# JunkyByte/easy_ViTPose

Measured on AMD Instinct MI355X. Metric: persons_per_sec, higher is better.
Workload: dtype fp16; 1 GPU; ViTPose-B coco K=17, batch 256 x 256x192 crops per GPU (f32 input resident in HBM) -> (y,x,conf) keypoints in HBM; global_batch=256, weights=seeded random init (no checkpoint offline)

## Files before the change

### easy_vitpose_amd/_capi.py

```python
from __future__ import annotations

import ctypes as C
import os

LIB_PATH = os.path.join(os.path.dirname(os.path.abspath(__file__)), '_lib', 'libvitpose_hip.so')

VP_OK, VP_ERR_INVALID, VP_ERR_HIP, VP_ERR_STATE, VP_ERR_MISSING_TENSOR, VP_ERR_SHAPE = range(6)
VP_DTYPE_F16, VP_DTYPE_BF16, VP_DTYPE_FP8 = 0, 1, 2
VP_INPUT_F32_NCHW, VP_INPUT_U8_NHWC = 0, 1
VP_PIX_RGB24, VP_PIX_BGR24, VP_PIX_NV12 = 0, 1, 2
VP_YUV_BT601, VP_YUV_BT709, VP_YUV_BT601_FULL = 0, 1, 2
VP_PROF_NAMES = ['gemm_proj', 'gemm_fc1', 'gemm_qkv', 'gemm_patch', 'gemm_deconv', 'gemm_final',
                 'attention', 'layernorm', 'im2col', 'decode', 'gemm_fc2']
VP_PROF_COUNT = len(VP_PROF_NAMES)
DTYPES = {'fp16': VP_DTYPE_F16, 'f16': VP_DTYPE_F16, 'bf16': VP_DTYPE_BF16, 'fp8': VP_DTYPE_FP8}

SYMBOLS = ['vp_abi_version', 'vp_create', 'vp_load_weights', 'vp_infer', 'vp_infer_device', 'vp_infer_device_stream', 'vp_host_alloc', 'vp_host_free',
           'vp_infer_submit', 'vp_infer_wait', 'vp_group_create', 'vp_group_size', 'vp_group_member', 'vp_group_load_weights', 'vp_group_infer',
           'vp_group_infer_allgather', 'vp_group_destroy', 'vp_group_last_error', 'vp_infer_frame', 'vp_infer_flip', 'vp_infer_heatmaps',
           'vp_infer_tokens', 'vp_decode_only', 'vp_stream', 'vp_synchronize', 'vp_set_profiling',
           'vp_reset_profile', 'vp_get_profile', 'vp_profile_kernel', 'vp_group_peer_access_missing', 'vp_destroy', 'vp_last_error',
           'vp_dbg_gemm', 'vp_dbg_attention', 'vp_dbg_layernorm', 'vp_dbg_deconv', 'vp_dbg_gemm_case', 'vp_dbg_crop_prep',
           'vp_dbg_group_plan', 'vp_dbg_group_trace', 'vp_dbg_gemm8_pick', 'vp_dbg_gemm2_pick', 'vp_dbg_splitk_pick', 'vp_dbg_run_batch', 'vp_dbg_fp8_gemm', 'vp_dbg_mx_gemm', 'vp_dbg_host_e4m3', 'vp_dbg_gemm_fp8_case', 'vp_dbg_qkvattn',
           'vp_expert_info', 'vp_set_expert', 'vp_infer_experts', 'vp_dbg_expert_tile', 'vp_infer_frames', 'vp_dbg_frame_plan',
           'vp_dbg_chunk_plan', 'vp_infer_boxes_stream', 'vp_dbg_box_geometry',
           'vp_set_flip_test', 'vp_clear_flip_test', 'vp_flip_test_enabled', 'vp_group_set_flip_test', 'vp_group_clear_flip_test',
           'vp_dbg_flip_partner', 'vp_dbg_flip_layout', 'vp_dbg_decode_flip',
           'vp_infer_experts_device_stream', 'vp_infer_frames_experts', 'vp_infer_boxes_experts_stream', 'vp_dbg_mix_plan', 'vp_dbg_decode_mix',
           'vp_set_flip_test_experts', 'vp_dbg_mix_plan_flip', 'vp_dbg_decode_flip_mix',
           'vp_infer_images', 'vp_infer_boxes_images_stream', 'vp_dbg_image_plan', 'vp_dbg_crop_prep_image',
           'vp_dbg_gemm_case_planes', 'vp_dbg_gemm_fp8_case_planes', 'vp_dbg_attention_case',
           'vp_pose_nms_stream', 'vp_pose_nms', 'vp_dbg_pose_nms_host', 'vp_dbg_pose_oks',
           'vp_dbg_ln_finalize', 'vp_dbg_gemm_case_lnpart', 'vp_dbg_qkvattn_ln', 'vp_dbg_ln_quant',
           'vp_infer_images_affine', 'vp_infer_boxes_affine_stream', 'vp_dbg_box_cs', 'vp_dbg_affine_plan', 'vp_dbg_crop_affine', 'vp_dbg_decode_affine',
           'vp_dbg_decode_affine_flip',
           'vp_draw_poses_stream', 'vp_draw_poses', 'vp_dbg_draw_host',
           'vp_tracker_create', 'vp_tracker_destroy', 'vp_tracker_reset_stream', 'vp_tracker_update_stream', 'vp_tracker_update', 'vp_tracker_state_bytes',
           'vp_tracker_download_state', 'vp_dbg_track_host', 'vp_dbg_lsap']


class HipExtensionMissing(RuntimeError):
    pass


class VpError(RuntimeError):
    def __init__(self, code: int, msg: str):
        super().__init__(f'[vitpose_hip status {code}] {msg}')
        self.code = code
        self.msg = msg


class vp_config(C.Structure):
    _fields_ = [('embed_dim', C.c_int32), ('depth', C.c_int32), ('num_heads', C.c_int32),
                ('num_keypoints', C.c_int32), ('dtype', C.c_int32), ('device_id', C.c_int32),
                ('max_batch', C.c_int32)]


class vp_tensor_desc(C.Structure):
    _fields_ = [('name', C.c_char_p), ('data', C.POINTER(C.c_float)), ('numel', C.c_int64)]


class vp_frame(C.Structure):
    _fields_ = [('data', C.c_void_p), ('h', C.c_int32), ('w', C.c_int32)]


class vp_image(C.Structure):
    _fields_ = [('plane', C.c_void_p * 2), ('pitch', C.c_int64 * 2), ('h', C.c_int32), ('w', C.c_int32), ('format', C.c_int32), ('matrix', C.c_int32)]


class vp_pose_nms_cfg(C.Structure):
    _fields_ = [('oks_thr', C.c_float), ('vis_thr', C.c_float), ('use_vis_thr', C.c_int32), ('soft', C.c_int32), ('max_dets', C.c_int32),
                ('n_sigmas', C.c_int32), ('sigmas', C.c_void_p)]


class vp_draw_cfg(C.Structure):
    _fields_ = [('conf_thr', C.c_float), ('radius', C.c_int32), ('thickness', C.c_int32), ('n_limbs', C.c_int32), ('limbs', C.c_void_p),
                ('n_point_colors', C.c_int32), ('point_colors', C.c_void_p), ('n_limb_colors', C.c_int32), ('limb_colors', C.c_void_p)]


class vp_track_cfg(C.Structure):
    _fields_ = [('max_age', C.c_int32), ('min_hits', C.c_int32), ('iou_threshold', C.c_float), ('n_streams', C.c_int32)]


class vp_profile(C.Structure):
    _fields_ = [('ms', C.c_double * VP_PROF_COUNT), ('flops', C.c_double * VP_PROF_COUNT),
                ('bytes', C.c_double * VP_PROF_COUNT), ('launches', C.c_int64 * VP_PROF_COUNT)]


_lib = None


def load_library():
    global _lib
    if _lib is not None:
        return _lib
    lib_path = os.environ.get('VP_HIP_LIB', LIB_PATH)
    if not os.path.exists(lib_path):
        raise HipExtensionMissing(
            f'{lib_path} not found. Build it with `python -m easy_vitpose_amd.build` '
            '(needs hipcc). There is no CPU fallback for the ViTPose path.')
    try:
        lib = C.CDLL(lib_path)
    except OSError as e:
        raise HipExtensionMissing(f'cannot load {lib_path}: {e}') from e
    H = C.c_void_p
    lib.vp_abi_version.restype = C.c_int
    lib.vp_create.argtypes = [C.POINTER(H), C.POINTER(vp_config)]
    lib.vp_load_weights.argtypes = [H, C.POINTER(vp_tensor_desc), C.c_int32]
    lib.vp_infer.argtypes = [H, C.c_void_p, C.c_int32, C.c_int32, C.c_void_p, C.c_void_p]
    lib.vp_infer_device.argtypes = [H, C.c_void_p, C.c_int32, C.c_int32, C.c_void_p, C.c_void_p, C.c_int32]
    lib.vp_infer_device_stream.argtypes = [H, C.c_void_p, C.c_int32, C.c_int32, C.c_void_p, C.c_void_p, C.c_void_p]
    lib.vp_host_alloc.argtypes = [C.c_size_t]
    lib.vp_host_alloc.restype = C.c_void_p
    lib.vp_host_free.argtypes = [C.c_void_p]
    lib.vp_host_free.restype = None
    lib.vp_infer_submit.argtypes = [H, C.c_void_p, C.c_int32, C.c_int32, C.c_void_p, C.c_void_p, C.POINTER(C.c_int32)]
    lib.vp_infer_wait.argtypes = [H, C.c_int32]
    lib.vp_group_create.argtypes = [C.POINTER(H), C.POINTER(vp_config), C.POINTER(C.c_int32), C.c_int32]
    lib.vp_group_size.argtypes = [H]
    lib.vp_group_member.argtypes = [H, C.c_int32]
    lib.vp_group_member.restype = C.c_void_p
    lib.vp_group_load_weights.argtypes = [H, C.POINTER(vp_tensor_desc), C.c_int32]
    lib.vp_group_infer.argtypes = [H, C.c_void_p, C.c_int32, C.c_int32, C.c_void_p, C.c_void_p]
    lib.vp_group_infer_allgather.argtypes = [H, C.c_void_p, C.c_int32, C.c_int32, C.c_void_p, C.POINTER(C.c_void_p), C.c_void_p]
    lib.vp_group_destroy.argtypes = [H]
    lib.vp_group_last_error.argtypes = [H]
    lib.vp_group_last_error.restype = C.c_char_p
    lib.vp_infer_frame.argtypes = [H, C.c_void_p, C.c_int32, C.c_int32, C.c_void_p, C.c_int32, C.c_void_p]
    lib.vp_infer_frames.argtypes = [H, C.POINTER(vp_frame), C.c_int32, C.c_int32, C.c_void_p, C.c_int32, C.c_void_p]
    lib.vp_dbg_frame_plan.argtypes = [C.POINTER(vp_frame), C.c_int32, C.c_void_p, C.c_int32, C.c_void_p]
    lib.vp_infer_boxes_stream.argtypes = [H, C.POINTER(vp_frame), C.c_int32, C.c_void_p, C.c_int32, C.c_void_p, C.c_int32, C.c_int32,
                                          C.c_void_p, C.c_void_p, C.c_void_p, C.c_void_p]
    lib.vp_dbg_box_geometry.argtypes = [C.c_void_p, C.c_int32, C.c_void_p, C.c_void_p, C.c_int32, C.c_int32, C.c_int32, C.c_void_p, C.c_void_p]
    lib.vp_dbg_crop_prep.argtypes = [C.c_int32, C.c_void_p, C.c_int32, C.c_int32, C.c_void_p, C.c_int32, C.c_void_p]
    lib.vp_infer_heatmaps.argtypes = [H, C.c_void_p, C.c_int32, C.c_int32, C.c_void_p]
    lib.vp_infer_tokens.argtypes = [H, C.c_void_p, C.c_int32, C.c_int32, C.c_void_p]
    lib.vp_decode_only.argtypes = [C.c_int32, C.c_void_p, C.c_int32, C.c_int32, C.c_void_p, C.c_void_p]
    lib.vp_stream.argtypes = [H]
    lib.vp_stream.restype = C.c_void_p
    lib.vp_synchronize.argtypes = [H]
    lib.vp_set_profiling.argtypes = [H, C.c_int32]
    lib.vp_reset_profile.argtypes = [H]
    lib.vp_get_profile.argtypes = [H, C.POINTER(vp_profile)]
    lib.vp_destroy.argtypes = [H]
    lib.vp_last_error.argtypes = [H]
    lib.vp_last_error.restype = C.c_char_p
    lib.vp_dbg_gemm.argtypes = [C.c_int32] * 6 + [C.c_void_p] * 5
    lib.vp_dbg_attention.argtypes = [C.c_int32] * 5 + [C.c_void_p] * 2
    lib.vp_dbg_attention_case.argtypes = [C.c_int32] * 6 + [C.c_void_p] * 3
    lib.vp_dbg_layernorm.argtypes = [C.c_int32] * 4 + [C.c_void_p] * 5
    lib.vp_dbg_deconv.argtypes = [C.c_int32] * 6 + [C.c_void_p, C.POINTER(vp_tensor_desc), C.c_int32, C.c_void_p]
    lib.vp_infer_flip.argtypes = [C.c_void_p, C.c_void_p, C.c_int32, C.c_int32, C.c_void_p, C.c_void_p, C.c_int32, C.c_int32,
                                  C.c_void_p, C.c_void_p]
    lib.vp_dbg_gemm_case.argtypes = [C.c_int32] * 9 + [C.c_void_p] * 8
    if hasattr(lib, 'vp_dbg_gemm8_timeline'):
        lib.vp_dbg_gemm8_timeline.argtypes = [C.c_int32] * 9 + [C.POINTER(C.c_uint64), C.c_int32]
        lib.vp_dbg_gemm_timeline.argtypes = [C.c_int32] * 6 + [C.POINTER(C.c_uint64), C.c_int32]
        lib.vp_dbg_gemm8_timeline.restype = lib.vp_dbg_gemm_timeline.restype = C.c_int
        lib.vp_dbg_gemm_bench.argtypes = [C.c_int32] * 9 + [C.POINTER(C.c_float)]
        lib.vp_dbg_gemm_bench2.argtypes = [C.c_int32] * 10 + [C.POINTER(C.c_float)]
        lib.vp_dbg_gemm_compare.argtypes = [C.c_int32] * 13 + [C.POINTER(C.c_uint64), C.POINTER(C.c_double)]
        lib.vp_dbg_peak.argtypes = [C.c_int32, C.c_int32, C.POINTER(C.c_double)]
        for n_ in ('vp_dbg_gemm_bench', 'vp_dbg_gemm_bench2', 'vp_dbg_gemm_compare', 'vp_dbg_peak'):
            getattr(lib, n_).restype = C.c_int
    lib.vp_profile_kernel.argtypes = [H, C.c_int32, C.c_char_p, C.c_int32]
    lib.vp_group_peer_access_missing.argtypes = [H]
    lib.vp_dbg_group_plan.argtypes = [C.c_int32] * 3 + [C.c_void_p, C.c_void_p, C.c_int32]
    lib.vp_dbg_gemm8_pick.argtypes = [C.c_int32] * 4 + [C.c_void_p]
    lib.vp_dbg_gemm2_pick.argtypes = [C.c_int32] * 4 + [C.c_void_p]
    lib.vp_dbg_splitk_pick.argtypes = [C.c_int32] * 3 + [C.c_void_p]
    lib.vp_dbg_run_batch.argtypes = [C.c_int32] * 3
    lib.vp_dbg_group_trace.argtypes = [C.c_int32] * 3 + [C.c_void_p, C.c_int32]
    lib.vp_dbg_fp8_gemm.argtypes = [C.c_int32] * 4 + [C.c_void_p] * 7
    lib.vp_dbg_mx_gemm.argtypes = [C.c_int32] * 4 + [C.c_void_p] * 7
    lib.vp_dbg_host_e4m3.argtypes = [C.c_void_p, C.c_void_p, C.c_int64]
    lib.vp_dbg_gemm_fp8_case.argtypes = [C.c_int32] * 5 + [C.c_void_p] * 8
    lib.vp_dbg_gemm_case_planes.argtypes = [C.c_int32] * 9 + [C.c_void_p] * 6 + [C.c_int32] + [C.c_void_p] * 3
    lib.vp_dbg_gemm_fp8_case_planes.argtypes = [C.c_int32] * 4 + [C.c_void_p] * 5 + [C.c_int32] + [C.c_void_p] * 5
    lib.vp_expert_info.argtypes = [H, C.c_void_p, C.c_void_p, C.c_void_p]
    lib.vp_set_expert.argtypes = [H, C.c_int32]
    lib.vp_infer_experts.argtypes = [H, C.c_void_p, C.c_int32, C.c_int32, C.c_void_p, C.c_void_p, C.c_void_p]
    lib.vp_dbg_expert_tile.argtypes = [C.c_int32] * 4 + [C.c_void_p, C.c_int32]
    lib.vp_infer_experts_device_stream.argtypes = [H, C.c_void_p, C.c_int32, C.c_int32, C.c_void_p, C.c_void_p, C.c_void_p, C.c_void_p]
    lib.vp_infer_frames_experts.argtypes = [H, C.POINTER(vp_frame), C.c_int32, C.c_int32, C.c_void_p, C.c_int32, C.c_void_p, C.c_void_p]
    lib.vp_infer_boxes_experts_stream.argtypes = [H, C.POINTER(vp_frame), C.c_int32, C.c_void_p, C.c_int32, C.c_void_p, C.c_int32, C.c_int32,
                                                  C.c_void_p, C.c_void_p, C.c_void_p, C.c_void_p, C.c_void_p]
    lib.vp_dbg_mix_plan.argtypes = [C.c_void_p, C.c_int32, C.c_int32, C.c_int32] + [C.c_void_p] * 6
    lib.vp_dbg_decode_mix.argtypes = [C.c_int32, C.c_void_p, C.c_int32, C.c_int32, C.c_int32, C.c_void_p, C.c_void_p, C.c_void_p]
    lib.vp_dbg_chunk_plan.argtypes = [C.POINTER(vp_config), C.c_int32, C.c_void_p, C.c_int32]
    lib.vp_dbg_qkvattn.argtypes = [C.c_int32] * 5 + [C.c_void_p] * 4
    lib.vp_dbg_qkvattn_ln.argtypes = [C.c_int32] * 5 + [C.c_void_p] * 6
    lib.vp_dbg_ln_finalize.argtypes = [C.c_int32] * 4 + [C.c_void_p] * 2
    lib.vp_dbg_gemm_case_lnpart.argtypes = [C.c_int32] * 9 + [C.c_void_p] * 4 + [C.c_int32] + [C.c_void_p] * 2
    lib.vp_dbg_ln_quant.argtypes = [C.c_int32] * 5 + [C.c_void_p] * 4
    lib.vp_set_flip_test.argtypes = [H, C.c_void_p, C.c_int32, C.c_int32]
    lib.vp_clear_flip_test.argtypes = [H]
    lib.vp_flip_test_enabled.argtypes = [H]
    lib.vp_group_set_flip_test.argtypes = [H, C.c_void_p, C.c_int32, C.c_int32]
    lib.vp_group_clear_flip_test.argtypes = [H]
    lib.vp_set_flip_test_experts.argtypes = [H, C.c_void_p, C.c_void_p, C.c_int32]
    lib.vp_dbg_mix_plan_flip.argtypes = [C.c_void_p, C.c_int32, C.c_int32, C.c_int32] + [C.c_void_p] * 6
    lib.vp_dbg_decode_flip_mix.argtypes = [C.c_int32, C.c_void_p, C.c_int32, C.c_int32, C.c_int32, C.c_void_p, C.c_void_p, C.c_int32, C.c_int32, C.c_void_p, C.c_void_p]
    lib.vp_infer_images.argtypes = [H, C.POINTER(vp_image), C.c_int32, C.c_int32, C.c_void_p, C.c_int32, C.c_void_p, C.c_void_p]
    lib.vp_infer_boxes_images_stream.argtypes = [H, C.POINTER(vp_image), C.c_int32, C.c_void_p, C.c_int32, C.c_void_p, C.c_int32, C.c_int32,
                                                 C.c_void_p, C.c_void_p, C.c_void_p, C.c_void_p, C.c_void_p]
    lib.vp_dbg_image_plan.argtypes = [C.POINTER(vp_image), C.c_int32, C.c_void_p, C.c_int32, C.c_void_p]
    lib.vp_dbg_crop_prep_image.argtypes = [C.c_int32, C.POINTER(vp_image), C.c_void_p, C.c_int32, C.c_void_p]
    lib.vp_dbg_flip_partner.argtypes = [C.c_int32, C.c_void_p, C.c_int32, C.c_void_p]
    lib.vp_dbg_flip_layout.argtypes = [C.c_int32, C.c_int32, C.c_void_p, C.c_void_p]
    lib.vp_dbg_decode_flip.argtypes = [C.c_int32, C.c_void_p, C.c_int32, C.c_int32, C.c_void_p, C.c_int32, C.c_int32, C.c_void_p, C.c_void_p]
    nms_host = [C.c_void_p, C.c_int32, C.c_int32, C.c_void_p, C.c_int32, C.c_void_p, C.c_void_p, C.c_int32, C.POINTER(vp_pose_nms_cfg), C.c_void_p, C.c_void_p, C.c_void_p]
    lib.vp_pose_nms_stream.argtypes = [H] + nms_host + [C.c_void_p]
    lib.vp_pose_nms.argtypes = [H] + nms_host
    lib.vp_dbg_pose_nms_host.argtypes = nms_host
    lib.vp_dbg_pose_oks.argtypes = [C.c_int32, C.c_void_p, C.c_int32, C.c_int32, C.c_void_p, C.POINTER(vp_pose_nms_cfg), C.c_void_p]
    lib.vp_infer_images_affine.argtypes = [H, C.POINTER(vp_image), C.c_int32, C.c_int32, C.c_void_p, C.c_void_p, C.c_int32, C.c_void_p]
    lib.vp_infer_boxes_affine_stream.argtypes = [H, C.POINTER(vp_image), C.c_int32, C.c_void_p, C.c_int32, C.c_void_p, C.c_int32, C.c_float,
                                                 C.c_void_p, C.c_void_p, C.c_void_p, C.c_void_p]
    lib.vp_dbg_box_cs.argtypes = [C.c_void_p, C.c_int32, C.c_void_p, C.c_int32, C.c_int32, C.c_float, C.c_void_p, C.c_void_p]
    lib.vp_dbg_affine_plan.argtypes = [C.POINTER(vp_image), C.c_int32, C.c_void_p, C.c_void_p, C.c_int32, C.c_void_p]
    lib.vp_dbg_crop_affine.argtypes = [C.c_int32, C.POINTER(vp_image), C.c_void_p, C.c_int32, C.c_void_p]
    lib.vp_dbg_decode_affine.argtypes = [C.c_int32, C.c_void_p, C.c_int32, C.c_int32, C.c_void_p, C.c_void_p]
    lib.vp_dbg_decode_affine_flip.argtypes = [C.c_int32, C.c_void_p, C.c_int32, C.c_int32, C.c_void_p, C.c_int32, C.c_int32, C.c_void_p, C.c_void_p]
    draw_host = [C.POINTER(vp_image), C.c_int32, C.c_void_p, C.c_int32, C.c_int32, C.c_void_p, C.c_int32, C.c_void_p, C.c_void_p, C.c_void_p, C.c_int32,
                 C.POINTER(vp_draw_cfg)]
    lib.vp_draw_poses_stream.argtypes = [H] + draw_host + [C.c_void_p]
    lib.vp_draw_poses.argtypes = [H] + draw_host
    lib.vp_dbg_draw_host.argtypes = draw_host
    trk_io = [C.c_void_p, C.c_int32, C.c_void_p, C.c_int32, C.c_uint64, C.c_void_p, C.c_void_p, C.c_void_p, C.c_int32, C.c_void_p, C.c_void_p]
    lib.vp_tracker_create.argtypes = [H, C.POINTER(vp_track_cfg), C.POINTER(C.c_void_p)]
    lib.vp_tracker_destroy.argtypes = [C.c_void_p]
    lib.vp_tracker_reset_stream.argtypes = [C.c_void_p, C.c_uint64, C.c_void_p]
    lib.vp_tracker_update_stream.argtypes = [C.c_void_p] + trk_io + [C.c_void_p]
    lib.vp_tracker_update.argtypes = [C.c_void_p] + trk_io
    lib.vp_tracker_state_bytes.argtypes = [C.c_int32, C.POINTER(C.c_int64)]
    lib.vp_tracker_download_state.argtypes = [C.c_void_p, C.c_void_p]
    lib.vp_dbg_track_host.argtypes = [C.c_void_p, C.POINTER(vp_track_cfg)] + trk_io
    lib.vp_dbg_lsap.argtypes = [C.c_int32, C.c_void_p, C.c_int32, C.c_int32, C.c_float, C.c_void_p]
    for name in SYMBOLS:
        if name not in ('vp_stream', 'vp_last_error', 'vp_host_alloc', 'vp_host_free', 'vp_group_member', 'vp_group_last_error'):
            getattr(lib, name).restype = C.c_int
    _lib = lib
    return lib


def last_error(handle=None) -> str:
    lib = load_library()
    s = lib.vp_last_error(handle)
    return s.decode('utf-8', 'replace') if s else ''


def check(code: int, handle=None):
    if code != VP_OK:
        raise VpError(code, last_error(handle))
```

### easy_vitpose_amd/csrc/api_internal.h

```cpp
#pragma once
#include <hip/hip_runtime.h>

#include <algorithm>
#include <cmath>
#include <cstdio>
#include <cstdlib>
#include <cstring>
#include <string>
#include <unordered_map>
#include <vector>

#include "../../include/vitpose_hip.h"
#ifdef VP_TOOLS
#include "../../include/vitpose_hip_tools.h"
#endif
#include "kernels.h"
#include "mx8.h"

namespace vpi {

struct Block {
    float *ln1_g, *ln1_b, *ln2_g, *ln2_b;
    uint16_t *w_qkv, *w_proj, *w_fc1, *w_fc2;
    float *b_qkv, *b_proj, *b_fc1, *b_fc2;
    float *s_qkv, *s_fc1;
    uint16_t* w_qkvh = nullptr;
    float *b_qkvh = nullptr, *s_qkvh = nullptr;
    uint8_t *w_qkv8 = nullptr, *w_fc18 = nullptr, *w_fc28 = nullptr, *w_proj8 = nullptr;
    float *ws_qkv = nullptr, *ws_fc1 = nullptr, *ws_fc2 = nullptr, *ws_proj = nullptr;
};

struct Switches {
    int g8_stagger = 0;
    int gemm8_mask = 0x7;
    long g8_min_tiles = 448;
    bool persist_gemm = true;
    int order_mask = 8;
    bool blocked_hid = true;
    bool blocked_qkv = true;
    bool fuse_ln = true;
    bool fuse_qkv_attn = true;
    bool qa_min_set = false;
    long qa_min_tiles = 108;
    long qa80_min_tiles = 192;
    int qa80_group = 8;
    int attn_qsplit = 128;
    int g8_bm192 = 3;
    bool pad_batch = true;
    bool g8_cost_model = true;
    bool deconv_parity_fast = true;
    bool fuse_head = true;
    bool fp8_proj16 = false;
    int graph_max_n = 16;
    bool graph_null = true;
    int caller_stream_max_n = 16;
    bool fold_rule = true;
    int graph_max_n_stats = 8;
    bool splitk_on = true;
    int splitk_force[2][2] = {{0, 0}, {0, 0}};
    int gemm_variant[VP_PROF_COUNT] = {-1, -1, -1, -1, -1, -1, -1, -1, -1, -1, -1};
    int gemm_group_m[VP_PROF_COUNT] = {0};
    int fam_ablate[VP_PROF_COUNT] = {0};
};

}

namespace vpi {
struct MixPlan {
    int nb = 0;
    std::vector<int32_t> order, ids;
    std::vector<int> seg_e, seg_s;
    uint64_t pattern = 0;
};
}

struct vp_ctx {
    vp_config cfg;
    vpi::Switches sw;
    int D, L, heads, Kp, dtype, maxb;
    hipStream_t stream = nullptr;
    std::string err;
    bool loaded = false;
    std::vector<void*> allocs;
    uint16_t* w_patch = nullptr;
    float* pos = nullptr;
    std::vector<vpi::Block> blocks;
    float *lnf_g = nullptr, *lnf_b = nullptr;
    uint16_t *w_d1 = nullptr, *w_d2 = nullptr, *w_fin = nullptr;
    size_t fin_rows = 0;
    float *b_d1 = nullptr, *b_d2 = nullptr, *b_fin = nullptr, *b_zero = nullptr;
    uint16_t* zero = nullptr;
    void* in_stage = nullptr;
    int32_t* wh_stage = nullptr;
    float* x = nullptr;
    uint16_t *y = nullptr, *qkv = nullptr, *hid = nullptr, *d1 = nullptr, *d2 = nullptr;
    float *hm = nullptr, *kp = nullptr, *tok = nullptr;
    float* hm_keep = nullptr;
    int32_t* partner = nullptr;
    bool flip_on = false;
    int flip_shift = 0;
    uint32_t flip_gen = 0, flip_counter = 0;
    int32_t* flip_table = nullptr;
    std::vector<int32_t> flip_pairs;
    bool flip_ex = false;
    int32_t* flip_tables = nullptr;
    float *ln_part = nullptr, *rowstat = nullptr;
    bool fp8 = false;
    size_t Mp = 0;
    uint8_t *x8 = nullptr, *xs8 = nullptr, *hs8 = nullptr;
    uint8_t *y8 = nullptr, *ys8 = nullptr;
    struct Slot {
        void* in = nullptr; int32_t* wh = nullptr; float* kp = nullptr; hipEvent_t h2d = nullptr, done = nullptr, out = nullptr; bool busy = false;
        float* host_kp = nullptr; float* user_out = nullptr; size_t out_bytes = 0;
        char* host_in = nullptr; size_t host_in_cap = 0;
    };
    Slot slots[2];
    hipStream_t copy_stream = nullptr;
    hipStream_t d2h_stream = nullptr;
    int next_slot = 0;
    struct GraphKey {
        int n = 0, fmt = -1;
        const void* src = nullptr; const int32_t* wh = nullptr; float* out = nullptr;
        int expert = 0;
        const int32_t* post = nullptr;
        uint32_t flip = 0;
        const float* cs = nullptr;
        uint64_t mix = 0;
        bool wide = false;
        bool operator==(const GraphKey& o) const {
            return n == o.n && fmt == o.fmt && src == o.src && wh == o.wh && out == o.out && expert == o.expert && post == o.post && flip == o.flip &&
                   cs == o.cs && mix == o.mix && wide == o.wide;
        }
    };
    struct GraphEntry { GraphKey key; hipGraphExec_t exec = nullptr; bool no_graph = false; };
    GraphEntry graphs[4];
    int graph_victim = 0;
    float* splitk_ws = nullptr;
    size_t splitk_rows = 0;
    hipEvent_t ev_in = nullptr, ev_out = nullptr;
    hipStream_t own_stream = nullptr;
    const void* last_stream_id = nullptr;
    bool foreign_pending = false;
    hipEvent_t ev_sw = nullptr;
    uint8_t* frame_stage = nullptr;
    size_t frame_cap = 0;
    vp::CropRec* crecs = nullptr;
    vp::AffRec* arecs = nullptr;
    float* cs_stage = nullptr;
    void* draw_ws = nullptr;
    int32_t* box_aux = nullptr;
    struct Head { uint16_t *w_d1 = nullptr, *w_d2 = nullptr, *w_fin = nullptr; float *b_d1 = nullptr, *b_d2 = nullptr, *b_fin = nullptr; size_t fin_rows = 0; int K = 0; };
    int Kmax = 0;
    int n_experts = 0, part_features = 0, expert = 0;
    size_t fc2_w_stride = 0, fc2_b_stride = 0;
    std::vector<Head> ex_heads;
    int32_t* expert_ids = nullptr;
    void* mix_stage = nullptr;
    size_t mix_stage_cap = 0;
    const int32_t* mix_expert = nullptr;
    std::vector<int> mix_bounds;
    int32_t* mix_slot = nullptr;
    vp::MixRec* mix_recs = nullptr;
    vp::MixRecFlip* mix_recs_flip = nullptr;
    const vpi::MixPlan* mix = nullptr;
    vpi::MixPlan mix_host;
    std::vector<int32_t> mix_ks, mix_first, mix_k;
    uint32_t prof = 0;
    int gemm_ablate = 0;
    struct Ev { hipEvent_t a, b; int fam; double flops, bytes; };
    std::vector<Ev> evs;
    std::vector<std::pair<hipEvent_t, hipEvent_t>> ev_pool;
    vp_profile acc{};
    std::string kernel_desc[VP_PROF_COUNT];
};

namespace vpi {

extern thread_local std::string g_create_error;

int fail(vp_ctx* c, int code, const std::string& msg);
int need_weights(vp_ctx* c);
bool slots_busy(const vp_ctx* c);
int slots_idle(vp_ctx* c, const char* who);
int quiesce(vp_ctx* c);
inline size_t crop_bytes(int fmt) { return (size_t)3 * 256 * 192 * (fmt == VP_INPUT_F32_NCHW ? 4 : 1); }

#define HIPCHK(c, expr)                                                                         \
    do {                                                                                        \
        hipError_t e__ = (expr);                                                                \
        if (e__ != hipSuccess)                                                                  \
            return fail((c), VP_ERR_HIP, std::string(#expr) + ": " + hipGetErrorString(e__));   \
    } while (0)

template <class T> int dalloc(vp_ctx* c, T** p, size_t count) {
    void* q = nullptr;
    HIPCHK(c, hipMalloc(&q, count * sizeof(T) + 256));
    c->allocs.push_back(q);
    *p = (T*)q;
    return VP_OK;
}

uint16_t host_to_bits(float v, int dtype);
float host_from_bits(uint16_t h, int dtype);
size_t pad128(size_t n);
// ... 115 lines not shown
```

### easy_vitpose_amd/csrc/debug_taps.hip

```cpp
#include "dbg_util.h"

using namespace vpi;


static int upload_planes(vp_ctx* c, uint16_t** dst, const float* aux, const uint16_t* r_hi, const uint16_t* r_lo, size_t MN) {
    if (!(r_hi && r_lo) && !aux) return fail(c, VP_ERR_INVALID, "aux required");
    std::vector<uint16_t> hp(2 * MN);
    if (r_hi && r_lo) {
        std::memcpy(hp.data(), r_hi, MN * 2);
        std::memcpy(hp.data() + MN, r_lo, MN * 2);
    } else
        for (size_t i = 0; i < MN; ++i) {
            const uint16_t hi = host_to_bits(aux[i], c->dtype);
            hp[i] = hi;
            hp[MN + i] = host_to_bits(aux[i] - host_from_bits(hi, c->dtype), c->dtype);
        }
    int r;
    if ((r = dalloc(c, dst, 2 * MN))) return r;
    if (hipMemcpy(*dst, hp.data(), hp.size() * 2, hipMemcpyHostToDevice) != hipSuccess) return fail(c, VP_ERR_HIP, "H2D");
    return VP_OK;
}
static int download_planes(vp_ctx* c, const uint16_t* planes, float* out, uint16_t* o_hi, uint16_t* o_lo, size_t MN) {
    if (o_hi && o_lo) {
        if (hipMemcpy(o_hi, planes, MN * 2, hipMemcpyDeviceToHost) != hipSuccess || hipMemcpy(o_lo, planes + MN, MN * 2, hipMemcpyDeviceToHost) != hipSuccess)
// ... 80 lines not shown
    const size_t out_bytes = mx ? MD : MD * 2;
    if ((rc = dalloc(c, &dq, M * N3)) || (rc = dalloc(c, &dout, out_bytes)) || (mx && (rc = dalloc(c, &dsc, MD / 32)))) return dbg_finish(c, rc);
    hipError_t e = hipMemcpy(dq, hq.data(), hq.size() * 2, hipMemcpyHostToDevice);
    if (e == hipSuccess) e = hipMemset(dout, 0xff, out_bytes);
    if (e == hipSuccess && mx) e = hipMemset(dsc, 0xff, MD / 32);
    if (e == hipSuccess) e = vp::attention_launch(c->dtype, dq, (uint16_t*)dout, B, D, heads, nullptr, qsplit, blocked, dsc);
    if (e == hipSuccess) e = hipDeviceSynchronize();
    if (e != hipSuccess) return dbg_finish(c, fail(c, VP_ERR_HIP, std::string("attention case: ") + hipGetErrorString(e)));
    if (!mx) return dbg_finish(c, download16(c, (const uint16_t*)dout, out, MD));
    std::vector<uint8_t> co(MD), so(MD / 32);
    if (hipMemcpy(co.data(), dout, MD, hipMemcpyDeviceToHost) != hipSuccess || hipMemcpy(so.data(), dsc, MD / 32, hipMemcpyDeviceToHost) != hipSuccess)
        return dbg_finish(c, fail(c, VP_ERR_HIP, "D2H"));
    for (size_t m = 0; m < M; ++m)
        for (size_t n = 0; n < (size_t)D; ++n) {
            const uint8_t sb = so[vp::mx_scale_off(m, n >> 5, D)];
            out[m * D + n] = vp_host_e4m3_to_float(co[vp::mx_code_off(m, n, D)]) * std::ldexp(1.0f, (int)sb - 127);
            if (!(n & 31)) out_scales[m * (D / 32) + (n >> 5)] = sb;
        }
    return dbg_finish(c, VP_OK);
}

}

static int qkvattn_case(int32_t device, int32_t dtype, int32_t npairs, int32_t D, int32_t heads, const float* x, const float* W, const float* bias, const float* rowstat,
                        const float* ln_s, float* out) {
    if (npairs <= 0 || D <= 0 || heads <= 0 || !x || !W || !bias || !out || !rowstat != !ln_s) return fail(nullptr, VP_ERR_INVALID, "bad qkvattn test shape");
    vp_ctx* c = dbg_ctx(device, dtype);
    if (!c) return VP_ERR_HIP;
    const size_t M = (size_t)npairs * 384;
    uint16_t *dx, *dw, *dwh, *dy;
    float *db, *dbh, *ds, *dsh, *drow;
    int rc;
    std::vector<float> zeros(3 * (size_t)D, 0.f), row(2 * M);
    for (size_t m = 0; m < M; ++m) { row[2 * m] = 0.f; row[2 * m + 1] = 1.f; }
    if ((rc = upload_mat(c, &dx, x, M, D, M)) || (rc = upload_mat(c, &dw, W, 3 * (size_t)D, D, pad128(3 * (size_t)D))) || (rc = upload_f32(c, &db, bias, 3 * (size_t)D)) ||
        (rc = upload_f32(c, &ds, ln_s ? ln_s : zeros.data(), 3 * (size_t)D)) || (rc = upload_f32(c, &drow, rowstat ? rowstat : row.data(), 2 * M)) || (rc = dalloc(c, &dwh, 3 * (size_t)D * D)) ||
        (rc = dalloc(c, &dbh, 3 * (size_t)D)) || (rc = dalloc(c, &dsh, 3 * (size_t)D)) || (rc = dalloc(c, &dy, M * D)))
        return dbg_finish(c, rc);
    if (heads * 80 == D) {
        uint16_t* dwh80; float *dbh80, *dsh80;
        const size_t rows = (size_t)heads * 256;
        if ((rc = dalloc(c, &dwh80, rows * D)) || (rc = dalloc(c, &dbh80, rows)) || (rc = dalloc(c, &dsh80, rows))) return dbg_finish(c, rc);
        hipError_t e8 = vp::qkv_head_major80_launch(dw, db, ds, dwh80, dbh80, dsh80, D, D, heads, nullptr);
        vp::GemmArgs g80{};
        g80.A = dx; g80.W = dwh80; g80.bias = dbh80; g80.ln_s = dsh80; g80.rowstat = drow; g80.out = dy;
        g80.M = (int)M; g80.N = heads * 256; g80.K = D; g80.ldo = D; g80.w_rows = heads * 256; g80.variant = 18;
        g80.attn_scale_log2e = vp::softmax_scale_log2e(80);
        if (e8 == hipSuccess && !vp::gemm8_supported(vp::EPI_QKV_ATTN, g80, 256, 192)) return dbg_finish(c, fail(c, VP_ERR_INVALID, "shape not supported by the fused qkv + attention tile (head dim 80)"));
        if (e8 == hipSuccess) e8 = vp::gemm_launch(c->dtype, vp::EPI_QKV_ATTN, g80, nullptr);
        if (e8 == hipSuccess) e8 = hipDeviceSynchronize();
        if (e8 != hipSuccess) return dbg_finish(c, fail(c, VP_ERR_HIP, std::string("qkvattn (head dim 80): ") + hipGetErrorString(e8)));
        return dbg_finish(c, download16(c, dy, out, M * D));
    }
    hipError_t e = vp::qkv_head_major_launch(dw, db, ds, dwh, dbh, dsh, D, D, nullptr);
    vp::QkvAttnArgs qa{};
    qa.x_hi = dx; qa.wh = dwh; qa.bh = dbh; qa.sh = dsh; qa.rowstat = drow; qa.y = dy; qa.npairs = npairs; qa.ncrops = 2 * npairs; qa.heads = heads; qa.D = D;
    qa.scale_log2e = vp::softmax_scale_log2e(64);
    if (e == hipSuccess && !vp::qkvattn_supported(qa)) return dbg_finish(c, fail(c, VP_ERR_INVALID, "shape not supported by the fused qkv + attention kernel"));
    if (e == hipSuccess) e = vp::qkvattn_launch(c->dtype, qa, nullptr, nullptr, 0);
    if (e == hipSuccess) e = hipDeviceSynchronize();
    if (e != hipSuccess) return dbg_finish(c, fail(c, VP_ERR_HIP, std::string("qkvattn: ") + hipGetErrorString(e)));
    return dbg_finish(c, download16(c, dy, out, M * D));
}

extern "C" {

VP_API int vp_dbg_qkvattn(int32_t device, int32_t dtype, int32_t npairs, int32_t D, int32_t heads, const float* x, const float* W, const float* bias, float* out) {
    return qkvattn_case(device, dtype, npairs, D, heads, x, W, bias, nullptr, nullptr, out);
}

VP_API int vp_dbg_qkvattn_ln(int32_t device, int32_t dtype, int32_t npairs, int32_t D, int32_t heads, const float* x, const float* W, const float* bias,
                             const float* rowstat, const float* ln_s, float* out) {
    if (!rowstat || !ln_s) return fail(nullptr, VP_ERR_INVALID, "bad qkvattn test shape");
    return qkvattn_case(device, dtype, npairs, D, heads, x, W, bias, rowstat, ln_s, out);
}

VP_API int vp_dbg_ln_finalize(int32_t device, int32_t M, int32_t tiles, int32_t D, const float* partials, float* rowstat) {
    if (M <= 0 || tiles <= 0 || D <= 0 || !partials || !rowstat) return fail(nullptr, VP_ERR_INVALID, "bad ln_finalize case");
    vp_ctx* c = dbg_ctx(device, VP_DTYPE_F16);
    if (!c) return VP_ERR_HIP;
    float *dP, *dR;
    int rc;
    if ((rc = upload_f32(c, &dP, partials, (size_t)M * tiles * 2)) || (rc = dalloc(c, &dR, (size_t)M * 2))) return dbg_finish(c, rc);
    hipError_t e = hipMemset(dR, 0xff, (size_t)M * 8);
    if (e == hipSuccess) e = vp::ln_finalize_launch(dP, dR, M, tiles, D, nullptr);
    if (e == hipSuccess) e = hipDeviceSynchronize();
    if (e == hipSuccess) e = hipMemcpy(rowstat, dR, (size_t)M * 8, hipMemcpyDeviceToHost);
    if (e != hipSuccess) rc = fail(c, VP_ERR_HIP, std::string("ln_finalize: ") + hipGetErrorString(e));
    return dbg_finish(c, rc);
}

VP_API int vp_dbg_ln_quant(int32_t device, int32_t dtype, int32_t M, int32_t Mp, int32_t D, const uint16_t* x_hi, const float* partials, uint8_t* codes, uint8_t* scales) {
    if (M <= 0 || Mp < M || Mp % 64 || D <= 0 || D % 128 || !x_hi || !partials || !codes || !scales || (dtype != VP_DTYPE_F16 && dtype != VP_DTYPE_BF16))
        return fail(nullptr, VP_ERR_INVALID, "bad ln_quant case");
    vp_ctx* c = dbg_ctx(device, dtype);
    if (!c) return VP_ERR_HIP;
    const size_t MD = (size_t)M * D, PD = (size_t)Mp * D;
    uint16_t* dX;
    float* dP;
    uint8_t *dC, *dS;
    int rc;
    if ((rc = dalloc(c, &dX, MD)) || (rc = upload_f32(c, &dP, partials, (size_t)M * (D / 64) * 2)) || (rc = dalloc(c, &dC, PD)) || (rc = dalloc(c, &dS, PD / 32)))
        return dbg_finish(c, rc);
    hipError_t e = hipMemcpy(dX, x_hi, MD * 2, hipMemcpyHostToDevice);
    if (e == hipSuccess) e = hipMemset(dC, 0xff, PD);
    if (e == hipSuccess) e = hipMemset(dS, 0xff, PD / 32);
    if (e == hipSuccess) e = vp::ln_quant_launch(c->dtype, dX, dP, D / 64, dC, dS, M, Mp, D, nullptr);
    if (e == hipSuccess) e = hipDeviceSynchronize();
    if (e == hipSuccess) e = hipMemcpy(codes, dC, PD, hipMemcpyDeviceToHost);
    if (e == hipSuccess) e = hipMemcpy(scales, dS, PD / 32, hipMemcpyDeviceToHost);
    if (e != hipSuccess) rc = fail(c, VP_ERR_HIP, std::string("ln_quant: ") + hipGetErrorString(e));
    return dbg_finish(c, rc);
}

VP_API int vp_dbg_layernorm(int32_t device, int32_t dtype, int32_t M, int32_t D, const float* x, const float* gamma,
                            const float* beta, float* out16, float* out32) {
    vp_ctx* c = dbg_ctx(device, dtype);
    if (!c) return VP_ERR_HIP;
    float *dx, *dg, *db, *d32;
    uint16_t* d16;
    int rc;
    const size_t MD = (size_t)M * D;
    if ((rc = upload_f32(c, &dx, x, MD)) || (rc = upload_f32(c, &dg, gamma, D)) || (rc = upload_f32(c, &db, beta, D)) ||
        (rc = dalloc(c, &d32, MD)) || (rc = dalloc(c, &d16, MD))) return dbg_finish(c, rc);
    hipError_t e = vp::layernorm_launch(c->dtype, dx, dg, db, d16, d32, M, D, nullptr);
    if (e == hipSuccess) e = hipDeviceSynchronize();
    if (e == hipSuccess) e = hipMemcpy(out32, d32, MD * 4, hipMemcpyDeviceToHost);
    if (e != hipSuccess) return dbg_finish(c, fail(c, VP_ERR_HIP, std::string("layernorm: ") + hipGetErrorString(e)));
    return dbg_finish(c, download16(c, d16, out16, MD));
}

VP_API int vp_dbg_deconv(int32_t device, int32_t dtype, int32_t B, int32_t Hin, int32_t Win, int32_t Cin, const float* x,
                         const vp_tensor_desc* tensors, int32_t n_tensors, float* out) {
    vp_ctx* c = dbg_ctx(device, dtype);
    if (!c) return VP_ERR_HIP;
    Lookup lk;
    lk.c = c;
    for (int i = 0; i < n_tensors; ++i) lk.map[tensors[i].name] = &tensors[i];
    uint16_t *dx, *dw, *dout;
    float* db;
    int rc;
    const size_t Min = (size_t)B * Hin * Win;
    if ((rc = pack_deconv(c, lk, 0, Cin, &dw, &db))) return dbg_finish(c, rc);
    if ((rc = upload_mat(c, &dx, x, Min, Cin, Min))) return dbg_finish(c, rc);
    if ((rc = dalloc(c, &dout, Min * 4 * 256))) return dbg_finish(c, rc);
    if ((rc = dalloc(c, &c->zero, (size_t)256))) return dbg_finish(c, rc);
    if (hipMemset(c->zero, 0, 512) != hipSuccess) return dbg_finish(c, fail(c, VP_ERR_HIP, "memset"));
    rc = gemm(c, 0, vp::EPI_DECONV, resolve_gemm(c->sw, 0, vp::EPI_DECONV, (int)Min, 256, 4 * Cin), dx, dw, db, dout, nullptr, (int)Min, 256, 4 * Cin, 256, Hin, Win, Cin);
    if (!rc && hipDeviceSynchronize() != hipSuccess) rc = fail(c, VP_ERR_HIP, "deconv kernel failed");
    if (!rc) rc = download16(c, dout, out, Min * 4 * 256);
    return dbg_finish(c, rc);
}


static int gemm_case(int32_t device, int32_t dtype, int32_t epi, int32_t variant, int32_t group_m, int32_t flags, int32_t M, int32_t N, int32_t K, const float* A,
                     const float* W, const float* bias, const float* aux, const float* rowstat, const float* ln_s, float* out, float* stats, const PlaneIO* io,
                     const float* ln_part = nullptr, int ln_tiles = 0) {
    if (M <= 0 || N <= 0 || K <= 0 || K % 64 || !A || !W || !bias) return fail(nullptr, VP_ERR_INVALID, "bad gemm case");
    vp_ctx* c = dbg_ctx(device, dtype);
    if (!c) return VP_ERR_HIP;
    c->Kp = N;
    int r;
    const size_t MN = (size_t)M * N, wrows = pad128(N);
    const bool ablk = (flags & 4) != 0, oblk = (flags & 2) != 0;
    uint16_t *dA, *dW;
    float *dB, *dAux32 = nullptr, *dRow = nullptr, *dS = nullptr, *dStats = nullptr;
    uint16_t* dAux16 = nullptr;
    void* dOut = nullptr;
    {
        std::vector<uint16_t> ha((size_t)M * K);
        for (size_t m = 0; m < (size_t)M; ++m)
            for (size_t k = 0; k < (size_t)K; ++k) {
                const size_t dst = ablk ? ((((m >> 6) * (K >> 6) + (k >> 6)) << 12) + ((m & 63) << 6) + (k & 63)) : m * K + k;
                ha[dst] = host_to_bits(A[m * K + k], c->dtype);
            }
        if ((r = dalloc(c, &dA, (size_t)M * K))) return dbg_finish(c, r);
        if (hipMemcpy(dA, ha.data(), ha.size() * 2, hipMemcpyHostToDevice) != hipSuccess) return dbg_finish(c, fail(c, VP_ERR_HIP, "H2D"));
    }
    size_t fin_rows = 0;
    if (epi == vp::EPI_HEATMAP) { if ((r = upload_final(c, &dW, W, N, K, &fin_rows))) return dbg_finish(c, r); }
    else if ((r = upload_mat(c, &dW, W, N, K, wrows))) return dbg_finish(c, r);
    if ((r = upload_f32(c, &dB, bias, N, wrows)) || (r = dalloc(c, &c->zero, (size_t)256))) return dbg_finish(c, r);
    vp::GemmArgs g{};
    g.A = dA; g.W = dW; g.bias = dB; g.M = M; g.N = N; g.K = K; g.ldo = N; g.zero = c->zero; g.Kp = N;
    g.w_rows = (int)wrows; g.variant = variant; g.group_m = group_m;
    g.persist = (flags & 1) != 0; g.out_blocked = oblk; g.a_blocked = ablk; g.reverse = (flags & 8) != 0;
    if (rowstat && ln_s) {
        if ((r = upload_f32(c, &dRow, rowstat, (size_t)M * 2)) || (r = upload_f32(c, &dS, ln_s, N, wrows))) return dbg_finish(c, r);
        g.rowstat = dRow; g.ln_s = dS;
    }
    if (ln_part) {
        float* dPart;
        if ((r = upload_f32(c, &dPart, ln_part, (size_t)M * ln_tiles * 2)) || (r = upload_f32(c, &dS, ln_s, N, wrows))) return dbg_finish(c, r);
        g.ln_part = dPart; g.ln_tiles = ln_tiles; g.ln_inv_d = 1.0f / (float)K; g.ln_s = dS;
    }
    size_t out_bytes = 0;
    const bool prod = epi == vp::EPI_BIAS_RESID_LN || epi == vp::EPI_POS_LN;
    if (epi == vp::EPI_BIAS || epi == vp::EPI_BIAS_GELU) out_bytes = MN * 2;
    else if (epi == vp::EPI_BIAS_RESID || epi == vp::EPI_POS || prod) out_bytes = MN * 4;
    else if (epi == vp::EPI_HEATMAP) { out_bytes = MN * 4; g.N = (int)fin_rows; g.ldo = 0; g.w_rows = (int)pad128(fin_rows); }
    else return dbg_finish(c, fail(c, VP_ERR_INVALID, "unsupported epilogue"));
    if (epi == vp::EPI_BIAS_RESID || epi == vp::EPI_POS || epi == vp::EPI_POS_LN) {
        if (!aux) return dbg_finish(c, fail(c, VP_ERR_INVALID, "aux required"));
        if ((r = upload_f32(c, &dAux32, aux, epi == vp::EPI_BIAS_RESID ? MN : (size_t)192 * N))) return dbg_finish(c, r);
        g.aux = dAux32;
    }
    if (epi == vp::EPI_BIAS_RESID_LN) {
        if ((r = upload_planes(c, &dAux16, aux, io ? io->r_hi : nullptr, io ? io->r_lo : nullptr, MN))) return dbg_finish(c, r);
        g.aux = (const float*)dAux16;
    }
    if (prod) {
        g.plane = MN;
        if ((r = dalloc(c, &dStats, (size_t)M * (N / 64) * 2))) return dbg_finish(c, r);
        g.stats_out = dStats;
    }
    if (io && io->in_place) dOut = dAux16;
    else {
        char* o;
        if ((r = dalloc(c, &o, out_bytes))) return dbg_finish(c, r);
        dOut = o;
        hipMemset(dOut, 0xff, out_bytes);
    }
    g.out = dOut;
    const int splitk = (flags >> 8) & 15;
    hipError_t e;
    if (splitk > 1) {
        if (epi != vp::EPI_BIAS_RESID_LN) return dbg_finish(c, fail(c, VP_ERR_INVALID, "split-K is a residual-GEMM path (epi 6)"));
        float* ws = nullptr;
        if ((r = dalloc(c, &ws, (size_t)splitk * MN))) return dbg_finish(c, r);
        hipMemset(ws, 0xff, (size_t)splitk * MN * 4);
        vp::GemmArgs p = g;
        p.out = ws; p.aux = nullptr; p.bias = nullptr; p.stats_out = nullptr; p.plane = 0; p.splitk = splitk; p.persist = 0;
        e = vp::gemm_launch(c->dtype, vp::EPI_PARTIAL, p, nullptr);
        if (e == hipSuccess) e = vp::splitk_reduce_launch(c->dtype, ws, splitk, dB, dAux16, MN, dStats, M, N, nullptr);
        dOut = dAux16;
    } else {
        e = vp::gemm_launch(c->dtype, epi, g, nullptr);
    }
    if (e == hipSuccess) e = hipDeviceSynchronize();
    if (e != hipSuccess) return dbg_finish(c, fail(c, VP_ERR_HIP, std::string("gemm case: ") + hipGetErrorString(e)));
    if (epi == vp::EPI_BIAS || epi == vp::EPI_BIAS_GELU) {
        std::vector<float> t(MN);
        if ((r = download16(c, (const uint16_t*)dOut, t.data(), MN))) return dbg_finish(c, r);
        for (size_t m = 0; m < (size_t)M; ++m)
            for (size_t n = 0; n < (size_t)N; ++n) {
                const size_t src = oblk ? ((((m >> 6) * ((size_t)N >> 6) + (n >> 6)) << 12) + ((m & 63) << 6) + (n & 63)) : m * N + n;
                out[m * N + n] = t[src];
            }
    } else if (prod) {
        if ((r = download_planes(c, (const uint16_t*)dOut, out, io ? io->o_hi : nullptr, io ? io->o_lo : nullptr, MN))) return dbg_finish(c, r);
        if (stats && hipMemcpy(stats, dStats, (size_t)M * (N / 64) * 8, hipMemcpyDeviceToHost) != hipSuccess) return dbg_finish(c, fail(c, VP_ERR_HIP, "D2H"));
    } else {
        if (hipMemcpy(out, dOut, out_bytes, hipMemcpyDeviceToHost) != hipSuccess) return dbg_finish(c, fail(c, VP_ERR_HIP, "D2H"));
    }
    return dbg_finish(c, VP_OK);
}

VP_API int vp_dbg_gemm_case(int32_t device, int32_t dtype, int32_t epi, int32_t variant, int32_t group_m, int32_t flags, int32_t M,
                            int32_t N, int32_t K, const float* A, const float* W, const float* bias, const float* aux, const float* rowstat,
                            const float* ln_s, float* out, float* stats) {
    if (!out) return fail(nullptr, VP_ERR_INVALID, "bad gemm case");
    return gemm_case(device, dtype, epi, variant, group_m, flags, M, N, K, A, W, bias, aux, rowstat, ln_s, out, stats, nullptr);
}

VP_API int vp_dbg_gemm_case_lnpart(int32_t device, int32_t dtype, int32_t epi, int32_t variant, int32_t group_m, int32_t flags, int32_t M, int32_t N, int32_t K,
                                   const float* A, const float* W, const float* bias, const float* partials, int32_t ln_tiles, const float* ln_s, float* out) {
    if ((epi != vp::EPI_BIAS && epi != vp::EPI_BIAS_GELU) || !partials || ln_tiles <= 0 || !ln_s || !out) return fail(nullptr, VP_ERR_INVALID, "bad gemm ln_part case");
    return gemm_case(device, dtype, epi, variant, group_m, flags, M, N, K, A, W, bias, nullptr, nullptr, ln_s, out, nullptr, nullptr, partials, ln_tiles);
}

VP_API int vp_dbg_gemm_case_planes(int32_t device, int32_t dtype, int32_t epi, int32_t variant, int32_t group_m, int32_t flags, int32_t M, int32_t N, int32_t K,
                                   const float* A, const float* W, const float* bias, const uint16_t* r_hi, const uint16_t* r_lo, const float* pos,
                                   int32_t in_place, uint16_t* o_hi, uint16_t* o_lo, float* stats) {
    if ((epi != vp::EPI_BIAS_RESID_LN && epi != vp::EPI_POS_LN) || !o_hi || !o_lo || !stats || (epi == vp::EPI_BIAS_RESID_LN ? !r_hi || !r_lo : !pos || in_place))
        return fail(nullptr, VP_ERR_INVALID, "bad gemm planes case");
    const PlaneIO io{r_hi, r_lo, o_hi, o_lo, in_place != 0};
    return gemm_case(device, dtype, epi, variant, group_m, flags, M, N, K, A, W, bias, pos, nullptr, nullptr, nullptr, stats, &io);
}

VP_API int vp_dbg_crop_prep_image(int32_t device, const vp_image* image, const int32_t* crop_params, int32_t n, uint8_t* out) {
    if (!image || !crop_params || !out || n <= 0) return fail(nullptr, VP_ERR_INVALID, "bad argument");
    std::vector<int32_t> p9((size_t)n * 9, 0);
    for (int i = 0; i < n; ++i) std::memcpy(&p9[9 * (size_t)i + 1], crop_params + 8 * (size_t)i, 32);
    int32_t band[2];
    std::string why;
    if (image_plan(image, 1, p9.data(), n, band, &why)) return fail(nullptr, VP_ERR_INVALID, why);
    vp_ctx* c = dbg_ctx(device, VP_DTYPE_F16);
    if (!c) return VP_ERR_HIP;
    std::vector<vp::CropRec> recs;
    uint8_t* dout;
    vp::CropRec* drec;
    int rc;
    const size_t ob = (size_t)n * 256 * 192 * 3;
    if ((rc = stage_frames(c, image, 1, false, p9.data(), n, band, recs)) || (rc = dalloc(c, &dout, ob)) || (rc = dalloc(c, &drec, (size_t)n)))
        return dbg_finish(c, rc);
    hipError_t e = hipMemcpy(drec, recs.data(), (size_t)n * sizeof(vp::CropRec), hipMemcpyHostToDevice);
    if (e == hipSuccess) e = vp::crop_resize_launch(drec, dout, n, nullptr);
    if (e == hipSuccess) e = hipDeviceSynchronize();
    if (e == hipSuccess) e = hipMemcpy(out, dout, ob, hipMemcpyDeviceToHost);
    if (e != hipSuccess) rc = fail(c, VP_ERR_HIP, std::string("crop_prep: ") + hipGetErrorString(e));
    return dbg_finish(c, rc);
}

VP_API int vp_dbg_crop_affine(int32_t device, const vp_image* image, const float* cs, int32_t n, uint8_t* out) {
    if (!image || !cs || !out || n <= 0) return fail(nullptr, VP_ERR_INVALID, "bad argument");
    int32_t band[2];
// ... 158 lines not shown
```

### easy_vitpose_amd/csrc/forward.hip

```cpp
#include "api_internal.h"
#include "tiles.h"

using namespace vpi;

namespace vpi {

static void note_kernel(vp_ctx* c, int fam, const char* desc) {
    if (desc[0] && c->kernel_desc[fam] != desc) c->kernel_desc[fam] = desc;
}

int gemm(vp_ctx* c, int fam, int epi, const GemmPick& pk, const uint16_t* A, const uint16_t* W, const float* bias, void* out,
         const float* aux, int M, int N, int K, int ldo, int Hin, int Win, int Cin, const LnFuse* ln) {
    vp::GemmArgs g{};
    g.A = A; g.W = W; g.bias = bias; g.out = out; g.aux = aux;
    g.M = M; g.N = N; g.K = K; g.ldo = ldo;
    g.Hin = Hin; g.Win = Win; g.Cin = Cin; g.zero = c->zero; g.Kp = c->Kp;
    g.w_rows = (int)pad128((size_t)N);
    g.variant = pk.variant; g.group_m = pk.group_m; g.persist = pk.persist; g.stagger = pk.stagger;
    g.ablate = c->gemm_ablate | c->sw.fam_ablate[fam];
    g.parity_fast = c->sw.deconv_parity_fast;
    if (c->mix_expert && fam == VP_PROF_GEMM_FC2) g.expert = c->mix_expert;
    if (ln) {
        g.a_blocked = ln->a_blocked; g.out_blocked = ln->out_blocked; g.reverse = ln->reverse;
        g.plane = ln->plane; g.stats_out = ln->stats_out; g.rowstat = ln->rowstat; g.ln_s = ln->ln_s;
        g.ln_part = ln->ln_part; g.ln_tiles = ln->ln_tiles; g.ln_inv_d = 1.0f / (float)K;
        if (ln->tiles_out) *ln->tiles_out = N / 64;
    }
    if (epi == vp::EPI_DECONV_FINAL) { g.W2 = c->w_fin; g.bias2 = c->b_fin; g.out2 = (float*)out; g.out = nullptr; }
    const bool deconv = epi == vp::EPI_DECONV || epi == vp::EPI_DECONV_FINAL;
    const double par = deconv ? 4.0 : 1.0;
    const double Nalg = (epi == vp::EPI_HEATMAP) ? (double)c->Kp : (double)N;
    double flops = 2.0 * M * Nalg * K * par;
    const bool resid = epi == vp::EPI_BIAS_RESID || epi == vp::EPI_BIAS_RESID_LN;
    const bool f32out = resid || epi == vp::EPI_POS || epi == vp::EPI_POS_LN || epi == vp::EPI_HEATMAP;
    const double out_b = f32out ? 4.0 : 2.0;
    double bytes = 2.0 * M * (double)(deconv ? Cin : K) + 2.0 * N * (double)K * par + out_b * M * Nalg * par;
    if (epi == vp::EPI_DECONV_FINAL) {
        flops += 2.0 * M * par * (double)c->Kp * N;
        bytes += (4.0 * c->Kp - out_b * N) * M * par + 2.0 * c->fin_rows * N;
    }
    if (resid) bytes += 4.0 * M * (double)N;
    if (epi == vp::EPI_BIAS_RESID_LN || epi == vp::EPI_POS_LN) bytes += 8.0 * M * (double)(N / 64);
    char desc[192];
    desc[0] = 0;
    g.desc = desc; g.desc_cap = (int)sizeof(desc);
    if (pk.splitk > 1) {
        if (out != (void*)aux || (size_t)M > c->splitk_rows || !c->splitk_ws) return fail(c, VP_ERR_INVALID, "split-K: a residual GEMM in place within the workspace only");
        vp::GemmArgs p = g;
        p.out = c->splitk_ws; p.aux = nullptr; p.bias = nullptr; p.stats_out = nullptr; p.plane = 0;
        p.variant = pk.splitk_variant; p.group_m = 0; p.splitk = pk.splitk; p.ldo = N; p.persist = 0;
        LAUNCH(c, fam, flops, bytes, vp::gemm_launch(c->dtype, vp::EPI_PARTIAL, p, c->stream));
        if (desc[0]) {
            char d2[224];
            snprintf(d2, sizeof(d2), "%s x split-K %d + splitk_reduce_kernel", desc, pk.splitk);
            note_kernel(c, fam, d2);
        }
        LAUNCH(c, fam, 0.0, 0.0, vp::splitk_reduce_launch(c->dtype, c->splitk_ws, pk.splitk, bias, (uint16_t*)out, g.plane, g.stats_out, M, N, c->stream));
        return VP_OK;
    }
    LAUNCH(c, fam, flops, bytes, vp::gemm_launch(c->dtype, epi, g, c->stream));
    note_kernel(c, fam, desc);
    return VP_OK;
}

int gemm_fp8(vp_ctx* c, int fam, int epi, const GemmPick& pk, const uint8_t* A8, const uint8_t* a_scales, const uint8_t* W8, const float* w_scale, const float* bias,
             void* out, uint8_t* out_scales, const float* aux, int M, int N, int K, const LnFuse* ln) {
    vp::GemmArgs g{};
    g.A = (const uint16_t*)A8; g.W = (const uint16_t*)W8; g.bias = bias; g.out = out; g.aux = aux;
    g.M = M; g.N = N; g.K = K; g.ldo = N;
    g.a_scales = a_scales; g.w_scale = w_scale; g.out_scales = out_scales;
    g.w_rows = (int)pad128((size_t)N);
    if (ln) {
        g.out_blocked = ln->out_blocked; g.reverse = ln->reverse;
        g.plane = ln->plane; g.stats_out = ln->stats_out;
        if (ln->tiles_out) *ln->tiles_out = N / 64;
    }
    const int bn = vp::tile8_bn(pk.variant);
    g.group_m = pk.group_m;
    if (!vp::gemm8f_supported(epi, g, bn))
        return fail(c, VP_ERR_SHAPE, "fp8 mode: GEMM shape " + std::to_string(M) + " x " + std::to_string(N) + " x " + std::to_string(K) + " not supported by the MXFP8 kernel");
    const double flops = 2.0 * M * (double)N * K;
    double bytes = 1.0 * M * (double)K + M * (double)(K / 32) + 1.0 * N * (double)K;
    bytes += epi == vp::EPI_BIAS ? 2.0 * M * (double)N : epi == vp::EPI_BIAS_GELU ? (1.0 + 1.0 / 32) * M * (double)N : 8.0 * M * (double)N + 8.0 * M * (double)(N / 64);
    char desc[192];
    desc[0] = 0;
    g.desc = desc; g.desc_cap = (int)sizeof(desc);
    LAUNCH(c, fam, flops, bytes, vp::gemm8f_launch(epi, g, bn, c->stream));
    note_kernel(c, fam, desc);
    return VP_OK;
}

static const uint16_t* fc2_w(const vp_ctx* c, const vpi::Block& b) { return c->mix_expert ? b.w_fc2 : b.w_fc2 + (size_t)c->expert * c->fc2_w_stride; }
static const float* fc2_b(const vp_ctx* c, const vpi::Block& b) { return c->mix_expert ? b.b_fc2 : b.b_fc2 + (size_t)c->expert * c->fc2_b_stride; }

int forward_chunk(vp_ctx* c, const void* d_crops, int fmt, int n_in, const FwdOpts& o) {
    const int D = c->D;
    const ChunkPlan pl = plan_chunk(c->sw, D, c->heads, c->maxb, c->fp8, n_in, c->fin_rows, c->mix_expert ? &c->mix_bounds : nullptr);
    const GemmPick* pk = pl.gemm;
    const int n = pl.n;
    const int M = n * 192;
    const double in_b = (fmt == VP_INPUT_F32_NCHW ? 4.0 : 1.0) * n_in * 3.0 * 256 * 192;
    if (o.twin_src) LAUNCH(c, VP_PROF_IM2COL, 0.0, 0.5 * in_b + 2.0 * M * 768, vp::im2col_twin_launch(c->dtype, d_crops, fmt, c->hid, n, o.twin_src, c->stream));
    else LAUNCH(c, VP_PROF_IM2COL, 0.0, in_b + 2.0 * M * 768, vp::im2col_launch(c->dtype, d_crops, fmt, c->hid, n, c->stream, o.mirror, n_in));
    int rc;
    size_t plane = 0;
    const bool qkv_blocked = c->sw.blocked_qkv && D / c->heads == 64;
    auto attention = [&](uint16_t* out, double bytes, uint8_t* mx_scales) -> int {
        LAUNCH(c, VP_PROF_ATTN, 4.0 * 192 * 192 * (double)D * n, bytes,
               vp::attention_launch(c->dtype, c->qkv, out, n, D, c->heads, c->stream, pl.attn_qsplit, qkv_blocked ? 1 : 0, mx_scales));
        return VP_OK;
    };
    if (c->fp8) {
        const int Mp = (int)std::max<size_t>((size_t)(M + 255) / 256 * 256, 512);
        plane = c->Mp * (size_t)D;
        uint16_t* xh = (uint16_t*)c->x;
        int tiles = 0;
        LnFuse prod; prod.plane = plane; prod.stats_out = c->ln_part; prod.tiles_out = &tiles;
        auto quant = [&]() -> int {
            LAUNCH(c, VP_PROF_LAYERNORM, 0.0, 8.0 * M * tiles + 2.0 * M * D + (1.0 + 1.0 / 32) * Mp * (double)D,
                   vp::ln_quant_launch(c->dtype, xh, c->ln_part, tiles, c->x8, c->xs8, M, Mp, D, c->stream));
            return VP_OK;
        };
        if ((rc = gemm(c, VP_PROF_GEMM_PATCH, vp::EPI_POS_LN, pk[VP_PROF_GEMM_PATCH], c->hid, c->w_patch, c->b_zero, c->x, c->pos, M, D, 768, D, 0, 0, 0, &prod))) return rc;
        for (int l = 0; l < c->L; ++l) {
            const Block& b = c->blocks[l];
            if ((rc = quant())) return rc;
            LnFuse cq; cq.out_blocked = qkv_blocked;
            if ((rc = gemm_fp8(c, VP_PROF_GEMM_QKV, vp::EPI_BIAS, pk[VP_PROF_GEMM_QKV], c->x8, c->xs8, b.w_qkv8, b.ws_qkv, b.b_qkv, c->qkv, nullptr, nullptr, Mp, 3 * D, D, &cq))) return rc;
            LnFuse pp = prod;
            if (pl.proj_fp8) {
                if ((rc = attention((uint16_t*)c->y8, 7.0 * M * D, c->ys8))) return rc;
                if ((rc = gemm_fp8(c, VP_PROF_GEMM_PROJ, vp::EPI_BIAS_RESID_LN, pk[VP_PROF_GEMM_PROJ], c->y8, c->ys8, b.w_proj8, b.ws_proj, b.b_proj, c->x, nullptr, c->x, Mp, D, D, &pp))) return rc;
            } else {
                if ((rc = attention(c->y, 8.0 * M * D, nullptr))) return rc;
                if ((rc = gemm(c, VP_PROF_GEMM_PROJ, vp::EPI_BIAS_RESID_LN, pk[VP_PROF_GEMM_PROJ], c->y, b.w_proj, b.b_proj, c->x, c->x, M, D, D, D, 0, 0, 0, &pp))) return rc;
            }
            if ((rc = quant())) return rc;
            if ((rc = gemm_fp8(c, VP_PROF_GEMM_FC1, vp::EPI_BIAS_GELU, pk[VP_PROF_GEMM_FC1], c->x8, c->xs8, b.w_fc18, b.ws_fc1, b.b_fc1, c->hid, c->hs8, nullptr, Mp, 4 * D, D, nullptr))) return rc;
            LnFuse p2 = prod;
            if ((rc = gemm_fp8(c, VP_PROF_GEMM_FC2, vp::EPI_BIAS_RESID_LN, pk[VP_PROF_GEMM_FC2], (const uint8_t*)c->hid, c->hs8, b.w_fc28, b.ws_fc2, b.b_fc2, c->x, nullptr, c->x, Mp, D, 4 * D, &p2))) return rc;
        }
    } else if (c->sw.fuse_ln) {
        plane = (size_t)M * D;
        uint16_t* xh = (uint16_t*)c->x;
        int tiles = 0;
        LnFuse prod; prod.plane = plane; prod.stats_out = c->ln_part; prod.tiles_out = &tiles;
        auto finalize = [&](bool folded) -> int {
            if (folded) return VP_OK;
            LAUNCH(c, VP_PROF_LAYERNORM, 0.0, 8.0 * M * tiles + 8.0 * M, vp::ln_finalize_launch(c->ln_part, c->rowstat, M, tiles, D, c->stream));
            return VP_OK;
        };
        const double qkv_attn_flops = 2.0 * M * 3.0 * D * D + 4.0 * 192 * 192 * (double)D * n, qkv_attn_bytes = 2.0 * M * D + 2.0 * 3 * D * (double)D + 2.0 * M * D;
        if ((rc = gemm(c, VP_PROF_GEMM_PATCH, vp::EPI_POS_LN, pk[VP_PROF_GEMM_PATCH], c->hid, c->w_patch, c->b_zero, c->x, c->pos, M, D, 768, D, 0, 0, 0, &prod))) return rc;
        if ((rc = finalize(pl.fold1))) return rc;
        for (int l = 0; l < c->L; ++l) {
            const Block& b = c->blocks[l];
            if (pl.qkv_path == QKV_ATTN80) {
                vp::GemmArgs g80{};
                g80.A = xh; g80.W = b.w_qkvh; g80.bias = b.b_qkvh; g80.ln_s = b.s_qkvh; g80.rowstat = c->rowstat; g80.out = c->y;
                g80.M = M; g80.N = c->heads * 256; g80.K = D; g80.ldo = D; g80.w_rows = c->heads * 256; g80.variant = 18;
                g80.group_m = c->sw.qa80_group;
                g80.attn_scale_log2e = vp::softmax_scale_log2e(80);
                g80.ablate = c->gemm_ablate | c->sw.fam_ablate[VP_PROF_GEMM_QKV];
                char desc[192];
                desc[0] = 0;
                g80.desc = desc; g80.desc_cap = (int)sizeof(desc);
                LAUNCH(c, VP_PROF_GEMM_QKV, qkv_attn_flops, qkv_attn_bytes, vp::gemm_launch(c->dtype, vp::EPI_QKV_ATTN, g80, c->stream));
                note_kernel(c, VP_PROF_GEMM_QKV, desc);
            } else if (pl.qkv_path == QKV_ATTN64) {
                vp::QkvAttnArgs qa{};
                qa.x_hi = xh; qa.wh = b.w_qkvh; qa.bh = b.b_qkvh; qa.sh = b.s_qkvh; qa.rowstat = c->rowstat; qa.y = c->y;
                qa.npairs = (n + 1) / 2; qa.ncrops = n; qa.heads = c->heads; qa.D = D;
                qa.scale_log2e = vp::softmax_scale_log2e(64);
                char desc[96];
                desc[0] = 0;
                LAUNCH(c, VP_PROF_GEMM_QKV, qkv_attn_flops, qkv_attn_bytes, vp::qkvattn_launch(c->dtype, qa, c->stream, desc, (int)sizeof(desc)));
                note_kernel(c, VP_PROF_GEMM_QKV, desc);
            } else {
                LnFuse cq; cq.rowstat = c->rowstat; cq.ln_s = b.s_qkv; cq.reverse = (c->sw.order_mask & 1) != 0; cq.out_blocked = qkv_blocked;
                if (pl.fold1) { cq.rowstat = nullptr; cq.ln_part = c->ln_part; cq.ln_tiles = D / 64; }
                if ((rc = gemm(c, VP_PROF_GEMM_QKV, vp::EPI_BIAS, pk[VP_PROF_GEMM_QKV], xh, b.w_qkv, b.b_qkv, c->qkv, nullptr, M, 3 * D, D, 3 * D, 0, 0, 0, &cq))) return rc;
// ... 199 lines not shown
```

### easy_vitpose_amd/csrc/gemm.hip

```cpp
#include <cstdio>
#include <cstdlib>
#include <type_traits>
#include <utility>

#include "common.h"
#include "kernels.h"
#include "tiles.h"

namespace vp {

template <int BM_, int BN_, int BK_, int WM_, int WN_, int STAGES_, int PIPE_ = 0>
struct TileCfg {
    static constexpr int BM = BM_, BN = BN_, BK = BK_, WM = WM_, WN = WN_, STAGES = STAGES_;
    static constexpr int PIPE = PIPE_;
    static_assert(PIPE == 0 || PIPE == 1 || PIPE == 6, "PIPE");
    static constexpr int NWM = BM / WM, NWN = BN / WN, NWAVES = NWM * NWN, NT = NWAVES * 64;
    static constexpr int ROWB = BK * 2;
    static constexpr int SLOTS = ROWB / 16;
    static constexpr int RPG = 1024 / ROWB;
    static constexpr int W_BYTES = BN * ROWB, A_BYTES = BM * ROWB, STAGE_BYTES = W_BYTES + A_BYTES;
    static constexpr int LDS = STAGES * STAGE_BYTES;
    static constexpr int WP = BN / RPG / NWAVES, AP = BM / RPG / NWAVES;
    static constexpr int G = WP + AP;
    static constexpr int KK = BK / 32, TI = WN / 16, TJ = WM / 16;
    static_assert(BK == 64 || BK == 32, "BK");
    static_assert(WP * RPG * NWAVES == BN && AP * RPG * NWAVES == BM, "tile rows must split evenly over waves");
    static_assert(LDS <= 160 * 1024, "LDS");
};

template <int BK> __device__ __forceinline__ int swz(int row, int slot) {
    return BK == 64 ? (slot ^ ((row >> 1) & 7)) : (slot ^ (((row >> 3) & 1) * 3));
}


template <class C, int ES> constexpr int epi_rows_per_pass() {
    int jp = C::TJ;
    while (jp > 1 && C::NWM * jp * 16 * (C::BN * ES + 16) > C::LDS) jp /= 2;
    return jp;
}

template <class C> constexpr int epi_rows_per_pass_ln() {
    int jp = C::TJ;
    while (jp > 1 && C::NWM * jp * 16 * (C::BN * 4 + 16) + C::BM * (C::BN / 64) * 8 > C::LDS) jp /= 2;
    return jp;
}

template <class T, int EPI_, int AMODE, class C, bool EXPERT = false>
__global__ __launch_bounds__(C::NT, 2) void gemm_kernel(GemmArgs g) {
    constexpr bool LN_PROD = (EPI_ == EPI_BIAS_RESID_LN || EPI_ == EPI_POS_LN);
    constexpr int EPI = LN_PROD ? EPI_ - 4 : EPI_;
    extern __shared__ __attribute__((aligned(16))) char smem[];
    const int tid = threadIdx.x, lane = tid & 63, wave = tid >> 6;
    const int tiles_n = (g.N + C::BN - 1) / C::BN;
    const int tiles_m = (g.M + C::BM - 1) / C::BM;
    int bid, parity = 0, split = 0;
    if (AMODE == A_DECONV && g.parity_fast) {
        const int lb = xcd_remap(blockIdx.x, tiles_m * tiles_n * 4);
        parity = lb & 3;
        bid = lb >> 2;
    } else if (EPI_ == EPI_PARTIAL) {
        const int lb = xcd_remap(blockIdx.x, tiles_m * tiles_n * g.splitk);
        split = lb / (tiles_m * tiles_n);
        bid = lb - split * (tiles_m * tiles_n);
    } else {
        bid = xcd_remap(blockIdx.x, tiles_m * tiles_n);
        if (AMODE == A_DECONV) parity = blockIdx.y;
    }
    if (g.reverse) bid = tiles_m * tiles_n - 1 - bid;
    int tm, tn;
    if (g.group_m > 1) {
        const int per_group = g.group_m * tiles_n;
        const int grp = bid / per_group, first_m = grp * g.group_m;
        const int gsz = min(tiles_m - first_m, g.group_m);
        const int r = bid - grp * per_group;
        tm = first_m + r % gsz;
        tn = r / gsz;
    } else {
        tm = bid / tiles_n;
        tn = bid - tm * tiles_n;
    }
    const int n0 = tn * C::BN, m0 = tm * C::BM;
    if constexpr (EXPERT) {
        const int e = g.expert[m0 / 192];
        g.W += (size_t)e * g.w_rows * g.K;
        g.bias += (size_t)e * g.w_rows;
    }
    const int K = g.K;
    const int klen = (EPI_ == EPI_PARTIAL) ? K / g.splitk : K;
    const int kbase = (EPI_ == EPI_PARTIAL) ? split * klen : 0;

    const int rip = lane / C::SLOTS, pslot = lane % C::SLOTS;
    const uint16_t* wsrc[C::WP];
    const uint16_t* asrc[C::AP];
    int ai[C::AP], aj[C::AP];
    const uint16_t* W = g.W + (AMODE == A_DECONV ? (size_t)parity * g.w_parity_stride : 0);
#pragma unroll
    for (int p = 0; p < C::WP; ++p) {
        const int r = (p * C::NWAVES + wave) * C::RPG + rip;
        wsrc[p] = W + (size_t)(n0 + r) * K + swz<C::BK>(r, pslot) * 8;
    }
#pragma unroll
    for (int p = 0; p < C::AP; ++p) {
        const int r = (p * C::NWAVES + wave) * C::RPG + rip;
        int m = ((VP_ABLATE(g) & 2) ? 0 : m0) + r;
        if (m > g.M - 1) m = g.M - 1;
        const int sl = swz<C::BK>(r, pslot) * 8;
        if (AMODE == A_DENSE) {
            asrc[p] = g.a_blocked ? g.A + ((size_t)(m >> 6) * (K >> 6) << 12) + ((m & 63) << 6) + sl : g.A + (size_t)m * K + sl;
        } else {
            const int t = m / g.Win;
            ai[p] = t % g.Hin;
            aj[p] = m - t * g.Win;
            asrc[p] = g.A + (size_t)m * g.Cin + sl;
        }
    }
    auto stage = [&](int kt, int buf) {
        char* base = smem + buf * C::STAGE_BYTES + wave * 1024;
        const int k0 = kbase + kt * C::BK;
#pragma unroll
        for (int p = 0; p < C::WP; ++p) glds16(wsrc[p] + k0, base + p * (C::NWAVES * 1024));
        if (AMODE == A_DENSE) {
            const int ka = g.a_blocked ? ((k0 >> 6) << 12) + (k0 & 63) : k0;
#pragma unroll
            for (int p = 0; p < C::AP; ++p) glds16(asrc[p] + ka, base + C::W_BYTES + p * (C::NWAVES * 1024));
        } else {
            const int tap = k0 / g.Cin, c0 = k0 - tap * g.Cin;
            const int ti = tap >> 1, tj = tap & 1;
            const int pa = parity >> 1, pb = parity & 1;
            const int di = pa ? (ti ? 0 : 1) : (ti ? -1 : 0);
            const int dj = pb ? (tj ? 0 : 1) : (tj ? -1 : 0);
#pragma unroll
            for (int p = 0; p < C::AP; ++p) {
                const bool ok = (unsigned)(ai[p] + di) < (unsigned)g.Hin && (unsigned)(aj[p] + dj) < (unsigned)g.Win;
                const uint16_t* src = ok ? asrc[p] + (ptrdiff_t)(di * g.Win + dj) * g.Cin + c0 : g.zero + pslot * 8;
                glds16(src, base + C::W_BYTES + p * (C::NWAVES * 1024));
            }
        }
    };

    const int wn = wave / C::NWM, wm = wave % C::NWM;
    const int frow = lane & 15, fg = lane >> 4;
    const int foff = frow * C::ROWB + (swz<C::BK>(frow, fg) << 4);
    const int woff = wn * C::WN * C::ROWB + foff;
    const int aoff = C::W_BYTES + wm * C::WM * C::ROWB + foff;

    f32x4 acc[C::TI][C::TJ];
#pragma unroll
    for (int i = 0; i < C::TI; ++i)
#pragma unroll
        for (int j = 0; j < C::TJ; ++j) acc[i][j] = f32x4{0.f, 0.f, 0.f, 0.f};

    const int nk = klen / C::BK;
    constexpr int KS = (C::PIPE == 6) ? 2 : 1;
    static_assert(C::PIPE != 6 || (C::STAGES >= 4 && C::KK == 2), "PIPE 6: >= 4 stages, BK = 64");
#pragma unroll
    for (int s = 0; s < C::STAGES - KS; ++s)
        if (s < nk) stage(s, s);
    if constexpr (EPI == EPI_BIAS || EPI == EPI_BIAS_GELU) {
        if (g.ln_part) {
            float2* st = (float2*)(smem + C::LDS);
            for (int r = tid; r < C::BM; r += C::NT) {
                int m = m0 + r;
                if (m > g.M - 1) m = g.M - 1;
                const float* src = g.ln_part + (size_t)m * g.ln_tiles * 2;
                float mean = 0.f, rstd = 1.f;
                switch (g.ln_tiles) {
                    case 6: ln_merge_row<6>(src, g.ln_inv_d, mean, rstd); break;
                    case 12: ln_merge_row<12>(src, g.ln_inv_d, mean, rstd); break;
                    case 16: ln_merge_row<16>(src, g.ln_inv_d, mean, rstd); break;
                    case 20: ln_merge_row<20>(src, g.ln_inv_d, mean, rstd); break;
                    default: ln_merge(src, g.ln_tiles, g.ln_inv_d, mean, rstd);
                }
                st[r] = float2{mean, rstd};
            }
        }
    }
    int buf = 0, pbuf = C::STAGES - KS;
    for (int kt = 0; kt < nk; kt += KS) {
        if (C::STAGES > 2 * KS && kt + C::STAGES - KS <= nk) wait_vmcnt<C::G * (C::STAGES - 2 * KS)>();
        else wait_vmcnt<0>();
        __builtin_amdgcn_s_barrier();
        asm volatile("" ::: "memory");
#pragma unroll
        for (int ks = 0; ks < KS; ++ks) {
            const int pb = pbuf + ks >= C::STAGES ? pbuf + ks - C::STAGES : pbuf + ks;
            if (kt + C::STAGES - KS + ks < nk && !(VP_ABLATE(g) & 1)) stage(kt + C::STAGES - KS + ks, pb);
        }
#pragma unroll
        for (int ks = 0; ks < KS; ++ks) {
            const int cbuf = buf + ks >= C::STAGES ? buf + ks - C::STAGES : buf + ks;
            const char* sb = smem + cbuf * C::STAGE_BYTES;
            if (C::PIPE == 1 && C::KK == 2) {
                u32x4 wf0[C::TI], af0[C::TJ], wf1[C::TI], af1[C::TJ];
#pragma unroll
                for (int i = 0; i < C::TI; ++i) wf0[i] = *(const u32x4*)(sb + (woff + i * 16 * C::ROWB));
#pragma unroll
                for (int j = 0; j < C::TJ; ++j) af0[j] = *(const u32x4*)(sb + (aoff + j * 16 * C::ROWB));
                __builtin_amdgcn_sched_barrier(0);
                __builtin_amdgcn_s_setprio(1);
#pragma unroll
                for (int i = 0; i < C::TI / 2; ++i)
#pragma unroll
                    for (int j = 0; j < C::TJ; ++j) acc[i][j] = mfma16<T>(wf0[i], af0[j], acc[i][j]);
                __builtin_amdgcn_sched_barrier(0);
#pragma unroll
                for (int i = 0; i < C::TI; ++i) wf1[i] = *(const u32x4*)(sb + ((woff + i * 16 * C::ROWB) ^ 64));
#pragma unroll
                for (int j = 0; j < C::TJ; ++j) af1[j] = *(const u32x4*)(sb + ((aoff + j * 16 * C::ROWB) ^ 64));
                __builtin_amdgcn_sched_barrier(0);
#pragma unroll
                for (int i = C::TI / 2; i < C::TI; ++i)
#pragma unroll
                    for (int j = 0; j < C::TJ; ++j) acc[i][j] = mfma16<T>(wf0[i], af0[j], acc[i][j]);
                __builtin_amdgcn_sched_barrier(0);
#pragma unroll
                for (int i = 0; i < C::TI; ++i)
#pragma unroll
                    for (int j = 0; j < C::TJ; ++j) acc[i][j] = mfma16<T>(wf1[i], af1[j], acc[i][j]);
                __builtin_amdgcn_s_setprio(0);
            } else {
#pragma unroll
                for (int kk = 0; kk < C::KK; ++kk) {
                    u32x4 wf[C::TI], af[C::TJ];
#pragma unroll
                    for (int i = 0; i < C::TI; ++i) wf[i] = *(const u32x4*)(sb + ((woff + i * 16 * C::ROWB) ^ (kk << 6)));
#pragma unroll
                    for (int j = 0; j < C::TJ; ++j) af[j] = *(const u32x4*)(sb + ((aoff + j * 16 * C::ROWB) ^ (kk << 6)));
#pragma unroll
                    for (int i = 0; i < C::TI; ++i)
#pragma unroll
                        for (int j = 0; j < C::TJ; ++j) acc[i][j] = mfma16<T>(wf[i], af[j], acc[i][j]);
                }
            }
        }
        buf = (buf + KS >= C::STAGES) ? buf + KS - C::STAGES : buf + KS;
        pbuf = (pbuf + KS >= C::STAGES) ? pbuf + KS - C::STAGES : pbuf + KS;
    }

    if constexpr (EPI == EPI_DECONV_FINAL) {
        static_assert(C::BN == 256 && C::BM % (C::NWAVES * 16) == 0, "the fused head needs all 256 channels in one tile");
        constexpr int RB = C::BN * 2 + 16;
        constexpr int RPW = C::BM / C::NWAVES, JW = RPW / 16;
        f32x4 bias4[C::TI];
#pragma unroll
        for (int i = 0; i < C::TI; ++i) bias4[i] = *(const f32x4*)(g.bias + wn * C::WN + i * 16 + fg * 4);
        asm volatile("s_waitcnt vmcnt(0)" ::: "memory");
        __syncthreads();
#pragma unroll
        for (int j = 0; j < C::TJ; ++j) {
            char* lrow = smem + (wm * C::WM + j * 16 + frow) * RB + (wn * C::WN + fg * 4) * 2;
#pragma unroll
            for (int i = 0; i < C::TI; ++i) {
                f32x4 v = acc[i][j] + bias4[i];
#pragma unroll
                for (int r = 0; r < 4; ++r) v[r] = fmaxf(v[r], 0.f);
                u32x2 o;
                o[0] = pack2<T>(v[0], v[1]);
                o[1] = pack2<T>(v[2], v[3]);
                *(u32x2*)(lrow + i * 32) = o;
            }
        }
        const int groups = (g.Kp + 15) >> 4;
        auto ldw = [&](u32x4(&w)[16], int u) {
            int frow_w = frow, fg_w = fg;
            asm volatile("" : "+v"(frow_w), "+v"(fg_w));
            const uint16_t* wrow = g.W2 + (size_t)(u * 32 + frow_w) * C::BN + fg_w * 8;
#pragma unroll
            for (int ks = 0; ks < 8; ++ks) {
                w[2 * ks] = *(const u32x4*)(wrow + ks * 32);
                w[2 * ks + 1] = *(const u32x4*)(wrow + 16 * C::BN + ks * 32);
            }
        };
        u32x4 wA[16], wB[16];
        ldw(wA, 0);
        __syncthreads();
        u32x4 bf[JW][8];
#pragma unroll
        for (int jj = 0; jj < JW; ++jj)
#pragma unroll
            for (int ks = 0; ks < 8; ++ks) bf[jj][ks] = *(const u32x4*)(smem + (wave * RPW + jj * 16 + frow) * RB + (ks * 32 + fg * 8) * 2);
        int oimg[JW], opx[JW];
        const int opix = 4 * g.Hin * g.Win;
#pragma unroll
        for (int jj = 0; jj < JW; ++jj) {
            const int m = m0 + wave * RPW + jj * 16 + frow;
            const int t = m / g.Win, jx = m - t * g.Win, ii = t % g.Hin, img = t / g.Hin;
            oimg[jj] = (m < g.M && !(VP_ABLATE(g) & 8)) ? img : -1;
            opx[jj] = (2 * ii + (parity >> 1)) * (2 * g.Win) + 2 * jx + (parity & 1);
        }
        auto group = [&](const u32x4(&w)[16], int u) {
            f32x4 ah[JW], al[JW];
            int fg_g = fg;
            asm volatile("" : "+v"(fg_g));
            const int nb = u * 16 + fg_g * 4;
            const f32x4 b2 = *(const f32x4*)(g.bias2 + nb);
#pragma unroll
            for (int jj = 0; jj < JW; ++jj) { ah[jj] = f32x4{0.f, 0.f, 0.f, 0.f}; al[jj] = f32x4{0.f, 0.f, 0.f, 0.f}; }
#pragma unroll
            for (int ks = 0; ks < 8; ++ks)
#pragma unroll
                for (int jj = 0; jj < JW; ++jj) {
                    ah[jj] = mfma16<T>(w[2 * ks], bf[jj][ks], ah[jj]);
                    al[jj] = mfma16<T>(w[2 * ks + 1], bf[jj][ks], al[jj]);
                }
#pragma unroll
            for (int jj = 0; jj < JW; ++jj) {
                const f32x4 v = ah[jj] + al[jj];
                int im = oimg[jj], px = opx[jj];
                asm volatile("" : "+v"(im), "+v"(px));
                float* orow = g.out2 + ((size_t)im * g.Kp + nb) * opix + px;
#pragma unroll
                for (int r = 0; r < 4; ++r)
                    if (im >= 0 && nb + r < g.Kp) orow[(size_t)r * opix] = v[r] + b2[r];
            }
        };
        for (int u = 0; u < groups; u += 2) {
            if (u + 1 < groups) ldw(wB, u + 1);
            group(wA, u);
            if (u + 1 < groups) {
                if (u + 2 < groups) ldw(wA, u + 2);
                group(wB, u + 1);
            }
        }
    } else if constexpr (LN_PROD) {
        constexpr int ROWBYTES = C::BN * 4 + 16;
        constexpr int JP = epi_rows_per_pass_ln<C>();
        constexpr int CR = C::NWM * JP * 16;
        constexpr int CPR = C::BN / 8;
        constexpr int NCH = CR * CPR / C::NT;
        constexpr int GR = C::BN / 64;
        static_assert(NCH * C::NT == CR * CPR && CPR % 8 == 0 && C::NT % 8 == 0, "chunks must split evenly over threads");
        static_assert(CR * ROWBYTES + C::BM * GR * 8 <= C::LDS, "row statistics must fit behind the staged rows");
        float* statbuf = (float*)(smem + CR * ROWBYTES);
        uint16_t* out_hi = (uint16_t*)g.out;
        uint16_t* out_lo = out_hi + g.plane;
        const uint16_t* aux_hi = (const uint16_t*)g.aux;
        const uint16_t* aux_lo = aux_hi + g.plane;
        f32x4 bias4[C::TI];
#pragma unroll
        for (int i = 0; i < C::TI; ++i)
            bias4[i] = (EPI == EPI_POS) ? f32x4{0.f, 0.f, 0.f, 0.f} : *(const f32x4*)(g.bias + n0 + wn * C::WN + i * 16 + fg * 4);
        asm volatile("s_waitcnt vmcnt(0)" ::: "memory");
        __syncthreads();
#pragma unroll
        for (int p = 0; p < C::TJ / JP; ++p) {
            size_t orow_q[NCH];
            u32x4 ra[NCH], rb[NCH];
#pragma unroll
            for (int q = 0; q < NCH; ++q) {
                const int c = tid + q * C::NT;
                const int lr = c / CPR, ch = c - lr * CPR;
                const int wmr = lr / (JP * 16), rr = lr - wmr * (JP * 16);
                const int m = m0 + wmr * C::WM + p * JP * 16 + rr;
                const int n = n0 + ch * 8;
                orow_q[q] = (size_t)-1;
                if (m >= g.M || n >= g.N) continue;
                orow_q[q] = (size_t)m * g.ldo;
                if (EPI == EPI_POS) {
                    const float* pr = g.aux + (size_t)(m % 192) * g.ldo + n;
                    ra[q] = *(const u32x4*)pr;
                    rb[q] = *(const u32x4*)(pr + 4);
                } else {
                    ra[q] = *(const u32x4*)(aux_hi + orow_q[q] + n);
                    rb[q] = *(const u32x4*)(aux_lo + orow_q[q] + n);
                }
            }
#pragma unroll
            for (int jj = 0; jj < JP; ++jj) {
                char* lrow = smem + ((wm * JP + jj) * 16 + frow) * ROWBYTES + (wn * C::WN + fg * 4) * 4;
#pragma unroll
                for (int i = 0; i < C::TI; ++i) *(f32x4*)(lrow + i * 64) = acc[i][p * JP + jj] + bias4[i];
            }
            __syncthreads();
#pragma unroll
            for (int q = 0; q < NCH; ++q) {
                const int c = tid + q * C::NT;
                const int lr = c / CPR, ch = c - lr * CPR;
                const bool ok = orow_q[q] != (size_t)-1;
                float v[8];
#pragma unroll
                for (int e = 0; e < 8; ++e) v[e] = 0.f;
                if (ok) {
                    const f32x4 s0 = *(const f32x4*)(smem + lr * ROWBYTES + ch * 32);
                    const f32x4 s1 = *(const f32x4*)(smem + lr * ROWBYTES + ch * 32 + 16);
#pragma unroll
                    for (int e = 0; e < 8; ++e) {
                        const float r = EPI == EPI_POS ? __builtin_bit_cast(float, e < 4 ? ra[q][e] : rb[q][e - 4]) : planes_decode8<T>(ra[q], rb[q], e);
                        v[e] = (e < 4 ? s0[e] : s1[e - 4]) + r;
                    }
                    u32x4 oh, ol;
                    planes_split8<T>(v, oh, ol);
                    if (!(VP_ABLATE(g) & 8)) {
                        *(u32x4*)(out_hi + orow_q[q] + n0 + ch * 8) = oh;
                        *(u32x4*)(out_lo + orow_q[q] + n0 + ch * 8) = ol;
                    }
                }
                const float2 gs = granule_stats8(v);
                if ((ch & 7) == 0) {
                    const int wmr = lr / (JP * 16), rr = lr - wmr * (JP * 16);
                    const int trow = wmr * C::WM + p * JP * 16 + rr;
                    *(float2*)(statbuf + (trow * GR + (ch >> 3)) * 2) = gs;
                }
            }
            if (p + 1 < C::TJ / JP) __syncthreads();
        }
        __syncthreads();
        for (int t = tid; t < C::BM * GR; t += C::NT) {
            const int trow = t / GR, gi = t - trow * GR;
            const int m = m0 + trow, n = n0 + gi * 64;
            if (m < g.M && n < g.N && !(VP_ABLATE(g) & 8))
                *(float2*)(g.stats_out + ((size_t)m * (g.N / 64) + (n >> 6)) * 2) = *(const float2*)(statbuf + t * 2);
        }
    } else if constexpr (EPI != EPI_HEATMAP) {
        constexpr int ES = (EPI == EPI_BIAS_RESID || EPI == EPI_POS || EPI == EPI_PARTIAL) ? 4 : 2;
        constexpr int ROWBYTES = C::BN * ES + 16;
        constexpr int JP = epi_rows_per_pass<C, ES>();
        constexpr int CR = C::NWM * JP * 16;
        constexpr int CPR = C::BN * ES / 16;
        constexpr int EPC = 16 / ES;
        constexpr int NCH = CR * CPR / C::NT;
        static_assert(NCH * C::NT == CR * CPR, "chunks must split evenly over threads");
        f32x4 bias4[C::TI];
#pragma unroll
        for (int i = 0; i < C::TI; ++i)
            bias4[i] = (EPI == EPI_POS || EPI == EPI_PARTIAL) ? f32x4{0.f, 0.f, 0.f, 0.f} : *(const f32x4*)(g.bias + n0 + wn * C::WN + i * 16 + fg * 4);
        constexpr bool LN_CONSUMER = (EPI == EPI_BIAS || EPI == EPI_BIAS_GELU);
        const bool ln_in = LN_CONSUMER && (g.rowstat != nullptr || g.ln_part != nullptr);
        float ln_mean[LN_CONSUMER ? C::TJ : 1], ln_rstd[LN_CONSUMER ? C::TJ : 1];
        f32x4 ln_s4[LN_CONSUMER ? C::TI : 1];
        if (LN_CONSUMER) {
#pragma unroll
            for (int i = 0; i < C::TI; ++i) ln_s4[i] = f32x4{0.f, 0.f, 0.f, 0.f};
#pragma unroll
            for (int j = 0; j < C::TJ; ++j) { ln_mean[j] = 0.f; ln_rstd[j] = 1.f; }
        }
        if (LN_CONSUMER && ln_in) {
#pragma unroll
            for (int i = 0; i < C::TI; ++i) ln_s4[i] = *(const f32x4*)(g.ln_s + n0 + wn * C::WN + i * 16 + fg * 4);
#pragma unroll
            for (int j = 0; j < C::TJ; ++j) {
                int m = m0 + wm * C::WM + j * 16 + frow;
                if (m > g.M - 1) m = g.M - 1;
                if (g.ln_part) {
                    const float2 s2 = ((const float2*)(smem + C::LDS))[wm * C::WM + j * 16 + frow];
                    ln_mean[j] = s2.x;
                    ln_rstd[j] = s2.y;
                } else {
                    ln_mean[j] = g.rowstat[2 * (size_t)m];
                    ln_rstd[j] = g.rowstat[2 * (size_t)m + 1];
                }
            }
        }
        asm volatile("s_waitcnt vmcnt(0)" ::: "memory");
        __syncthreads();
#pragma unroll
        for (int p = 0; p < C::TJ / JP; ++p) {
            size_t orow_q[NCH];
            f32x4 res[(ES == 4 && EPI != EPI_PARTIAL) ? NCH : 1];
#pragma unroll
            for (int q = 0; q < NCH; ++q) {
                const int c = tid + q * C::NT;
                const int lr = c / CPR, ch = c - lr * CPR;
                const int wmr = lr / (JP * 16), rr = lr - wmr * (JP * 16);
                const int m = m0 + wmr * C::WM + p * JP * 16 + rr;
                const int n = n0 + ch * EPC;
                orow_q[q] = (size_t)-1;
                if (m >= g.M || n >= g.N) continue;
                if (EPI == EPI_DECONV) {
                    const int t = m / g.Win, jx = m - t * g.Win, ii = t % g.Hin, img = t / g.Hin;
                    orow_q[q] = ((size_t)(img * 2 * g.Hin + 2 * ii + (parity >> 1)) * (2 * g.Win) + 2 * jx + (parity & 1)) * (size_t)g.ldo;
                } else {
                    orow_q[q] = (size_t)m * g.ldo;
                }
                if (EPI == EPI_PARTIAL) orow_q[q] += (size_t)split * g.M * g.ldo;
                if (ES == 4 && EPI != EPI_PARTIAL) {
                    const size_t arow = (EPI == EPI_POS) ? (size_t)(m % 192) * g.ldo : orow_q[q];
                    res[q] = *(const f32x4*)(g.aux + arow + n);
                }
            }
#pragma unroll
            for (int jj = 0; jj < JP; ++jj) {
                char* lrow = smem + ((wm * JP + jj) * 16 + frow) * ROWBYTES + (wn * C::WN + fg * 4) * ES;
#pragma unroll
                for (int i = 0; i < C::TI; ++i) {
                    f32x4 v = acc[i][p * JP + jj];
                    if (LN_CONSUMER) {
                        const float mu = ln_mean[p * JP + jj], rs = ln_rstd[p * JP + jj];
#pragma unroll
                        for (int r = 0; r < 4; ++r) v[r] = ln_fold(v[r], mu, ln_s4[i][r], rs, bias4[i][r]);
                    } else {
                        v += bias4[i];
                    }
                    if (EPI == EPI_BIAS_GELU) {
#pragma unroll
                        for (int r = 0; r < 4; ++r) v[r] = gelu_sat<T>(v[r]);
                    }
                    if (EPI == EPI_DECONV) {
#pragma unroll
                        for (int r = 0; r < 4; ++r) v[r] = fmaxf(v[r], 0.f);
                    }
                    if (ES == 2) {
                        u32x2 o;
                        if (EPI == EPI_BIAS_GELU) {
                            o[0] = pack2_nosat<T>(v[0], v[1]);
                            o[1] = pack2_nosat<T>(v[2], v[3]);
                        } else {
                            o[0] = pack2<T>(v[0], v[1]);
                            o[1] = pack2<T>(v[2], v[3]);
                        }
                        *(u32x2*)(lrow + i * 16 * ES) = o;
                    } else {
                        *(f32x4*)(lrow + i * 16 * ES) = v;
                    }
                }
            }
            __syncthreads();
            if (!(VP_ABLATE(g) & 8)) {
#pragma unroll
                for (int q = 0; q < NCH; ++q) {
                    const int c = tid + q * C::NT;
                    const int lr = c / CPR, ch = c - lr * CPR;
                    const int n = n0 + ch * EPC;
                    const char* src = smem + lr * ROWBYTES + ch * 16;
                    if (orow_q[q] == (size_t)-1) continue;
                    if (ES == 2) {
                        const u32x4 v = *(const u32x4*)src;
                        uint16_t* dst = (uint16_t*)g.out + orow_q[q] + n;
                        if (EPI != EPI_DECONV && g.out_blocked) {
                            const int wmr = lr / (JP * 16), rr = lr - wmr * (JP * 16);
                            const int m = m0 + wmr * C::WM + p * JP * 16 + rr;
                            dst = (uint16_t*)g.out + (((size_t)(m >> 6) * (g.ldo >> 6) + (n >> 6)) << 12) + ((m & 63) << 6) + (n & 63);
                        }
                        if (n + 8 <= g.N) *(u32x4*)dst = v;
                        else *(u32x2*)dst = u32x2{v[0], v[1]};
                    } else if (EPI == EPI_PARTIAL) {
                        *(f32x4*)((float*)g.out + orow_q[q] + n) = *(const f32x4*)src;
                    } else {
                        *(f32x4*)((float*)g.out + orow_q[q] + n) = *(const f32x4*)src + res[q];
                    }
                }
            }
            if (p + 1 < C::TJ / JP) __syncthreads();
        }
    } else {
#pragma unroll
        for (int j = 0; j < C::TJ; ++j) {
            const int m = m0 + wm * C::WM + j * 16 + frow;
            if (m >= g.M || (VP_ABLATE(g) & 8)) continue;
            const int img = m / 3072, pix = m - img * 3072;
            const size_t orow = (size_t)img * g.Kp * 3072 + pix;
#pragma unroll
            for (int u = 0; u < C::TI / 2; ++u) {
                const int nb = (n0 + wn * C::WN) / 2 + u * 16 + fg * 4;
                if (nb >= g.Kp) continue;
                const f32x4 v = acc[2 * u][j] + acc[2 * u + 1][j];
#pragma unroll
                for (int r = 0; r < 4; ++r)
                    if (nb + r < g.Kp) ((float*)g.out)[orow + (size_t)(nb + r) * 3072] = v[r] + g.bias[nb + r];
            }
        }
    }
}

template <class T, int EPI, class C>
__global__ __launch_bounds__(C::NT, 2) void gemm_persist_kernel(GemmArgs g) {
    static_assert(C::BK == 64 && C::STAGES == 2 && C::PIPE == 1 && (EPI == EPI_BIAS || EPI == EPI_BIAS_GELU), "persistent variant");
    extern __shared__ __attribute__((aligned(16))) char smem[];
    const int tid = threadIdx.x, lane = tid & 63, wave = __builtin_amdgcn_readfirstlane(tid >> 6);
    const int tiles_n = (g.N + C::BN - 1) / C::BN;
    const int tiles_m = (g.M + C::BM - 1) / C::BM;
    const int ntiles = tiles_m * tiles_n;
    const int K = g.K, nk = K / C::BK;
    const int xcd = blockIdx.x & 7, j0 = blockIdx.x >> 3, nloc = gridDim.x >> 3;
    const int q = ntiles >> 3, r8 = ntiles & 7;
    const int base = (xcd < r8) ? xcd * (q + 1) : r8 * (q + 1) + (xcd - r8) * q;
    const int cnt = q + (xcd < r8 ? 1 : 0);
    if (j0 >= cnt) return;
    auto tile_origin = [&](int t, int& m0, int& n0) {
        const int bid = base + t;
        int tm, tn;
        if (g.group_m > 1) {
            const int per_group = g.group_m * tiles_n;
            const int grp = bid / per_group, first_m = grp * g.group_m;
            const int gsz = min(tiles_m - first_m, g.group_m);
            const int r = bid - grp * per_group;
            tm = first_m + r % gsz;
            tn = r / gsz;
        } else {
            tm = bid / tiles_n;
            tn = bid - tm * tiles_n;
        }
        m0 = tm * C::BM;
        n0 = tn * C::BN;
    };
    static_assert(C::RPG == 8 && C::NWAVES % 2 == 0, "address split assumes 8 rows per piece and an even wave count");
    const int rip = lane >> 3, pslot = lane & 7;
    const int sw = pslot ^ (((wave & 1) << 2) | (rip >> 1));
    const uint32_t voff_w = (uint32_t)(rip * K + sw * 8) * 2u;
    const uint32_t voff_a = g.a_blocked ? (uint32_t)(rip * 64 + sw * 8) * 2u : voff_w;
    const char* wbase = nullptr;
    const char* abase = nullptr;
    auto set_addr = [&](int m0, int n0) {
        wbase = (const char*)(g.W + (size_t)(n0 + wave * 8) * K);
        abase = g.a_blocked ? (const char*)(g.A + ((size_t)(m0 >> 6) * (K >> 6) << 12))
                            : (const char*)(g.A + (size_t)(m0 + wave * 8) * K);
    };
    auto stage = [&](int kt, int buf) {
        char* sbase = smem + buf * C::STAGE_BYTES + wave * 1024;
        const int k0 = kt * C::BK;
#pragma unroll
        for (int p = 0; p < C::WP; ++p)
            glds16(wbase + ((size_t)(p * C::NWAVES * 8) * K + k0) * 2 + voff_w, sbase + p * (C::NWAVES * 1024));
#pragma unroll
        for (int p = 0; p < C::AP; ++p) {
            const char* pa;
            if (g.a_blocked) {
                const int pr = p * C::NWAVES + wave;
                pa = abase + ((((size_t)(pr >> 3) * (K >> 6) + (k0 >> 6)) << 12) + ((pr & 7) << 9)) * 2;
            } else {
                pa = abase + ((size_t)(p * C::NWAVES * 8) * K + k0) * 2;
            }
            glds16(pa + voff_a, sbase + C::W_BYTES + p * (C::NWAVES * 1024));
        }
    };
    const int wn = wave / C::NWM, wm = wave % C::NWM;
    const int frow = lane & 15, fg = lane >> 4;
    const int foff = frow * C::ROWB + (swz<C::BK>(frow, fg) << 4);
    const int woff = wn * C::WN * C::ROWB + foff;
    const int aoff = C::W_BYTES + wm * C::WM * C::ROWB + foff;

    constexpr int ROWBYTES = C::BN * 2 + 16;
    constexpr int JP = [] { int jp = C::TJ; while (jp > 1 && (C::TJ % jp || C::NWM * jp * 16 * ROWBYTES > C::STAGE_BYTES)) --jp; return jp; }();
    constexpr int CR = C::NWM * JP * 16, CPR = C::BN / 8, NCH = CR * CPR / C::NT;
    static_assert(C::TJ % JP == 0 && NCH * C::NT == CR * CPR && CR * ROWBYTES <= C::STAGE_BYTES, "epilogue staging must fit one ring buffer");
    char* cst = smem + C::STAGE_BYTES;
    const bool ln_in = g.rowstat != nullptr;

    int t = j0, m0, n0;
    tile_origin(t, m0, n0);
    set_addr(m0, n0);
    stage(0, 0);
    bool landed = false;
    for (;;) {
        f32x4 acc[C::TI][C::TJ];
#pragma unroll
        for (int i = 0; i < C::TI; ++i)
#pragma unroll
            for (int j = 0; j < C::TJ; ++j) acc[i][j] = f32x4{0.f, 0.f, 0.f, 0.f};
        int nm0 = 0, nn0 = 0;
        bool has_next = false;
        unsigned long long ts0 = 0, ts1 = 0, ks[5] = {0, 0, 0, 0, 0};
        if (VP_ABLATE(g) & 32) ts0 = __builtin_readcyclecounter();
        for (int kt = 0; kt < nk; ++kt) {
            const bool stamp = (VP_ABLATE(g) & 32) && kt == 5;
            if (stamp) ks[0] = __builtin_readcyclecounter();
            if (kt > 0 || !landed) wait_vmcnt<0>();
            __builtin_amdgcn_s_barrier();
            asm volatile("" ::: "memory");
            if (stamp) ks[1] = __builtin_readcyclecounter();
            if (kt + 1 < nk) {
                stage(kt + 1, (kt + 1) & 1);
            } else {
                has_next = t + nloc < cnt;
                if (has_next) {
                    tile_origin(t + nloc, nm0, nn0);
                    set_addr(nm0, nn0);
                    stage(0, 0);
                }
            }
            if (stamp) ks[2] = __builtin_readcyclecounter();
            const char* sb = smem + (kt & 1) * C::STAGE_BYTES;
            u32x4 wf0[C::TI], af0[C::TJ], wf1[C::TI], af1[C::TJ];
#pragma unroll
            for (int i = 0; i < C::TI; ++i) wf0[i] = *(const u32x4*)(sb + (woff + i * 16 * C::ROWB));
#pragma unroll
            for (int j = 0; j < C::TJ; ++j) af0[j] = *(const u32x4*)(sb + (aoff + j * 16 * C::ROWB));
            __builtin_amdgcn_sched_barrier(0);
            __builtin_amdgcn_s_setprio(1);
#pragma unroll
            for (int i = 0; i < C::TI / 2; ++i)
#pragma unroll
                for (int j = 0; j < C::TJ; ++j) acc[i][j] = mfma16<T>(wf0[i], af0[j], acc[i][j]);
            __builtin_amdgcn_sched_barrier(0);
            if (stamp) ks[3] = __builtin_readcyclecounter();
#pragma unroll
            for (int i = 0; i < C::TI; ++i) wf1[i] = *(const u32x4*)(sb + ((woff + i * 16 * C::ROWB) ^ 64));
#pragma unroll
            for (int j = 0; j < C::TJ; ++j) af1[j] = *(const u32x4*)(sb + ((aoff + j * 16 * C::ROWB) ^ 64));
            __builtin_amdgcn_sched_barrier(0);
#pragma unroll
            for (int i = C::TI / 2; i < C::TI; ++i)
#pragma unroll
                for (int j = 0; j < C::TJ; ++j) acc[i][j] = mfma16<T>(wf0[i], af0[j], acc[i][j]);
            __builtin_amdgcn_sched_barrier(0);
#pragma unroll
            for (int i = 0; i < C::TI; ++i)
#pragma unroll
                for (int j = 0; j < C::TJ; ++j) acc[i][j] = mfma16<T>(wf1[i], af1[j], acc[i][j]);
            __builtin_amdgcn_s_setprio(0);
            if (stamp) ks[4] = __builtin_readcyclecounter();
        }

        if (VP_ABLATE(g) & 32) ts1 = __builtin_readcyclecounter();
        f32x4 bias4[C::TI], ln_s4[C::TI];
        float ln_mean[C::TJ], ln_rstd[C::TJ];
#pragma unroll
        for (int i = 0; i < C::TI; ++i) bias4[i] = (VP_ABLATE(g) & 64) ? f32x4{0.f, 0.f, 0.f, 0.f} : *(const f32x4*)(g.bias + n0 + wn * C::WN + i * 16 + fg * 4);
#pragma unroll
        for (int i = 0; i < C::TI; ++i) ln_s4[i] = f32x4{0.f, 0.f, 0.f, 0.f};
#pragma unroll
        for (int j = 0; j < C::TJ; ++j) { ln_mean[j] = 0.f; ln_rstd[j] = 1.f; }
        if (ln_in) {
#pragma unroll
            for (int i = 0; i < C::TI; ++i) ln_s4[i] = *(const f32x4*)(g.ln_s + n0 + wn * C::WN + i * 16 + fg * 4);
#pragma unroll
            for (int j = 0; j < C::TJ; ++j) {
                int m = m0 + wm * C::WM + j * 16 + frow;
                if (m > g.M - 1) m = g.M - 1;
                ln_mean[j] = g.rowstat[2 * (size_t)m];
                ln_rstd[j] = g.rowstat[2 * (size_t)m + 1];
            }
        }
        __syncthreads();
#pragma unroll
        for (int p = 0; p < C::TJ / JP; ++p) {
#pragma unroll
            for (int jj = 0; jj < JP; ++jj) {
                char* lrow = cst + ((wm * JP + jj) * 16 + frow) * ROWBYTES + (wn * C::WN + fg * 4) * 2;
#pragma unroll
                for (int i = 0; i < C::TI; ++i) {
                    f32x4 v = acc[i][p * JP + jj];
                    {
                        const float mu = ln_mean[p * JP + jj], rs = ln_rstd[p * JP + jj];
#pragma unroll
                        for (int r = 0; r < 4; ++r) v[r] = ln_fold(v[r], mu, ln_s4[i][r], rs, bias4[i][r]);
                    }
                    u32x2 o;
                    if (EPI == EPI_BIAS_GELU) {
#pragma unroll
                        for (int r = 0; r < 4; ++r) v[r] = gelu_sat<T>(v[r]);
                        o[0] = pack2_nosat<T>(v[0], v[1]);
                        o[1] = pack2_nosat<T>(v[2], v[3]);
                    } else {
                        o[0] = pack2<T>(v[0], v[1]);
                        o[1] = pack2<T>(v[2], v[3]);
                    }
                    *(u32x2*)(lrow + i * 32) = o;
                }
            }
            if (p == 0) wait_vmcnt<0>();
            __syncthreads();
#pragma unroll
            for (int qq = 0; qq < NCH; ++qq) {
                const int c = tid + qq * C::NT;
                const int lr = c / CPR, ch = c - lr * CPR;
                const int wmr = lr / (JP * 16), rr = lr - wmr * (JP * 16);
                const int m = m0 + wmr * C::WM + p * JP * 16 + rr;
                const int n = n0 + ch * 8;
                if (m >= g.M || n >= g.N) continue;
                const u32x4 v = *(const u32x4*)(cst + lr * ROWBYTES + ch * 16);
                uint16_t* dst = g.out_blocked
                    ? (uint16_t*)g.out + (((size_t)(m >> 6) * (g.ldo >> 6) + (n >> 6)) << 12) + ((m & 63) << 6) + (n & 63)
                    : (uint16_t*)g.out + (size_t)m * g.ldo + n;
                *(u32x4*)dst = v;
            }
            if (p + 1 < C::TJ / JP) __syncthreads();
        }
        if ((VP_ABLATE(g) & 32) && tid == 0) {
            unsigned long long* st = (unsigned long long*)g.stats_out + ((size_t)blockIdx.x * 32 + (t - j0) / nloc) * 8;
            st[0] = ts0; st[1] = ts1; st[2] = __builtin_readcyclecounter();
#pragma unroll
            for (int e = 0; e < 5; ++e) st[3 + e] = ks[e];
        }
        if (!has_next) break;
        t += nloc;
        m0 = nm0;
        n0 = nn0;
        landed = true;
    }
}

template <class T, int EPI, class C>
static hipError_t launch_persist(const GemmArgs& a, hipStream_t s) {
    auto kern = gemm_persist_kernel<T, EPI, C>;
    static bool attr_done[64] = {};
    if (hipError_t e = lds_opt_in((const void*)kern, C::LDS, attr_done); e != hipSuccess) return e;
    const int tiles = ((a.M + C::BM - 1) / C::BM) * ((a.N + C::BN - 1) / C::BN);
    const int resident = 256 * (160 * 1024 / C::LDS);
    int grid = tiles < resident ? tiles : resident;
    grid &= ~7;
    if (grid < 8) return hipErrorInvalidValue;
    if (a.desc)
        snprintf(a.desc, a.desc_cap, "gemm_persist_kernel<%s, %d, TileCfg<%d, %d, %d, %d, %d, %d, %d>>", std::is_same<T, F16>::value ? "F16" : "BF16", EPI,
                 C::BM, C::BN, C::BK, C::WM, C::WN, C::STAGES, C::PIPE);
    hipLaunchKernelGGL(kern, dim3(grid), dim3(C::NT), C::LDS, s, a);
    return hipGetLastError();
}

template <int I>
using CfgAt = TileCfg<TILES[I].BM, TILES[I].BN, TILES[I].BK, TILES[I].WM, TILES[I].WN, TILES[I].STAGES, TILES[I].PIPE>;
constexpr int tile_index(int id) { return (int)(find_tile(id) - TILES); }
using Cfg3 = CfgAt<tile_index(3)>;
using Cfg8 = CfgAt<tile_index(8)>;
template <int... I>
constexpr bool table_matches_kernels(std::integer_sequence<int, I...>) {
    return ((tile_ring_bytes(TILES[I]) == CfgAt<I>::LDS && tile_threads(TILES[I]) == CfgAt<I>::NT) && ...);
}
static_assert(table_matches_kernels(std::make_integer_sequence<int, NUM_TILES>{}), "tiles.h: ring bytes / thread count differ from TileCfg");

template <class T, int EPI, int AMODE, class C>
static hipError_t launch(const GemmArgs& a, hipStream_t s) {
    auto kern = gemm_kernel<T, EPI, AMODE, C>;
    int ex = 0;
    if constexpr (EPI == EPI_BIAS_RESID || EPI == EPI_BIAS_RESID_LN)
        if (a.expert) { kern = gemm_kernel<T, EPI, AMODE, C, true>; ex = 1; }
    constexpr int LDS_BYTES = (EPI == EPI_DECONV_FINAL && C::BM * (C::BN * 2 + 16) > C::LDS) ? C::BM * (C::BN * 2 + 16) : C::LDS;
    constexpr int LN_STAT_BYTES = C::BM * 8;
    static_assert(LDS_BYTES + LN_STAT_BYTES <= 160 * 1024, "LDS");
    if (C::PIPE == 6 && a.K % 128 != 0) return hipErrorInvalidValue;
    if (a.ln_part && (a.ln_tiles & 1)) return hipErrorInvalidValue;
    static bool attr_done[2][64] = {};
    if (hipError_t e = lds_opt_in((const void*)kern, LDS_BYTES + LN_STAT_BYTES, attr_done[ex]); e != hipSuccess) return e;
    GemmArgs g = a;
    const int tiles_n = (a.N + C::BN - 1) / C::BN;
    g.w_parity_stride = (size_t)a.w_rows * a.K;
    if ((size_t)tiles_n * C::BN > (size_t)a.w_rows) return hipErrorInvalidValue;
    const int tiles = ((a.M + C::BM - 1) / C::BM) * tiles_n;
    if constexpr (EPI == EPI_PARTIAL) {
        if (a.splitk < 1 || a.K % (a.splitk * C::BK * (C::PIPE == 6 ? 2 : 1)) != 0 || a.ldo != a.N || a.N % 4 != 0) return hipErrorInvalidValue;
    }
    dim3 grid(AMODE == A_DECONV && a.parity_fast ? tiles * 4 : (EPI == EPI_PARTIAL ? tiles * a.splitk : tiles), AMODE == A_DECONV && !a.parity_fast ? 4 : 1);
    if (a.desc)
        snprintf(a.desc, a.desc_cap, "gemm_kernel<%s, %d, %d, TileCfg<%d, %d, %d, %d, %d, %d, %d>%s>", std::is_same<T, F16>::value ? "F16" : "BF16", EPI,
                 AMODE, C::BM, C::BN, C::BK, C::WM, C::WN, C::STAGES, C::PIPE, ex ? ", true" : "");
    hipLaunchKernelGGL(kern, grid, dim3(C::NT), LDS_BYTES + (a.ln_part ? LN_STAT_BYTES : 0), s, g);
    return hipGetLastError();
}

#ifdef VP_TOOLS
constexpr bool ALL_TILES = true;
#else
constexpr bool ALL_TILES = false;
#endif
template <class T, int EPI, int AMODE, int I>
static bool launch_row(const GemmArgs& a, hipStream_t s, hipError_t& e) {
    constexpr bool instantiated = EPI == EPI_PARTIAL ? TILES[I].partial : (TILES[I].product || ALL_TILES);
    if constexpr (instantiated)
        if (a.variant == TILES[I].id) { e = launch<T, EPI, AMODE, CfgAt<I>>(a, s); return true; }
    return false;
}
template <class T, int EPI, int AMODE, int... I>
static hipError_t by_variant(const GemmArgs& a, hipStream_t s, std::integer_sequence<int, I...>) {
    hipError_t e = hipErrorInvalidValue;
    (void)(... || launch_row<T, EPI, AMODE, I>(a, s, e));
    return e;
}
template <class T, int EPI, int AMODE>
static hipError_t by_variant(const GemmArgs& a, hipStream_t s) {
    return by_variant<T, EPI, AMODE>(a, s, std::make_integer_sequence<int, NUM_TILES>{});
}

template <class T>
static hipError_t dispatch(int epi, const GemmArgs& a, hipStream_t s) {
    switch (epi) {
        case EPI_BIAS: return by_variant<T, EPI_BIAS, A_DENSE>(a, s);
        case EPI_BIAS_GELU: return by_variant<T, EPI_BIAS_GELU, A_DENSE>(a, s);
        case EPI_BIAS_RESID: return by_variant<T, EPI_BIAS_RESID, A_DENSE>(a, s);
        case EPI_POS: return by_variant<T, EPI_POS, A_DENSE>(a, s);
        case EPI_DECONV: return by_variant<T, EPI_DECONV, A_DECONV>(a, s);
        case EPI_HEATMAP: return by_variant<T, EPI_HEATMAP, A_DENSE>(a, s);
        case EPI_BIAS_RESID_LN: return by_variant<T, EPI_BIAS_RESID_LN, A_DENSE>(a, s);
        case EPI_POS_LN: return by_variant<T, EPI_POS_LN, A_DENSE>(a, s);
        case EPI_PARTIAL: return by_variant<T, EPI_PARTIAL, A_DENSE>(a, s);
        case EPI_DECONV_FINAL:
            if (a.variant != 3 || a.N != Cfg3::BN || !a.W2 || !a.bias2 || !a.out2 || a.Kp <= 0) return hipErrorInvalidValue;
            return launch<T, EPI_DECONV_FINAL, A_DECONV, Cfg3>(a, s);
    }
    return hipErrorInvalidValue;
}

hipError_t gemm_launch(int dtype, int epi, const GemmArgs& a, hipStream_t s) {
    if (a.K % 64 != 0 || a.M <= 0 || a.N <= 0) return hipErrorInvalidValue;
    if (a.expert && ((epi != EPI_BIAS_RESID && epi != EPI_BIAS_RESID_LN) || a.persist || a.M % 192)) return hipErrorInvalidValue;
    if (const Tile8Row* t8 = find_tile8(a.variant)) {
        if (a.ln_part && (epi == EPI_BIAS || epi == EPI_BIAS_GELU)) return hipErrorInvalidValue;
#ifdef VP_TOOLS
        static const int stagger_env = [] { const char* e = getenv("VP_G8_STAGGER"); return e ? atoi(e) : -1; }();
        if (stagger_env >= 0) {
            GemmArgs b = a;
            b.stagger = stagger_env;
            return gemm8_launch(dtype, epi, b, t8->BN, s, t8->BM);
        }
#endif
        return gemm8_launch(dtype, epi, a, t8->BN, s, t8->BM);
    }
    if (a.persist) {
        if ((epi != EPI_BIAS && epi != EPI_BIAS_GELU) || a.variant != 8 || a.ln_part || a.K % 128 || a.N % 8 || a.ldo != a.N || a.reverse ||
            a.M % Cfg8::BM || (size_t)a.M * a.K * 2 >= (1ull << 32) ||
            (size_t)((a.N + Cfg8::BN - 1) / Cfg8::BN) * Cfg8::BN > (size_t)a.w_rows)
            return hipErrorInvalidValue;
        if (dtype == DT_F16)
            return epi == EPI_BIAS ? launch_persist<F16, EPI_BIAS, Cfg8>(a, s) : launch_persist<F16, EPI_BIAS_GELU, Cfg8>(a, s);
        return epi == EPI_BIAS ? launch_persist<BF16, EPI_BIAS, Cfg8>(a, s) : launch_persist<BF16, EPI_BIAS_GELU, Cfg8>(a, s);
    }
    if (a.a_blocked && (epi == EPI_DECONV || epi == EPI_DECONV_FINAL || (a.M & 63))) return hipErrorInvalidValue;
    if (a.out_blocked && ((epi != EPI_BIAS && epi != EPI_BIAS_GELU) || (a.M & 63) || (a.N & 63) || a.ldo != a.N)) return hipErrorInvalidValue;
    if ((epi == EPI_BIAS_RESID_LN || epi == EPI_POS_LN) && (a.N % 64 != 0 || !a.plane || !a.stats_out)) return hipErrorInvalidValue;
    return dtype == DT_F16 ? dispatch<F16>(epi, a, s) : dispatch<BF16>(epi, a, s);
}

}
```

### easy_vitpose_amd/csrc/handle.hip

```cpp
#include "api_internal.h"

using namespace vpi;

namespace vpi {

thread_local std::string g_create_error;

int fail(vp_ctx* c, int code, const std::string& msg) {
    if (c) c->err = msg; else g_create_error = msg;
    return code;
}

int need_weights(vp_ctx* c) {
    if (!c) return VP_ERR_INVALID;
    return c->loaded ? (int)VP_OK : fail(c, VP_ERR_STATE, "weights not loaded: call vp_load_weights first");
}

bool slots_busy(const vp_ctx* c) { return c->slots[0].busy || c->slots[1].busy; }

int slots_idle(vp_ctx* c, const char* who) {
    return slots_busy(c) ? fail(c, VP_ERR_STATE, std::string(who) + " with a vp_infer_submit in flight: call vp_infer_wait first") : (int)VP_OK;
}

int quiesce(vp_ctx* c) {
    if (c->foreign_pending && c->ev_sw) HIPCHK(c, hipEventSynchronize(c->ev_sw));
    if (c->stream) HIPCHK(c, hipStreamSynchronize(c->stream));
    return VP_OK;
}

bool prof_begin(vp_ctx* c, int fam, double flops, double bytes) {
    if (!((c->prof >> fam) & 1u)) return false;
    std::pair<hipEvent_t, hipEvent_t> p;
    if (!c->ev_pool.empty()) {
        p = c->ev_pool.back();
        c->ev_pool.pop_back();
    } else {
        hipEventCreate(&p.first);
        hipEventCreate(&p.second);
    }
    hipEventRecord(p.first, c->stream);
    c->evs.push_back({p.first, p.second, fam, flops, bytes});
    return true;
}
void prof_end(vp_ctx* c, bool on) {
    if (on) hipEventRecord(c->evs.back().b, c->stream);
}
void prof_collect(vp_ctx* c) {
    for (auto& e : c->evs) {
        float ms = 0.f;
        if (hipEventElapsedTime(&ms, e.a, e.b) == hipSuccess) {
            c->acc.ms[e.fam] += ms;
            c->acc.flops[e.fam] += e.flops;
            c->acc.bytes[e.fam] += e.bytes;
            c->acc.launches[e.fam] += 1;
        }
        c->ev_pool.push_back({e.a, e.b});
    }
    c->evs.clear();
}

void apply_gemm_tuning(Switches& s) {
#ifndef VP_TOOLS
    (void)s;
#else
    if (const char* t = getenv("VP_GEMM_TUNE")) {
        int f, v, gm, used = 0;
        while (sscanf(t, "%d:%d:%d%n", &f, &v, &gm, &used) == 3) {
            if (f >= 0 && f < VP_PROF_COUNT) { s.gemm_variant[f] = v; s.gemm_group_m[f] = gm; }
            t += used;
            if (*t == ',') ++t; else break;
        }
    }
#endif
}

void read_switches(Switches& s) {
    auto on = [](const char* name, bool& dst) { if (const char* f = getenv(name)) dst = atoi(f) != 0; };
    auto num = [](const char* name, auto& dst) { if (const char* f = getenv(name)) dst = atol(f); };
    on("VP_FUSE_LN", s.fuse_ln);
    on("VP_PERSIST", s.persist_gemm);
    if (const char* f = getenv("VP_GRAPH")) s.graph_max_n = atoi(f) == 1 ? 16 : atoi(f);
    on("VP_GRAPH_NULL", s.graph_null);
    if (const char* f = getenv("VP_CALLER_STREAM")) s.caller_stream_max_n = atoi(f) == 1 ? 16 : atoi(f);
    on("VP_FUSE_HEAD", s.fuse_head);
    if (const char* f = getenv("VP_FOLD_STATS")) { s.graph_max_n_stats = atoi(f); s.fold_rule = false; }
    on("VP_BLOCKED_QKV", s.blocked_qkv);
    on("VP_FUSE_QKV_ATTN", s.fuse_qkv_attn);
    s.qa_min_set = getenv("VP_QA_MIN_TILES") != nullptr;
    num("VP_QA_MIN_TILES", s.qa_min_tiles);
    num("VP_QA80_MIN_TILES", s.qa80_min_tiles);
    num("VP_QA80_GROUP", s.qa80_group);
    num("VP_ATTN_QSPLIT", s.attn_qsplit);
    on("VP_DECONV_PARITY_FAST", s.deconv_parity_fast);
    on("VP_G8_COST", s.g8_cost_model);
    on("VP_PAD_BATCH", s.pad_batch);
    num("VP_G8_BM192", s.g8_bm192);
    if (const char* f = getenv("VP_SPLITK")) {
        if (!strchr(f, ':')) s.splitk_on = atoi(f) != 0;
        else {
            const char* t = f;
            while (*t) {
                const int which = !strncmp(t, "fc2:", 4) ? 1 : !strncmp(t, "proj:", 5) ? 0 : -1;
                if (which < 0) break;
                t = strchr(t, ':') + 1;
                int S = 0, v = 0, used = 0;
                if (sscanf(t, "%d:%d%n", &S, &v, &used) != 2) break;
                s.splitk_force[which][0] = S; s.splitk_force[which][1] = v;
                t += used;
                if (*t == ',') ++t;
            }
        }
    }
    num("VP_GEMM8", s.gemm8_mask);
    s.fp8_proj16 = getenv("VP_FP8_PROJ16") != nullptr;
#ifdef VP_TOOLS
    num("VP_G8_MIN_TILES", s.g8_min_tiles);
    on("VP_BLOCKED_HID", s.blocked_hid);
    num("VP_ORDER", s.order_mask);
    num("VP_G8_STAGGER", s.g8_stagger);
    if (const char* t = getenv("VP_ABLATE_FAM")) {
        int f, b, used = 0;
        while (sscanf(t, "%d:%d%n", &f, &b, &used) == 2) {
            if (f >= 0 && f < VP_PROF_COUNT) s.fam_ablate[f] = b;
            t += used;
            if (*t == ',') ++t; else break;
        }
    }
#endif
    apply_gemm_tuning(s);
}

int flip_partner_table(int K, const int32_t* pairs, int n_pairs, int32_t* partner, std::string* why) {
    auto bad = [&](const std::string& m) { if (why) *why = m; return VP_ERR_INVALID; };
    if (K <= 0 || !partner) return bad("no joints");
    if (n_pairs < 0) return bad("negative n_pairs");
    if (n_pairs > 0 && !pairs) return bad("null flip_pairs with n_pairs > 0");
    for (int k = 0; k < K; ++k) partner[k] = k;
    for (int i = 0; i < n_pairs; ++i) {
        const int a = pairs[2 * i], b = pairs[2 * i + 1];
        if (a < 0 || b < 0 || a >= K || b >= K)
            return bad("flip pair " + std::to_string(i) + " = (" + std::to_string(a) + ", " + std::to_string(b) + ") outside the head's " + std::to_string(K) + " joints");
        partner[a] = b;
        partner[b] = a;
    }
    return VP_OK;
}

}

extern "C" {

int vp_abi_version(void) { return VP_ABI_VERSION; }

int vp_create(vp_handle* out, const vp_config* cfg) {
    if (!out || !cfg) return fail(nullptr, VP_ERR_INVALID, "null argument");
    *out = nullptr;
    const int D = cfg->embed_dim, h = cfg->num_heads;
    if (D <= 0 || h <= 0 || D % h != 0 || D % 128 != 0 || D > 1280)
        return fail(nullptr, VP_ERR_INVALID, "embed_dim must be a multiple of 128 (<= 1280) and divisible by num_heads");
    const int hd = D / h;
    if (hd != 32 && hd != 64 && hd != 80) return fail(nullptr, VP_ERR_INVALID, "head_dim must be 32, 64 or 80");
    if (cfg->depth <= 0 || cfg->num_keypoints <= 0 || cfg->num_keypoints > 1024 || cfg->max_batch <= 0)
        return fail(nullptr, VP_ERR_INVALID, "depth, num_keypoints and max_batch must be positive");
    if (cfg->dtype != VP_DTYPE_F16 && cfg->dtype != VP_DTYPE_BF16 && cfg->dtype != VP_DTYPE_FP8) return fail(nullptr, VP_ERR_INVALID, "unknown dtype");
    if (cfg->dtype == VP_DTYPE_FP8 && (D % 256 != 0 || D < 768))
        return fail(nullptr, VP_ERR_INVALID, "the fp8 mode needs embed_dim >= 768 and a multiple of 256 (K-tiles of 128, an even number of them; >= 8 tiles per GEMM at the smallest batch): ViTPose-B / -L / -H");
    int ndev = 0;
    hipError_t e = hipGetDeviceCount(&ndev);
    if (e != hipSuccess || ndev <= 0)
        return fail(nullptr, VP_ERR_HIP, std::string("no HIP device available (this library has no CPU fallback): ") +
                                             (e != hipSuccess ? hipGetErrorString(e) : "device count 0"));
    if (cfg->device_id < 0 || cfg->device_id >= ndev) return fail(nullptr, VP_ERR_INVALID, "device_id out of range");
    vp_ctx* c = new vp_ctx();
    c->cfg = *cfg;
    c->D = D; c->L = cfg->depth; c->heads = h; c->Kp = cfg->num_keypoints; c->Kmax = c->Kp;
    c->dtype = cfg->dtype == VP_DTYPE_BF16 ? vp::DT_BF16 : vp::DT_F16;
    c->fp8 = cfg->dtype == VP_DTYPE_FP8;
    c->maxb = cfg->max_batch;
    read_switches(c->sw);
    auto bail = [&](int rc) { g_create_error = c->err; vp_destroy(c); return rc; };
    if ((e = hipSetDevice(cfg->device_id)) != hipSuccess) { c->err = hipGetErrorString(e); return bail(VP_ERR_HIP); }
    if ((e = hipStreamCreateWithFlags(&c->stream, hipStreamNonBlocking)) != hipSuccess) { c->err = hipGetErrorString(e); return bail(VP_ERR_HIP); }
    c->own_stream = c->stream;
    const size_t B = (size_t)((c->maxb + 3) / 4 * 4);
    c->Mp = std::max<size_t>((B * 192 + 255) / 256 * 256, 512);
    const size_t M = c->fp8 ? c->Mp : B * 192;
    int rc = 0;
    void* stage = nullptr;
    if ((rc = dalloc(c, (char**)&stage, B * crop_bytes(VP_INPUT_F32_NCHW)))) return bail(rc);
    c->in_stage = stage;
    if ((rc = dalloc(c, &c->wh_stage, B * 2))) return bail(rc);
    if ((rc = dalloc(c, &c->x, M * D))) return bail(rc);
    if ((rc = dalloc(c, &c->y, M * D))) return bail(rc);
    if (c->fp8 && !c->sw.fuse_ln) { c->err = "the fp8 mode is built on the fused-LayerNorm path (unset VP_FUSE_LN)"; return bail(VP_ERR_INVALID); }
    if (c->sw.fuse_ln) {
        if ((rc = dalloc(c, &c->ln_part, M * (size_t)(D / 64) * 2))) return bail(rc);
        if ((rc = dalloc(c, &c->rowstat, M * 2))) return bail(rc);
    }
    if (c->fp8) {
        if ((rc = dalloc(c, &c->x8, M * D)) || (rc = dalloc(c, &c->xs8, M * (size_t)(D / 32))) || (rc = dalloc(c, &c->hs8, M * (size_t)(4 * D / 32)))) return bail(rc);
        if (hipMemset(c->x, 0, M * D * 4) != hipSuccess) { c->err = "hipMemset"; return bail(VP_ERR_HIP); }
        if (hd == 64 && !c->sw.fp8_proj16) {
            if ((rc = dalloc(c, &c->y8, M * D)) || (rc = dalloc(c, &c->ys8, M * (size_t)(D / 32)))) return bail(rc);
            if (hipMemset(c->y8, 0, M * D) != hipSuccess || hipMemset(c->ys8, 0, M * (size_t)(D / 32)) != hipSuccess) { c->err = "hipMemset"; return bail(VP_ERR_HIP); }
        }
    }
    if ((rc = dalloc(c, &c->qkv, M * 3 * D))) return bail(rc);
    if ((rc = dalloc(c, &c->hid, M * 4 * D))) return bail(rc);
    if ((rc = dalloc(c, &c->d1, B * 768 * 256))) return bail(rc);
    if ((rc = dalloc(c, &c->d2, B * 3072 * 256))) return bail(rc);
    if ((rc = dalloc(c, &c->hm, B * c->Kp * 3072))) return bail(rc);
    if ((rc = dalloc(c, &c->kp, B * c->Kp * 3))) return bail(rc);
    if (c->sw.fuse_ln && !c->fp8 && c->sw.splitk_on) {
        c->splitk_rows = (size_t)std::min<int>(c->maxb, SPLITK_MAX_CROPS) * 192;
        if ((rc = dalloc(c, &c->splitk_ws, (size_t)SPLITK_MAX_S * c->splitk_rows * D))) return bail(rc);
    }
    if ((rc = dalloc(c, &c->zero, (size_t)256))) return bail(rc);
    if ((rc = dalloc(c, (char**)&c->draw_ws, (size_t)VP_DRAW_MAX_RECORDS * 48))) return bail(rc);
    if (hipMemset(c->zero, 0, 512) != hipSuccess) { c->err = "hipMemset"; return bail(VP_ERR_HIP); }
    *out = c;
    return VP_OK;
}

void* vp_host_alloc(size_t bytes) {
    void* p = nullptr;
    if (hipHostMalloc(&p, bytes ? bytes : 1, hipHostMallocDefault) != hipSuccess) return nullptr;
    return p;
}
void vp_host_free(void* p) { if (p) hipHostFree(p); }

int vp_set_flip_test(vp_handle c, const int32_t* flip_pairs, int32_t n_pairs, int32_t shift_heatmap) {
    int rc = need_weights(c);
    if (rc) return rc;
    std::vector<int32_t> partner((size_t)c->Kmax);
    std::string why;
    if (flip_partner_table(c->Kp, flip_pairs, n_pairs, partner.data(), &why)) return fail(c, VP_ERR_INVALID, "vp_set_flip_test: " + why);
    for (int k = c->Kp; k < c->Kmax; ++k) partner[k] = k;
// ... 165 lines not shown
```

### easy_vitpose_amd/csrc/kernels.h

```cpp
#pragma once
#include <hip/hip_runtime.h>
#include <stdint.h>

#ifdef VP_TOOLS
#define VP_ABLATE(g) ((g).ablate)
#define VP_STAGGER(g) ((g).stagger)
namespace vp {
hipError_t peak_bench(int kind, double* result);
hipError_t hwid_probe_launch(uint32_t* d_out, int blocks, int threads, int lds_bytes, int spin, hipStream_t s);
}
#else
#define VP_ABLATE(g) 0
#define VP_STAGGER(g) 0
#endif

namespace vp {

enum { DT_F16 = 0, DT_BF16 = 1 };

inline hipError_t lds_opt_in(const void* kern, int bytes, bool (&done)[64]) {
    int dev = 0;
    (void)hipGetDevice(&dev);
    const bool known = dev >= 0 && dev < 64;
    if (known && done[dev]) return hipSuccess;
    const hipError_t e = hipFuncSetAttribute(kern, hipFuncAttributeMaxDynamicSharedMemorySize, bytes);
    if (e == hipSuccess && known) done[dev] = true;
    return e;
}

enum GemmEpi {
    EPI_BIAS = 0,
    EPI_BIAS_GELU = 1,
    EPI_BIAS_RESID = 2,
    EPI_POS = 3,
    EPI_DECONV = 4,
    EPI_HEATMAP = 5,
    EPI_BIAS_RESID_LN = 6,
    EPI_POS_LN = 7,
    EPI_DECONV_FINAL = 8,
    EPI_QKV_ATTN = 9,
    EPI_PARTIAL = 10,
};
enum GemmAMode { A_DENSE = 0, A_DECONV = 1 };

struct GemmArgs {
    const uint16_t* A;
    const uint16_t* W;
    const float* bias;
    void* out;
    const float* aux;
    int M, N, K, ldo;
    int Hin, Win, Cin;
    const uint16_t* zero;
    int Kp;
    const uint16_t* W2;
    const float* bias2;
    float* out2;
    int w_rows;
    int variant;
    int group_m;
    size_t w_parity_stride;
    size_t plane;
    float* stats_out;
    const float* rowstat;
    const float* ln_s;
    const float* ln_part;
    int ln_tiles;
    float ln_inv_d;
    int a_blocked, out_blocked;
    int reverse;
    int persist;
    int stagger;
    int ablate;
    char* desc;
    int desc_cap;
    float attn_scale_log2e;
    int splitk;
    int parity_fast;
    union {
        const uint8_t* a_scales;
        const int32_t* expert;
    };
    const float* w_scale;
    uint8_t* out_scales;
};
hipError_t gemm_launch(int dtype, int epi, const GemmArgs& a, hipStream_t s);
bool gemm8_supported(int epi, const GemmArgs& a, int bn, int bm = 256);
bool gemm8_shape_ok(int epi, int M, int N, int K, int ldo, int w_rows, int bn, int bm);
hipError_t gemm8_launch(int dtype, int epi, const GemmArgs& a, int bn, hipStream_t s, int bm = 256);

bool gemm8f_supported(int epi, const GemmArgs& a, int bn);
hipError_t gemm8f_launch(int epi, const GemmArgs& a, int bn, hipStream_t s);
hipError_t ln_quant_launch(int dtype, const uint16_t* x_hi, const float* ln_part, int tiles, uint8_t* codes, uint8_t* scales, int M, int Mp, int D,
                           hipStream_t s);
hipError_t mx_quantize_launch(const float* src, uint8_t* codes, uint8_t* scales, int M, int K, hipStream_t s);

hipError_t fill_random16(int dtype, uint16_t* p, size_t n, uint32_t seed, hipStream_t s);

hipError_t ln_finalize_launch(const float* partials, float* rowstat, int M, int tiles, int D, hipStream_t s);
hipError_t splitk_reduce_launch(int dtype, const float* partials, int S, const float* bias, uint16_t* x_hi, size_t plane, float* stats_out, int M, int N,
                                hipStream_t s);

hipError_t fp8_probe_launch(const float* dA, const float* dW, const float* dAs, const float* dWs, uint8_t* dA8, uint8_t* dW8, float* dOut,
                            int M, int N, int K, hipStream_t s);

hipError_t mx_probe_launch(const float* dA, const float* dW, const float* dWs, uint8_t* dA8, uint8_t* dAs, uint8_t* dW8, float* dOut,
                           int M, int N, int K, hipStream_t s);

hipError_t attention_launch(int dtype, const uint16_t* qkv, uint16_t* out, int B, int D, int heads, hipStream_t s, bool qsplit, int qkv_blocked = 0,
                            uint8_t* mx_scales = nullptr);
inline float softmax_scale_log2e(int head_dim) { return (1.0f / sqrtf((float)head_dim)) * 1.4426950408889634f; }

struct QkvAttnArgs {
    const uint16_t* x_hi;
    const uint16_t* wh;
    const float* bh;
    const float* sh;
    const float* rowstat;
    uint16_t* y;
    int npairs, heads, D;
    int ncrops;
    float scale_log2e;
    int ablate;
};
bool qkvattn_supported(const QkvAttnArgs& a);
hipError_t qkvattn_launch(int dtype, const QkvAttnArgs& a, hipStream_t s, char* desc, int desc_cap);
hipError_t qkv_head_major_launch(const uint16_t* w, const float* b, const float* s, uint16_t* wh, float* bh, float* sh, int D, int K, hipStream_t st);
hipError_t qkv_head_major80_launch(const uint16_t* w, const float* b, const float* s, uint16_t* wh, float* bh, float* sh, int D, int K, int heads, hipStream_t st);

hipError_t layernorm_launch(int dtype, const float* x, const float* gamma, const float* beta,
                            uint16_t* out16, float* out32, int M, int D, hipStream_t s, size_t plane = 0);
hipError_t im2col_launch(int dtype, const void* crops, int input_format, uint16_t* out, int B, hipStream_t s, bool flip = false, int n_src = 0);
hipError_t gather_crops_launch(const void* src, void* dst, const int32_t* idx, int n, size_t crop_bytes, hipStream_t s);
hipError_t flip_merge_launch(float* hm, const float* hm_flipped, const int32_t* partner, int N, int K, int shift, hipStream_t s, int interleaved = 0);
hipError_t im2col_twin_launch(int dtype, const void* crops, int input_format, uint16_t* out, int B, int n_src, hipStream_t s);
void flip_twin_layout(int bo, int n_src, int* src, int* mirror);

struct CropRec {
    const uint8_t* src;
    int64_t pitch;
    int32_t cw, ch, left, top, pw, ph;
    const uint8_t* src1;
    int64_t pitch1;
    int32_t format, matrix, oy, ox;
};
hipError_t crop_resize_launch(const CropRec* recs, uint8_t* out, int n, hipStream_t s);

constexpr int BOX_FRAMES_PER_LAUNCH = 64;
struct BoxFrame {
    const uint8_t* plane[2];
    int64_t pitch[2];
    int32_t h, w, format, matrix;
};
struct BoxFrames {
    BoxFrame fr[BOX_FRAMES_PER_LAUNCH];
    int32_t f0, count, n_frames;
};
hipError_t box_geometry_launch(const BoxFrames& fr, const float* xyxy, int row_stride, const int32_t* frame_idx, int n, int pad, const uint8_t* zero_px,
                               CropRec* recs, int32_t* wh, int32_t* aux, int32_t* p9_out, int32_t* status_out, hipStream_t s, const int32_t* slot = nullptr);

struct AffRec {
    const uint8_t* plane[2];
    int64_t pitch[2];
    double ax, bx, ay, by;
    int32_t w, y0, y1, format, matrix, pad_;
};
hipError_t crop_affine_launch(const AffRec* recs, uint8_t* out, int n, hipStream_t s);
hipError_t box_cs_launch(const BoxFrames& fr, const float* xyxy, int row_stride, const int32_t* frame_idx, int n, float box_scale, AffRec* recs, float* cs,
                         float* cs_out, int32_t* status_out, hipStream_t s);

hipError_t decode_launch(const float* hm, const int32_t* org_wh, float* out, int N, int K, hipStream_t s);
hipError_t decode_flip_launch(const float* hm, const int32_t* partner, int shift, const int32_t* org_wh, float* out, int N, int K, hipStream_t s);

hipError_t decode_affine_launch(const float* hm, const float* cs, float* out, int N, int K, hipStream_t s);
hipError_t decode_affine_flip_launch(const float* hm, const int32_t* partner, int shift, const float* cs, float* out, int N, int K, hipStream_t s);

struct MixRec {
    int32_t first, K, dst;
};
hipError_t decode_mix_launch(const float* hm, const MixRec* recs, const int32_t* org_wh, float* out, int N, int Kmax, hipStream_t s);
struct MixRecFlip {
    int32_t first, K, dst, e;
};
hipError_t decode_flip_mix_launch(const float* hm, const MixRecFlip* recs, const int32_t* partners, int shift, const int32_t* org_wh, float* out, int N, int Kmax,
                                  hipStream_t s);
hipError_t box_offsets_launch(const int32_t* aux, float* out, int n, int K, hipStream_t s, const int32_t* slot = nullptr, const MixRec* recs = nullptr);

constexpr int MIX_CROPS_PER_LAUNCH = 128;
struct MixTable {
    int32_t id[MIX_CROPS_PER_LAUNCH], order[MIX_CROPS_PER_LAUNCH], first[MIX_CROPS_PER_LAUNCH], K[MIX_CROPS_PER_LAUNCH];
    int32_t base, count, pad_to;
};
hipError_t mix_tables_launch(const MixTable& t, int32_t* ids, int32_t* order, int32_t* slot, MixRec* recs, hipStream_t s);
hipError_t mix_tables_flip_launch(const MixTable& t, int32_t* ids, int32_t* order, int32_t* slot, MixRec* recs, MixRecFlip* recs_flip, hipStream_t s);

}
```

### easy_vitpose_amd/csrc/tools_taps.hip

```cpp
#include "dbg_util.h"

using namespace vpi;

namespace {
struct RandCase {
    vp::GemmArgs g{};
    size_t out_bytes = 0, stats_floats = 0;
    void* out[2] = {nullptr, nullptr};
    float* stats[2] = {nullptr, nullptr};
};
int make_rand_case(vp_ctx* c, RandCase& rc, int epi, int flags, int M, int N, int K, int nout) {
    uint16_t *dA, *dW, *dAux16 = nullptr;
    float *dB, *dAux32 = nullptr, *dRow = nullptr, *dS = nullptr;
    int r;
    const size_t MN = (size_t)M * N, wrows = pad128(N);
    if ((r = dalloc(c, &dA, (size_t)M * K)) || (r = dalloc(c, &dW, wrows * K)) || (r = dalloc(c, &c->zero, (size_t)256))) return r;
    vp::fill_random16(c->dtype, dA, (size_t)M * K, 1u, nullptr);
    vp::fill_random16(c->dtype, dW, wrows * K, 2u, nullptr);
    if (flags & 64) { HIPCHK(c, hipMemset(dA, 0, (size_t)M * K * 2)); HIPCHK(c, hipMemset(dW, 0, wrows * K * 2)); }
    if (flags & 128) { HIPCHK(c, hipMemsetD16(dA, 0x3c00, (size_t)M * K)); HIPCHK(c, hipMemsetD16(dW, 0x3c00, wrows * K)); }
    std::vector<float> hb(wrows), hs(wrows), hr((size_t)M * 2);
    uint32_t lcg = 12345u;
    auto rnd = [&]() { lcg = lcg * 1664525u + 1013904223u; return (float)((lcg >> 8) & 0xffff) / 65536.f - 0.5f; };
    for (auto& v : hb) v = rnd();
// ... 59 lines not shown
    vp::fill_random16(c->dtype, dx, M * D, 1u, nullptr);
    vp::fill_random16(c->dtype, dwh, 3 * (size_t)D * D, 2u, nullptr);
    hipMemset(dbh, 0, 3 * (size_t)D * 4); hipMemset(dsh, 0, 3 * (size_t)D * 4); hipMemset(drow, 0, 2 * M * 4);
    vp::QkvAttnArgs qa{};
    qa.x_hi = dx; qa.wh = dwh; qa.bh = dbh; qa.sh = dsh; qa.rowstat = drow; qa.y = dy; qa.npairs = npairs; qa.ncrops = 2 * npairs; qa.heads = heads; qa.D = D; qa.ablate = ablate;
    qa.scale_log2e = vp::softmax_scale_log2e(64);
    vp::GemmArgs g80{};
    const bool h80 = heads * 80 == D;
    g80.A = dx; g80.W = dwh; g80.bias = dbh; g80.ln_s = dsh; g80.rowstat = drow; g80.out = dy;
    g80.M = (int)M; g80.N = heads * 256; g80.K = D; g80.ldo = D; g80.w_rows = heads * 256; g80.variant = 18; g80.ablate = ablate;
    g80.attn_scale_log2e = vp::softmax_scale_log2e(80);
    auto launch = [&]() { return h80 ? vp::gemm_launch(c->dtype, vp::EPI_QKV_ATTN, g80, nullptr) : vp::qkvattn_launch(c->dtype, qa, nullptr, nullptr, 0); };
    hipEvent_t e0, e1;
    hipEventCreate(&e0); hipEventCreate(&e1);
    hipError_t e = hipSuccess;
    for (int i = 0; i < 2 && e == hipSuccess; ++i) e = launch();
    hipDeviceSynchronize();
    hipEventRecord(e0, nullptr);
    for (int i = 0; i < iters && e == hipSuccess; ++i) e = launch();
    hipEventRecord(e1, nullptr);
    if (e == hipSuccess) e = hipDeviceSynchronize();
    float ms = 0.f;
    hipEventElapsedTime(&ms, e0, e1);
    *ms_out = ms / iters;
    hipEventDestroy(e0); hipEventDestroy(e1);
    if (e != hipSuccess) return dbg_finish(c, fail(c, VP_ERR_HIP, std::string("qkvattn bench: ") + hipGetErrorString(e)));
    return dbg_finish(c, VP_OK);
}

VP_API int vp_dbg_gemm_timeline(int32_t device, int32_t dtype, int32_t epi, int32_t M, int32_t N, int32_t K, uint64_t* stamps,
                                int32_t max_wg) {
    if ((epi != 0 && epi != 1) || !stamps) return fail(nullptr, VP_ERR_INVALID, "bad timeline request");
    vp_ctx* c = dbg_ctx(device, dtype);
    if (!c) return VP_ERR_HIP;
    uint16_t *dA, *dW, *dO;
    float* dB;
    unsigned long long* dS;
    int rc;
    const size_t wrows = pad128(N), nst = (size_t)max_wg * 32 * 8;
    if ((rc = dalloc(c, &dA, (size_t)M * K)) || (rc = dalloc(c, &dW, wrows * K)) || (rc = dalloc(c, &dB, wrows)) ||
        (rc = dalloc(c, &dO, (size_t)M * N)) || (rc = dalloc(c, &dS, nst)) || (rc = dalloc(c, &c->zero, (size_t)256)))
        return dbg_finish(c, rc);
    vp::fill_random16(c->dtype, dA, (size_t)M * K, 1u, nullptr);
    vp::fill_random16(c->dtype, dW, wrows * K, 2u, nullptr);
    hipMemset(dB, 0, wrows * 4);
    hipMemset(dS, 0, nst * 8);
    vp::GemmArgs g{};
    g.A = dA; g.W = dW; g.bias = dB; g.out = dO; g.M = M; g.N = N; g.K = K; g.ldo = N; g.zero = c->zero;
    g.w_rows = (int)wrows; g.variant = 8; g.group_m = 8; g.persist = 1;
    hipError_t e = vp::gemm_launch(c->dtype, epi, g, nullptr);
    g.ablate = 32 | (getenv("VP_TL_ABL") ? atoi(getenv("VP_TL_ABL")) : 0); g.stats_out = (float*)dS;
    if (e == hipSuccess) e = vp::gemm_launch(c->dtype, epi, g, nullptr);
    if (e == hipSuccess) e = hipDeviceSynchronize();
    if (e == hipSuccess) e = hipMemcpy(stamps, dS, nst * 8, hipMemcpyDeviceToHost);
    if (e != hipSuccess) return dbg_finish(c, fail(c, VP_ERR_HIP, std::string("timeline: ") + hipGetErrorString(e)));
    return dbg_finish(c, VP_OK);
}

VP_API int vp_dbg_gemm_bench(int32_t device, int32_t dtype, int32_t epi, int32_t variant, int32_t group_m, int32_t M,
                             int32_t N, int32_t K, int32_t iters, float* ms_out) {
    if (epi < 0 || epi > 3 || M <= 0 || N <= 0 || K <= 0 || K % 64 || iters <= 0 || !ms_out)
        return fail(nullptr, VP_ERR_INVALID, "bad gemm bench shape");
    vp_ctx* c = dbg_ctx(device, dtype);
    if (!c) return VP_ERR_HIP;
    uint16_t *dA, *dW, *dO16 = nullptr;
    float *dB, *dAux = nullptr, *dO32 = nullptr;
    int rc;
    const size_t MN = (size_t)M * N, wrows = pad128(N);
    if ((rc = dalloc(c, &dA, (size_t)M * K)) || (rc = dalloc(c, &dW, wrows * K)) || (rc = dalloc(c, &dB, wrows)) ||
        (rc = dalloc(c, &c->zero, (size_t)256)))
        return dbg_finish(c, rc);
    if (epi >= 2) { if ((rc = dalloc(c, &dO32, MN)) || (rc = dalloc(c, &dAux, (size_t)192 * N))) return dbg_finish(c, rc); }
    else if ((rc = dalloc(c, &dO16, MN))) return dbg_finish(c, rc);
    vp::fill_random16(c->dtype, dA, (size_t)M * K, 1u, nullptr);
    vp::fill_random16(c->dtype, dW, wrows * K, 2u, nullptr);
    hipMemset(dB, 0, wrows * 4);
    if (dO32) hipMemset(dO32, 0, MN * 4);
    if (dAux) hipMemset(dAux, 0, (size_t)192 * N * 4);
    c->sw.gemm_variant[0] = variant & 0xff;
    c->sw.gemm_group_m[0] = group_m;
    c->gemm_ablate = variant >> 8;
    hipEvent_t e0, e1;
    hipEventCreate(&e0); hipEventCreate(&e1);
    void* outp = epi >= 2 ? (void*)dO32 : (void*)dO16;
    const float* aux = epi == 2 ? dO32 : dAux;
    const GemmPick pk = resolve_gemm(c->sw, 0, epi, M, N, K);
    for (int i = 0; i < 2 && !rc; ++i) rc = gemm(c, 0, epi, pk, dA, dW, dB, outp, aux, M, N, K, N);
    hipDeviceSynchronize();
    hipEventRecord(e0, nullptr);
    for (int i = 0; i < iters && !rc; ++i) rc = gemm(c, 0, epi, pk, dA, dW, dB, outp, aux, M, N, K, N);
    hipEventRecord(e1, nullptr);
    if (!rc && hipDeviceSynchronize() != hipSuccess) rc = fail(c, VP_ERR_HIP, "gemm bench kernel failed");
    float ms = 0.f;
    hipEventElapsedTime(&ms, e0, e1);
    *ms_out = ms / iters;
    hipEventDestroy(e0); hipEventDestroy(e1);
    return dbg_finish(c, rc);
}

VP_API int vp_dbg_gemm_bench2(int32_t device, int32_t dtype, int32_t epi, int32_t variant, int32_t group_m, int32_t flags, int32_t M,
                              int32_t N, int32_t K, int32_t iters, float* ms_out) {
    if (M <= 0 || N <= 0 || K <= 0 || K % 64 || iters <= 0 || !ms_out) return fail(nullptr, VP_ERR_INVALID, "bad gemm bench shape");
    vp_ctx* c = dbg_ctx(device, dtype);
    if (!c) return VP_ERR_HIP;
    RandCase rc;
    int r = make_rand_case(c, rc, epi, flags, M, N, K, 1);
    if (r) return dbg_finish(c, r);
    vp::GemmArgs g = rc.g;
    g.variant = variant & 0xff; g.group_m = group_m; g.ablate = variant >> 8;
    g.out = rc.out[0]; g.stats_out = rc.stats[0];
    hipEvent_t e0, e1;
    hipEventCreate(&e0); hipEventCreate(&e1);
    hipError_t e = hipSuccess;
    for (int i = 0; i < 2 && e == hipSuccess; ++i) e = vp::gemm_launch(c->dtype, epi, g, nullptr);
    hipDeviceSynchronize();
    hipEventRecord(e0, nullptr);
    for (int i = 0; i < iters && e == hipSuccess; ++i) e = vp::gemm_launch(c->dtype, epi, g, nullptr);
    hipEventRecord(e1, nullptr);
    if (e == hipSuccess) e = hipDeviceSynchronize();
    float ms = 0.f;
    hipEventElapsedTime(&ms, e0, e1);
    *ms_out = ms / iters;
    hipEventDestroy(e0); hipEventDestroy(e1);
    if (e != hipSuccess) return dbg_finish(c, fail(c, VP_ERR_HIP, std::string("gemm bench2: ") + hipGetErrorString(e)));
    return dbg_finish(c, VP_OK);
}

VP_API int vp_dbg_gemm8_timeline(int32_t device, int32_t dtype, int32_t epi, int32_t variant, int32_t flags, int32_t ablate, int32_t M,
                                 int32_t N, int32_t K, uint64_t* stamps, int32_t max_wg) {
    if ((epi != 0 && epi != 1 && epi != vp::EPI_BIAS_RESID_LN) || !stamps || max_wg < 256) return fail(nullptr, VP_ERR_INVALID, "bad timeline request");
    vp_ctx* c = dbg_ctx(device, dtype);
    if (!c) return VP_ERR_HIP;
    RandCase rc;
    int r = make_rand_case(c, rc, epi, flags, M, N, K, 1);
    if (r) return dbg_finish(c, r);
    unsigned long long* dS;
    const size_t nst = (size_t)max_wg * 2 * 16 * 8;
    if ((r = dalloc(c, &dS, nst))) return dbg_finish(c, r);
    hipMemset(dS, 0, nst * 8);
    vp::GemmArgs g = rc.g;
    g.variant = variant; g.group_m = 8; g.out = rc.out[0];
    if (epi == vp::EPI_BIAS_RESID_LN) g.stats_out = rc.stats[0];
    hipError_t e = vp::gemm_launch(c->dtype, epi, g, nullptr);
    g.ablate = 32 | ablate;
    if (epi == vp::EPI_BIAS_RESID_LN) { g.stats_out = rc.stats[0]; g.ln_part = (const float*)dS; }
    else g.stats_out = (float*)dS;
    if (e == hipSuccess) e = vp::gemm_launch(c->dtype, epi, g, nullptr);
    if (e == hipSuccess) e = hipDeviceSynchronize();
    if (e == hipSuccess) e = hipMemcpy(stamps, dS, nst * 8, hipMemcpyDeviceToHost);
    if (e != hipSuccess) return dbg_finish(c, fail(c, VP_ERR_HIP, std::string("gemm8 timeline: ") + hipGetErrorString(e)));
    return dbg_finish(c, VP_OK);
}

VP_API int vp_dbg_gemm_compare(int32_t device, int32_t dtype, int32_t epi, int32_t variant_a, int32_t group_a, int32_t flags_a,
                               int32_t variant_b, int32_t group_b, int32_t flags_b, int32_t M, int32_t N, int32_t K, int32_t reps,
                               uint64_t* n_mismatch, double* max_abs_diff) {
    if (M <= 0 || N <= 0 || K <= 0 || K % 64 || reps <= 0 || !n_mismatch || !max_abs_diff) return fail(nullptr, VP_ERR_INVALID, "bad gemm compare shape");
    if ((flags_a & (2 | 4 | 16)) != (flags_b & (2 | 4 | 16))) return fail(nullptr, VP_ERR_INVALID, "layout / fold flags must agree");
    vp_ctx* c = dbg_ctx(device, dtype);
    if (!c) return VP_ERR_HIP;
    RandCase rc;
    int r = make_rand_case(c, rc, epi, flags_a, M, N, K, 2);
    if (r) return dbg_finish(c, r);
    *n_mismatch = 0; *max_abs_diff = 0.0;
    std::vector<uint16_t> ha(rc.out_bytes / 2), hb2(rc.out_bytes / 2);
    std::vector<float> sa(rc.stats_floats), sb(rc.stats_floats);
    for (int rep = 0; rep < reps; ++rep) {
        for (int w = 0; w < 2; ++w) {
            vp::GemmArgs g = rc.g;
            const int fl = w ? flags_b : flags_a;
            g.variant = w ? variant_b : variant_a; g.group_m = w ? group_b : group_a;
            g.persist = (fl & 1) != 0; g.reverse = (fl & 8) != 0;
            g.out = rc.out[w]; g.stats_out = rc.stats[w];
            hipMemsetAsync(rc.out[w], 0xff, rc.out_bytes, nullptr);
            hipError_t e = vp::gemm_launch(c->dtype, epi, g, nullptr);
            if (e != hipSuccess) return dbg_finish(c, fail(c, VP_ERR_HIP, std::string("gemm compare launch ") + (w ? "B: " : "A: ") + hipGetErrorString(e)));
        }
        hipError_t e = hipDeviceSynchronize();
        if (e == hipSuccess) e = hipMemcpy(ha.data(), rc.out[0], rc.out_bytes, hipMemcpyDeviceToHost);
        if (e == hipSuccess) e = hipMemcpy(hb2.data(), rc.out[1], rc.out_bytes, hipMemcpyDeviceToHost);
        if (e == hipSuccess && rc.stats_floats) e = hipMemcpy(sa.data(), rc.stats[0], rc.stats_floats * 4, hipMemcpyDeviceToHost);
        if (e == hipSuccess && rc.stats_floats) e = hipMemcpy(sb.data(), rc.stats[1], rc.stats_floats * 4, hipMemcpyDeviceToHost);
        if (e != hipSuccess) return dbg_finish(c, fail(c, VP_ERR_HIP, std::string("gemm compare: ") + hipGetErrorString(e)));
        const bool f32out = (epi == vp::EPI_BIAS_RESID || epi == vp::EPI_POS);
        if (f32out) {
            const float* fa = (const float*)ha.data(); const float* fb = (const float*)hb2.data();
            for (size_t i = 0; i < rc.out_bytes / 4; ++i)
                if (std::memcmp(&fa[i], &fb[i], 4)) { ++*n_mismatch; const double d = std::fabs((double)fa[i] - (double)fb[i]); if (!(d <= *max_abs_diff)) *max_abs_diff = d; }
        } else {
            for (size_t i = 0; i < ha.size(); ++i)
                if (ha[i] != hb2[i]) {
                    ++*n_mismatch;
                    const double d = std::fabs((double)host_from_bits(ha[i], c->dtype) - (double)host_from_bits(hb2[i], c->dtype));
                    if (!(d <= *max_abs_diff)) *max_abs_diff = d;
                }
        }
        for (size_t i = 0; i < sa.size(); ++i)
            if (std::memcmp(&sa[i], &sb[i], 4)) { ++*n_mismatch; const double d = std::fabs((double)sa[i] - (double)sb[i]); if (!(d <= *max_abs_diff)) *max_abs_diff = d; }
    }
    return dbg_finish(c, VP_OK);
}

VP_API int vp_dbg_hwid_probe(int32_t device, int32_t blocks, int32_t threads, int32_t lds_bytes, int32_t spin, uint32_t* out) {
    if (!out || blocks <= 0 || blocks > 65536 || threads <= 0 || threads > 1024 || lds_bytes < 16 || lds_bytes > 160 * 1024 || spin < 0) return fail(nullptr, VP_ERR_INVALID, "bad argument");
    if (hipSetDevice(device) != hipSuccess) return fail(nullptr, VP_ERR_HIP, "no HIP device");
    uint32_t* d = nullptr;
    if (hipMalloc((void**)&d, (size_t)blocks * 16) != hipSuccess) return fail(nullptr, VP_ERR_HIP, "hipMalloc");
    hipError_t e = vp::hwid_probe_launch(d, blocks, threads, lds_bytes, spin, nullptr);
    if (e == hipSuccess) e = hipDeviceSynchronize();
    if (e == hipSuccess) e = hipMemcpy(out, d, (size_t)blocks * 16, hipMemcpyDeviceToHost);
    hipFree(d);
    return e == hipSuccess ? VP_OK : fail(nullptr, VP_ERR_HIP, hipGetErrorString(e));
}

VP_API int vp_dbg_peak(int32_t device, int32_t kind, double* result) {
    const bool known = (kind >= 0 && kind <= 12) || (kind >= 100 && kind < 164) || (kind >= 170 && kind < 178) || (kind >= 200 && kind < 248) ||
                       (kind >= 300 && kind < 492) || (kind >= 500 && kind < 504);
    if (!result || !known) return fail(nullptr, VP_ERR_INVALID, "bad argument");
    if (hipSetDevice(device) != hipSuccess) return fail(nullptr, VP_ERR_HIP, "no HIP device");
    hipError_t e = vp::peak_bench(kind, result);
    return e == hipSuccess ? VP_OK : fail(nullptr, VP_ERR_HIP, hipGetErrorString(e));
}

}
```

### include/vitpose_hip.h

```cpp
#ifndef VITPOSE_HIP_H
#define VITPOSE_HIP_H

#include <stddef.h>
#include <stdint.h>

#ifdef __cplusplus
extern "C" {
#endif

#define VP_ABI_VERSION 4
#define VP_API __attribute__((visibility("default")))

enum {
    VP_OK = 0,
    VP_ERR_INVALID = 1,
    VP_ERR_HIP = 2,
    VP_ERR_STATE = 3,
    VP_ERR_MISSING_TENSOR = 4,
    VP_ERR_SHAPE = 5
};

enum {
    VP_DTYPE_F16 = 0,
    VP_DTYPE_BF16 = 1,
// ... 106 lines not shown
VP_API int vp_dbg_flip_layout(int32_t n, int32_t rows, int32_t* src, int32_t* mirror);
VP_API int vp_dbg_decode_flip(int32_t device_id, const float* heatmaps2, int32_t n, int32_t k, const int32_t* flip_pairs, int32_t n_pairs,
                              int32_t shift_heatmap, const int32_t* org_wh, float* out);

VP_API int vp_infer_heatmaps(vp_handle h, const void* crops, int32_t input_format, int32_t n, float* heatmaps);
VP_API int vp_infer_tokens(vp_handle h, const void* crops, int32_t input_format, int32_t n, float* tokens);

VP_API int vp_expert_info(vp_handle h, int32_t* n_experts, int32_t* part_features, int32_t* k_per_expert);
VP_API int vp_set_expert(vp_handle h, int32_t e);
VP_API int vp_infer_experts(vp_handle h, const void* crops, int32_t input_format, int32_t n, const int32_t* expert_ids,
                            const int32_t* org_wh, float* out);

#define VP_HAS_EXPERT_ENTRIES 1
VP_API int vp_infer_experts_device_stream(vp_handle h, const void* d_crops, int32_t input_format, int32_t n, const int32_t* expert_ids,
                                          const int32_t* d_org_wh, float* d_out, void* caller_stream);
VP_API int vp_infer_frames_experts(vp_handle h, const vp_frame* frames, int32_t n_frames, int32_t frames_on_device, const int32_t* crop_params,
                                   int32_t n, const int32_t* expert_ids, float* out);
VP_API int vp_infer_boxes_experts_stream(vp_handle h, const vp_frame* frames, int32_t n_frames, const float* d_xyxy, int32_t row_stride,
                                         const int32_t* d_frame_idx, int32_t n, int32_t pad, const int32_t* expert_ids, float* d_out,
                                         int32_t* d_crop_params, int32_t* d_status, void* caller_stream);
#define VP_HAS_IMAGE_ENTRIES 1
#define VP_PIX_RGB24 0
#define VP_PIX_BGR24 1
#define VP_PIX_NV12  2
#define VP_YUV_BT601      0
#define VP_YUV_BT709      1
#define VP_YUV_BT601_FULL 2
typedef struct vp_image {
    const uint8_t* plane[2];
    int64_t pitch[2];
    int32_t h, w;
    int32_t format;
    int32_t matrix;
} vp_image;
VP_API int vp_infer_images(vp_handle h, const vp_image* images, int32_t n_images, int32_t images_on_device, const int32_t* crop_params, int32_t n,
                           const int32_t* expert_ids, float* out);
VP_API int vp_infer_boxes_images_stream(vp_handle h, const vp_image* images, int32_t n_images, const float* d_xyxy, int32_t row_stride,
                                        const int32_t* d_frame_idx, int32_t n, int32_t pad, const int32_t* expert_ids, float* d_out,
                                        int32_t* d_crop_params, int32_t* d_status, void* caller_stream);
VP_API int vp_dbg_image_plan(const vp_image* images, int32_t n_images, const int32_t* params9, int32_t n, int32_t* bands);
VP_API int vp_dbg_crop_prep_image(int32_t device_id, const vp_image* image, const int32_t* crop_params, int32_t n, uint8_t* out);

#define VP_HAS_AFFINE_CROP 1
VP_API int vp_infer_images_affine(vp_handle h, const vp_image* images, int32_t n_images, int32_t images_on_device, const int32_t* frame_idx, const float* cs,
                                  int32_t n, float* out);
VP_API int vp_infer_boxes_affine_stream(vp_handle h, const vp_image* images, int32_t n_images, const float* d_xyxy, int32_t row_stride,
                                        const int32_t* d_frame_idx, int32_t n, float box_scale, float* d_out, float* d_cs, int32_t* d_status,
                                        void* caller_stream);
VP_API int vp_dbg_box_cs(const float* xyxy, int32_t row_stride, const int32_t* frame_idx, int32_t n_frames, int32_t n, float box_scale, float* cs, int32_t* status);
VP_API int vp_dbg_affine_plan(const vp_image* images, int32_t n_images, const int32_t* frame_idx, const float* cs, int32_t n, int32_t* bands);
VP_API int vp_dbg_crop_affine(int32_t device_id, const vp_image* image, const float* cs, int32_t n, uint8_t* out);
VP_API int vp_dbg_decode_affine(int32_t device_id, const float* heatmaps, int32_t n, int32_t k, const float* cs, float* out);
VP_API int vp_dbg_decode_affine_flip(int32_t device_id, const float* heatmaps2, int32_t n, int32_t k, const int32_t* flip_pairs, int32_t n_pairs,
                                     int32_t shift_heatmap, const float* cs, float* out);

#define VP_HAS_POSE_NMS 1
#define VP_NMS_MAX_PER_FRAME 1024
#define VP_NMS_MAX_K 256
typedef struct vp_pose_nms_cfg {
    float oks_thr;
    float vis_thr;
    int32_t use_vis_thr;
    int32_t soft;
    int32_t max_dets;
    int32_t n_sigmas;
    const float* sigmas;
} vp_pose_nms_cfg;
VP_API int vp_pose_nms_stream(vp_handle h, const float* d_kpts, int32_t n, int32_t k, const float* d_box_score, int32_t score_stride,
                              const int32_t* d_crop_params, const int32_t* d_status, int32_t n_frames, const vp_pose_nms_cfg* cfg, float* d_score,
                              int32_t* d_rank, int32_t* d_count, void* caller_stream);
VP_API int vp_pose_nms(vp_handle h, const float* kpts, int32_t n, int32_t k, const float* box_score, int32_t score_stride, const int32_t* crop_params,
                       const int32_t* status, int32_t n_frames, const vp_pose_nms_cfg* cfg, float* score, int32_t* rank, int32_t* count);
VP_API int vp_dbg_pose_nms_host(const float* kpts, int32_t n, int32_t k, const float* box_score, int32_t score_stride, const int32_t* crop_params,
                                const int32_t* status, int32_t n_frames, const vp_pose_nms_cfg* cfg, float* score, int32_t* rank, int32_t* count);
VP_API int vp_dbg_pose_oks(int32_t device_id, const float* kpts, int32_t n, int32_t k, const int32_t* crop_params, const vp_pose_nms_cfg* cfg, float* oks);

#define VP_HAS_DRAW 1
#define VP_DRAW_MAX_LIMBS  256
#define VP_DRAW_MAX_COLORS 32
#define VP_DRAW_MAX_RECORDS 65536
typedef struct vp_draw_cfg {
    float   conf_thr;
    int32_t radius, thickness;
    int32_t n_limbs;  const uint8_t* limbs;
    int32_t n_point_colors; const uint8_t* point_colors;
    int32_t n_limb_colors;  const uint8_t* limb_colors;
} vp_draw_cfg;
VP_API int vp_draw_poses_stream(vp_handle h, const vp_image* images, int32_t n_images, const float* d_kpts, int32_t n, int32_t k, const int32_t* d_frame_idx,
                                int32_t frame_stride, const int32_t* d_rank, const int32_t* d_ids, const float* d_boxes, int32_t box_stride,
                                const vp_draw_cfg* cfg, void* caller_stream);
VP_API int vp_draw_poses(vp_handle h, const vp_image* images, int32_t n_images, const float* kpts, int32_t n, int32_t k, const int32_t* frame_idx,
                         int32_t frame_stride, const int32_t* rank, const int32_t* ids, const float* boxes, int32_t box_stride, const vp_draw_cfg* cfg);
VP_API int vp_dbg_draw_host(const vp_image* images, int32_t n_images, const float* kpts, int32_t n, int32_t k, const int32_t* frame_idx, int32_t frame_stride,
                            const int32_t* rank, const int32_t* ids, const float* boxes, int32_t box_stride, const vp_draw_cfg* cfg);

#define VP_HAS_TRACKER 1
#define VP_TRACK_MAX 128
#define VP_TRACK_MAX_STREAMS 64
typedef struct vp_track_cfg {
    int32_t max_age, min_hits;
    float   iou_threshold;
    int32_t n_streams;
} vp_track_cfg;
typedef struct vp_tracker* vp_tracker_handle;
VP_API int vp_tracker_create(vp_handle h, const vp_track_cfg* cfg, vp_tracker_handle* out);
VP_API int vp_tracker_destroy(vp_tracker_handle t);
VP_API int vp_tracker_reset_stream(vp_tracker_handle t, uint64_t stream_mask, void* caller_stream);
VP_API int vp_tracker_update_stream(vp_tracker_handle t, const float* d_dets, int32_t row_stride, const int32_t* d_frame_idx, int32_t n_dets, uint64_t step_mask,
                                    float* d_rows, int32_t* d_ids, int32_t* d_stream, int32_t n_out, int32_t* d_count, int32_t* d_flags, void* caller_stream);
VP_API int vp_tracker_update(vp_tracker_handle t, const float* dets, int32_t row_stride, const int32_t* frame_idx, int32_t n_dets, uint64_t step_mask, float* rows,
                             int32_t* ids, int32_t* stream, int32_t n_out, int32_t* count, int32_t* flags);
VP_API int vp_tracker_state_bytes(int32_t n_streams, int64_t* bytes);
VP_API int vp_tracker_download_state(vp_tracker_handle t, void* out);
VP_API int vp_dbg_track_host(void* state, const vp_track_cfg* cfg, const float* dets, int32_t row_stride, const int32_t* frame_idx, int32_t n_dets, uint64_t step_mask,
                             float* rows, int32_t* ids, int32_t* stream, int32_t n_out, int32_t* count, int32_t* flags);
VP_API int vp_dbg_lsap(int32_t device_id, const double* iou, int32_t nd, int32_t nt, float thr, int32_t* trk_of_det);

VP_API int vp_dbg_mix_plan(const int32_t* expert_ids, int32_t n, int32_t n_experts, int32_t max_batch, const int32_t* k_per_expert, int32_t* order,
                           int32_t* ids_padded, int32_t* counts, int32_t* records, uint64_t* pattern);
VP_API int vp_dbg_decode_mix(int32_t device_id, const float* heatmaps, int32_t n_maps, int32_t n, int32_t kmax, const int32_t* records,
                             const int32_t* org_wh, float* out);
VP_API int vp_dbg_mix_plan_flip(const int32_t* expert_ids, int32_t n, int32_t n_experts, int32_t max_batch, const int32_t* k_per_expert, int32_t* order,
                                int32_t* row_ids, int32_t* counts, int32_t* records, uint64_t* pattern);
VP_API int vp_dbg_decode_flip_mix(int32_t device_id, const float* heatmaps, int32_t n_maps, int32_t n, int32_t kmax, const int32_t* records4,
                                  const int32_t* partners, int32_t n_experts, int32_t shift_heatmap, const int32_t* org_wh, float* out);

VP_API int vp_decode_only(int32_t device_id, const float* heatmaps, int32_t n, int32_t k,
                   const int32_t* org_wh, float* out);

VP_API void* vp_stream(vp_handle h);
VP_API int vp_synchronize(vp_handle h);

VP_API int vp_set_profiling(vp_handle h, int32_t family_mask);
VP_API int vp_reset_profile(vp_handle h);
VP_API int vp_get_profile(vp_handle h, vp_profile* out);
VP_API int vp_profile_kernel(vp_handle h, int32_t family, char* buf, int32_t cap);

VP_API int vp_destroy(vp_handle h);

VP_API const char* vp_last_error(vp_handle h);

VP_API int vp_dbg_gemm(int32_t device_id, int32_t dtype, int32_t epi, int32_t M, int32_t N, int32_t K,
                       const float* A, const float* W, const float* bias, const float* aux, float* out);
VP_API int vp_dbg_attention(int32_t device_id, int32_t dtype, int32_t B, int32_t D, int32_t heads,
                            const float* qkv, float* out);
VP_API int vp_dbg_attention_case(int32_t device_id, int32_t dtype, int32_t B, int32_t D, int32_t heads, int32_t flags, const float* qkv, float* out,
                                 uint8_t* out_scales);
VP_API int vp_dbg_qkvattn(int32_t device_id, int32_t dtype, int32_t npairs, int32_t D, int32_t heads, const float* x, const float* W,
                          const float* bias, float* out);
VP_API int vp_dbg_layernorm(int32_t device_id, int32_t dtype, int32_t M, int32_t D, const float* x,
                            const float* gamma, const float* beta, float* out16, float* out32);
VP_API int vp_dbg_deconv(int32_t device_id, int32_t dtype, int32_t B, int32_t Hin, int32_t Win, int32_t Cin,
                         const float* x, const vp_tensor_desc* tensors, int32_t n_tensors, float* out);
VP_API int vp_dbg_crop_prep(int32_t device_id, const uint8_t* frame, int32_t fh, int32_t fw, const int32_t* crop_params,
                            int32_t n, uint8_t* out);
VP_API int vp_dbg_gemm_case(int32_t device_id, int32_t dtype, int32_t epi, int32_t variant, int32_t group_m, int32_t flags,
                            int32_t M, int32_t N, int32_t K, const float* A, const float* W, const float* bias, const float* aux,
                            const float* rowstat, const float* ln_s, float* out, float* stats);
VP_API int vp_dbg_gemm_case_planes(int32_t device_id, int32_t dtype, int32_t epi, int32_t variant, int32_t group_m, int32_t flags, int32_t M, int32_t N,
                                   int32_t K, const float* A, const float* W, const float* bias, const uint16_t* r_hi, const uint16_t* r_lo,
                                   const float* pos, int32_t in_place, uint16_t* o_hi, uint16_t* o_lo, float* stats);
VP_API int vp_dbg_ln_finalize(int32_t device_id, int32_t M, int32_t tiles, int32_t D, const float* partials, float* rowstat);
VP_API int vp_dbg_gemm_case_lnpart(int32_t device_id, int32_t dtype, int32_t epi, int32_t variant, int32_t group_m, int32_t flags, int32_t M, int32_t N,
                                   int32_t K, const float* A, const float* W, const float* bias, const float* partials, int32_t ln_tiles, const float* ln_s,
                                   float* out);
VP_API int vp_dbg_qkvattn_ln(int32_t device_id, int32_t dtype, int32_t npairs, int32_t D, int32_t heads, const float* x, const float* W, const float* bias,
                             const float* rowstat, const float* ln_s, float* out);
VP_API int vp_dbg_ln_quant(int32_t device_id, int32_t dtype, int32_t M, int32_t Mp, int32_t D, const uint16_t* x_hi, const float* partials, uint8_t* codes,
                           uint8_t* scales);
VP_API int vp_dbg_group_plan(int32_t n, int32_t w, int32_t maxb, int32_t* offs, int32_t* cnts, int32_t cap);
VP_API int vp_dbg_frame_plan(const vp_frame* frames, int32_t n_frames, const int32_t* params9, int32_t n, int32_t* bands);
VP_API int vp_dbg_box_geometry(const float* xyxy, int32_t row_stride, const int32_t* frame_idx, const int32_t* frame_hw, int32_t n_frames,
                               int32_t n, int32_t pad, int32_t* out9, int32_t* status);
VP_API int vp_dbg_gemm8_pick(int32_t M, int32_t N, int32_t wide, int32_t bm192_mask, int32_t* tiles);
VP_API int vp_dbg_gemm2_pick(int32_t epi, int32_t M, int32_t N, int32_t K, int32_t* group_m);
VP_API int vp_dbg_splitk_pick(int32_t M, int32_t N, int32_t K, int32_t* variant);
VP_API int vp_dbg_run_batch(int32_t n, int32_t D, int32_t limit);
VP_API int vp_dbg_expert_tile(int32_t variant, int32_t M, int32_t N, int32_t gemm8_ok, const int32_t* bounds, int32_t n_bounds);
VP_API int vp_dbg_chunk_plan(const vp_config* cfg, int32_t n, int32_t* out, int32_t cap);
VP_API int vp_dbg_group_trace(int32_t n, int32_t w, int32_t maxb, int32_t* trace, int32_t cap);
VP_API int vp_dbg_fp8_gemm(int32_t device_id, int32_t M, int32_t N, int32_t K, const float* A, const float* a_scale, const float* W,
                           const float* w_scale, float* out, uint8_t* a_codes, uint8_t* w_codes);
VP_API int vp_dbg_mx_gemm(int32_t device_id, int32_t M, int32_t N, int32_t K, const float* A, const float* W, const float* w_scale, float* out,
                          uint8_t* a_codes, uint8_t* a_scales, uint8_t* w_codes);
VP_API int vp_dbg_gemm_fp8_case(int32_t device_id, int32_t epi, int32_t M, int32_t N, int32_t K, const float* A, const float* W, const float* bias,
                                const float* aux, float* out, float* stats, float* a_deq, float* w_deq);
VP_API int vp_dbg_gemm_fp8_case_planes(int32_t device_id, int32_t M, int32_t N, int32_t K, const float* A, const float* W, const float* bias,
                                       const uint16_t* r_hi, const uint16_t* r_lo, int32_t in_place, uint16_t* o_hi, uint16_t* o_lo, float* stats,
                                       float* a_deq, float* w_deq);
VP_API int vp_dbg_host_e4m3(const float* in, uint8_t* out, int64_t n);

#ifdef __cplusplus
}
#endif
#endif
```

Baseline: 25510 persons/s.

## Make fused deconv+heatmap head persistent with LDS-resident final weights and tile prefetch

The fused deconv/final-conv head kernel becomes persistent: a fixed grid of workgroups (256 by default, tunable via VP_HEAD_WGS) walks XCD-contiguous tile ranges. Each workgroup stages the final-layer weights and both biases into LDS once, instead of reloading them from global memory on every tile. During the epilogue it also prefetches the next tile's first K-stage, so loads overlap the heatmap computation. The cost is a larger LDS footprint and more complex control flow with goto. The smaller grid may underfill the GPU, and the code depends on subtle vmcnt ordering.

```diff
diff --git a/easy_vitpose_amd/_capi.py b/easy_vitpose_amd/_capi.py
--- a/easy_vitpose_amd/_capi.py
+++ b/easy_vitpose_amd/_capi.py
@@ -20,7 +20,7 @@
            'vp_group_infer_allgather', 'vp_group_destroy', 'vp_group_last_error', 'vp_infer_frame', 'vp_infer_flip', 'vp_infer_heatmaps',
            'vp_infer_tokens', 'vp_decode_only', 'vp_stream', 'vp_synchronize', 'vp_set_profiling',
            'vp_reset_profile', 'vp_get_profile', 'vp_profile_kernel', 'vp_group_peer_access_missing', 'vp_destroy', 'vp_last_error',
-           'vp_dbg_gemm', 'vp_dbg_attention', 'vp_dbg_layernorm', 'vp_dbg_deconv', 'vp_dbg_gemm_case', 'vp_dbg_crop_prep',
+           'vp_dbg_gemm', 'vp_dbg_attention', 'vp_dbg_layernorm', 'vp_dbg_deconv', 'vp_dbg_head_case', 'vp_dbg_gemm_case', 'vp_dbg_crop_prep',
            'vp_dbg_group_plan', 'vp_dbg_group_trace', 'vp_dbg_gemm8_pick', 'vp_dbg_gemm2_pick', 'vp_dbg_splitk_pick', 'vp_dbg_run_batch', 'vp_dbg_fp8_gemm', 'vp_dbg_mx_gemm', 'vp_dbg_host_e4m3', 'vp_dbg_gemm_fp8_case', 'vp_dbg_qkvattn',
            'vp_expert_info', 'vp_set_expert', 'vp_infer_experts', 'vp_dbg_expert_tile', 'vp_infer_frames', 'vp_dbg_frame_plan',
            'vp_dbg_chunk_plan', 'vp_infer_boxes_stream', 'vp_dbg_box_geometry',
@@ -153,6 +153,7 @@
     lib.vp_infer_flip.argtypes = [C.c_void_p, C.c_void_p, C.c_int32, C.c_int32, C.c_void_p, C.c_void_p, C.c_int32, C.c_int32,
                                   C.c_void_p, C.c_void_p]
     lib.vp_dbg_gemm_case.argtypes = [C.c_int32] * 9 + [C.c_void_p] * 8
+    lib.vp_dbg_head_case.argtypes = [C.c_int32] * 5 + [C.c_void_p] * 7
     if hasattr(lib, 'vp_dbg_gemm8_timeline'):
         lib.vp_dbg_gemm8_timeline.argtypes = [C.c_int32] * 9 + [C.POINTER(C.c_uint64), C.c_int32]
         lib.vp_dbg_gemm_timeline.argtypes = [C.c_int32] * 6 + [C.POINTER(C.c_uint64), C.c_int32]
diff --git a/easy_vitpose_amd/csrc/api_internal.h b/easy_vitpose_amd/csrc/api_internal.h
--- a/easy_vitpose_amd/csrc/api_internal.h
+++ b/easy_vitpose_amd/csrc/api_internal.h
@@ -50,6 +50,7 @@
     bool g8_cost_model = true;
     bool deconv_parity_fast = true;
     bool fuse_head = true;
+    int head_wgs = 0;
     bool fp8_proj16 = false;
     int graph_max_n = 16;
     bool graph_null = true;
diff --git a/easy_vitpose_amd/csrc/debug_taps.hip b/easy_vitpose_amd/csrc/debug_taps.hip
--- a/easy_vitpose_amd/csrc/debug_taps.hip
+++ b/easy_vitpose_amd/csrc/debug_taps.hip
@@ -256,6 +256,46 @@
     return dbg_finish(c, rc);
 }
 
+VP_API int vp_dbg_head_case(int32_t device, int32_t dtype, int32_t nh, int32_t Kp, int32_t head_wgs, const float* x, const float* w, const float* b,
+                            const float* wf, const float* bf, float* out_fused, float* out_pair) {
+    if (nh <= 0 || Kp <= 0 || head_wgs < 0 || !x || !w || !b || !wf || !bf || (!out_fused && !out_pair)) return fail(nullptr, VP_ERR_INVALID, "bad head case");
+    vp_ctx* c = dbg_ctx(device, dtype);
+    if (!c) return VP_ERR_HIP;
+    const size_t Min = (size_t)nh * 768, hm_n = (size_t)nh * Kp * 3072;
+    uint16_t *dx, *dw;
+    float *db, *hm;
+    int rc;
+    c->Kp = Kp;
+    c->sw.head_wgs = head_wgs;
+    if ((rc = upload_mat(c, &dx, x, Min, 256, Min)) || (rc = upload_mat(c, &dw, w, (size_t)4 * 256, 1024, (size_t)4 * 256)) || (rc = upload_f32(c, &db, b, 256)) ||
+        (rc = upload_final(c, &c->w_fin, wf, Kp, 256, &c->fin_rows)) || (rc = upload_f32(c, &c->b_fin, bf, Kp, pad128(Kp))) || (rc = dalloc(c, &hm, hm_n)) ||
+        (rc = dalloc(c, &c->zero, (size_t)256)))
+        return dbg_finish(c, rc);
+    if (hipMemset(c->zero, 0, 512) != hipSuccess) return dbg_finish(c, fail(c, VP_ERR_HIP, "memset"));
+    const int M = (int)Min;
+    if (out_fused) {
+        if (hipMemset(hm, 0xff, hm_n * 4) != hipSuccess) return dbg_finish(c, fail(c, VP_ERR_HIP, "memset"));
+        rc = gemm(c, VP_PROF_GEMM_DECONV, vp::EPI_DECONV_FINAL, resolve_gemm(c->sw, VP_PROF_GEMM_DECONV, vp::EPI_DECONV_FINAL, M, 256, 1024), dx, dw, db, hm, nullptr, M, 256,
+                  1024, 256, 32, 24, 256);
+        if (!rc && hipDeviceSynchronize() != hipSuccess) rc = fail(c, VP_ERR_HIP, "fused head kernel failed");
+        if (!rc && hipMemcpy(out_fused, hm, hm_n * 4, hipMemcpyDeviceToHost) != hipSuccess) rc = fail(c, VP_ERR_HIP, "D2H");
+        if (rc) return dbg_finish(c, rc);
+    }
+    if (out_pair) {
+        uint16_t* d2;
+        if ((rc = dalloc(c, &d2, Min * 4 * 256))) return dbg_finish(c, rc);
+        if (hipMemset(hm, 0xff, hm_n * 4) != hipSuccess) return dbg_finish(c, fail(c, VP_ERR_HIP, "memset"));
+        rc = gemm(c, VP_PROF_GEMM_DECONV, vp::EPI_DECONV, resolve_gemm(c->sw, VP_PROF_GEMM_DECONV, vp::EPI_DECONV, M, 256, 1024), dx, dw, db, d2, nullptr, M, 256, 1024, 256, 32, 24,
+                  256);
+        if (!rc)
+            rc = gemm(c, VP_PROF_GEMM_FINAL, vp::EPI_HEATMAP, resolve_gemm(c->sw, VP_PROF_GEMM_FINAL, vp::EPI_HEATMAP, nh * 3072, (int)c->fin_rows, 256), d2, c->w_fin, c->b_fin,
+                      hm, nullptr, nh * 3072, (int)c->fin_rows, 256, 0);
+        if (!rc && hipDeviceSynchronize() != hipSuccess) rc = fail(c, VP_ERR_HIP, "head kernels failed");
+        if (!rc && hipMemcpy(out_pair, hm, hm_n * 4, hipMemcpyDeviceToHost) != hipSuccess) rc = fail(c, VP_ERR_HIP, "D2H");
+    }
+    return dbg_finish(c, rc);
+}
+
 
 static int gemm_case(int32_t device, int32_t dtype, int32_t epi, int32_t variant, int32_t group_m, int32_t flags, int32_t M, int32_t N, int32_t K, const float* A,
                      const float* W, const float* bias, const float* aux, const float* rowstat, const float* ln_s, float* out, float* stats, const PlaneIO* io,
diff --git a/easy_vitpose_amd/csrc/forward.hip b/easy_vitpose_amd/csrc/forward.hip
--- a/easy_vitpose_amd/csrc/forward.hip
+++ b/easy_vitpose_amd/csrc/forward.hip
@@ -26,7 +26,7 @@
         g.ln_part = ln->ln_part; g.ln_tiles = ln->ln_tiles; g.ln_inv_d = 1.0f / (float)K;
         if (ln->tiles_out) *ln->tiles_out = N / 64;
     }
-    if (epi == vp::EPI_DECONV_FINAL) { g.W2 = c->w_fin; g.bias2 = c->b_fin; g.out2 = (float*)out; g.out = nullptr; }
+    if (epi == vp::EPI_DECONV_FINAL) { g.W2 = c->w_fin; g.bias2 = c->b_fin; g.out2 = (float*)out; g.out = nullptr; g.head_wgs = c->sw.head_wgs; }
     const bool deconv = epi == vp::EPI_DECONV || epi == vp::EPI_DECONV_FINAL;
     const double par = deconv ? 4.0 : 1.0;
     const double Nalg = (epi == vp::EPI_HEATMAP) ? (double)c->Kp : (double)N;
diff --git a/easy_vitpose_amd/csrc/gemm.hip b/easy_vitpose_amd/csrc/gemm.hip
--- a/easy_vitpose_amd/csrc/gemm.hip
+++ b/easy_vitpose_amd/csrc/gemm.hip
@@ -54,10 +54,23 @@
     const int tiles_n = (g.N + C::BN - 1) / C::BN;
     const int tiles_m = (g.M + C::BM - 1) / C::BM;
     int bid, parity = 0, split = 0;
-    if (AMODE == A_DECONV && g.parity_fast) {
-        const int lb = xcd_remap(blockIdx.x, tiles_m * tiles_n * 4);
+    constexpr bool HEAD = EPI_ == EPI_DECONV_FINAL;
+    constexpr int HEAD_RB = C::BN * 2 + 16, HEAD_RES_OFF = C::BM * HEAD_RB;
+    [[maybe_unused]] int lb = 0, lb_step = 0, lb_end = 0;
+    [[maybe_unused]] bool prefetched = false;
+    if (HEAD && g.parity_fast) {
+        const int nblk = tiles_m * tiles_n * 4, q = nblk >> 3, r8 = nblk & 7, xcd = blockIdx.x & 7;
+        const int base = (xcd < r8) ? xcd * (q + 1) : r8 * (q + 1) + (xcd - r8) * q;
+        lb = base + (blockIdx.x >> 3);
+        lb_step = gridDim.x >> 3;
+        lb_end = base + q + (xcd < r8 ? 1 : 0);
+        if (lb >= lb_end) return;
         parity = lb & 3;
         bid = lb >> 2;
+    } else if (AMODE == A_DECONV && g.parity_fast) {
+        const int lb1 = xcd_remap(blockIdx.x, tiles_m * tiles_n * 4);
+        parity = lb1 & 3;
+        bid = lb1 >> 2;
     } else if (EPI_ == EPI_PARTIAL) {
         const int lb = xcd_remap(blockIdx.x, tiles_m * tiles_n * g.splitk);
         split = lb / (tiles_m * tiles_n);
@@ -67,6 +80,32 @@
         if (AMODE == A_DECONV) parity = blockIdx.y;
     }
     if (g.reverse) bid = tiles_m * tiles_n - 1 - bid;
+    if constexpr (HEAD) {
+        if (g.w2_resident) {
+            char* res = smem + HEAD_RES_OFF;
+            for (int c = tid; c < 2 * g.Kp * 32; c += C::NT) {
+                const int row = c >> 5, u = row >> 5, kr = min(16, g.Kp - 16 * u), rr = row & 31;
+                const int src = u * 32 + (rr < kr ? rr : 16 + rr - kr);
+                *(u32x4*)(res + row * HEAD_RB + (c & 31) * 16) = *(const u32x4*)(g.W2 + (size_t)src * C::BN + (c & 31) * 8);
+            }
+            for (int j = tid; j < g.Kp; j += C::NT) *(float*)(res + 2 * g.Kp * HEAD_RB + j * 4) = g.bias2[j];
+            for (int j = tid; j < C::BN; j += C::NT) *(float*)(res + 2 * g.Kp * HEAD_RB + 128 + j * 4) = g.bias[j];
+        }
+    }
+    [[maybe_unused]] const int wave_s = HEAD ? __builtin_amdgcn_readfirstlane(tid >> 6) : 0;
+    auto fresh_tid = [&]() {
+        unsigned ones = ~0u;
+        asm volatile("" : "+s"(ones));
+        int win = g.Win, hin = g.Hin;
+        asm volatile("" : "+v"(win), "+v"(hin));
+        g.Win = __builtin_amdgcn_readfirstlane(win);
+        g.Hin = __builtin_amdgcn_readfirstlane(hin);
+        return wave_s * 64 + (int)__builtin_amdgcn_mbcnt_hi(ones, __builtin_amdgcn_mbcnt_lo(ones, 0u));
+    };
+    const int tid_once = tid;
+next_tile: __attribute__((unused));
+    {
+    const int tid = HEAD ? fresh_tid() : tid_once, lane = tid & 63, wave = tid >> 6;
     int tm, tn;
     if (g.group_m > 1) {
         const int per_group = g.group_m * tiles_n;
@@ -149,13 +188,15 @@
     for (int i = 0; i < C::TI; ++i)
 #pragma unroll
         for (int j = 0; j < C::TJ; ++j) acc[i][j] = f32x4{0.f, 0.f, 0.f, 0.f};
+    unsigned long long hs[HEAD ? 6 : 1] = {};
+    if (HEAD && (VP_ABLATE(g) & 32)) hs[0] = __builtin_readcyclecounter();
 
     const int nk = klen / C::BK;
     constexpr int KS = (C::PIPE == 6) ? 2 : 1;
     static_assert(C::PIPE != 6 || (C::STAGES >= 4 && C::KK == 2), "PIPE 6: >= 4 stages, BK = 64");
 #pragma unroll
     for (int s = 0; s < C::STAGES - KS; ++s)
-        if (s < nk) stage(s, s);
+        if (s < nk && !(HEAD && prefetched)) stage(s, s);
     if constexpr (EPI == EPI_BIAS || EPI == EPI_BIAS_GELU) {
         if (g.ln_part) {
             float2* st = (float2*)(smem + C::LDS);
@@ -181,6 +222,7 @@
         else wait_vmcnt<0>();
         __builtin_amdgcn_s_barrier();
         asm volatile("" ::: "memory");
+        if constexpr (HEAD) { if ((VP_ABLATE(g) & 32) && kt == 0) hs[1] = __builtin_readcyclecounter(); }
 #pragma unroll
         for (int ks = 0; ks < KS; ++ks) {
             const int pb = pbuf + ks >= C::STAGES ? pbuf + ks - C::STAGES : pbuf + ks;
@@ -239,88 +281,171 @@
 
     if constexpr (EPI == EPI_DECONV_FINAL) {
         static_assert(C::BN == 256 && C::BM % (C::NWAVES * 16) == 0, "the fused head needs all 256 channels in one tile");
-        constexpr int RB = C::BN * 2 + 16;
+        constexpr int RB = HEAD_RB;
         constexpr int RPW = C::BM / C::NWAVES, JW = RPW / 16;
-        f32x4 bias4[C::TI];
-#pragma unroll
-        for (int i = 0; i < C::TI; ++i) bias4[i] = *(const f32x4*)(g.bias + wn * C::WN + i * 16 + fg * 4);
-        asm volatile("s_waitcnt vmcnt(0)" ::: "memory");
-        __syncthreads();
-#pragma unroll
-        for (int j = 0; j < C::TJ; ++j) {
-            char* lrow = smem + (wm * C::WM + j * 16 + frow) * RB + (wn * C::WN + fg * 4) * 2;
-#pragma unroll
-            for (int i = 0; i < C::TI; ++i) {
-                f32x4 v = acc[i][j] + bias4[i];
-#pragma unroll
-                for (int r = 0; r < 4; ++r) v[r] = fmaxf(v[r], 0.f);
-                u32x2 o;
-                o[0] = pack2<T>(v[0], v[1]);
-                o[1] = pack2<T>(v[2], v[3]);
-                *(u32x2*)(lrow + i * 32) = o;
-            }
-        }
-        const int groups = (g.Kp + 15) >> 4;
-        auto ldw = [&](u32x4(&w)[16], int u) {
-            int frow_w = frow, fg_w = fg;
-            asm volatile("" : "+v"(frow_w), "+v"(fg_w));
-            const uint16_t* wrow = g.W2 + (size_t)(u * 32 + frow_w) * C::BN + fg_w * 8;
-#pragma unroll
-            for (int ks = 0; ks < 8; ++ks) {
-                w[2 * ks] = *(const u32x4*)(wrow + ks * 32);
-                w[2 * ks + 1] = *(const u32x4*)(wrow + 16 * C::BN + ks * 32);
+        static_assert(C::STAGES == 2 && C::PIPE != 6, "the first wait of a tile's K-loop must be vmcnt(0): it also stands for the previous tile's heatmap stores");
+        const bool has_next = lb + lb_step < lb_end;
+        auto tail = [&](auto res_t) {
+            constexpr bool RES = decltype(res_t)::value;
+            const int tid = fresh_tid(), lane = tid & 63, wave = tid >> 6, wn = wave / C::NWM, wm = wave % C::NWM, frow = lane & 15, fg = lane >> 4;
+            const int rip = lane / C::SLOTS, pslot = lane % C::SLOTS;
+            const char* res = smem + HEAD_RES_OFF;
+            const int res_b2 = 2 * g.Kp * RB, res_b = res_b2 + 128;
+            if (VP_ABLATE(g) & 32) hs[2] = __builtin_readcyclecounter();
+            f32x4 bias4[C::TI];
+#pragma unroll
+            for (int i = 0; i < C::TI; ++i)
+                bias4[i] = RES ? *(const f32x4*)(res + res_b + (wn * C::WN + i * 16 + fg * 4) * 4) : *(const f32x4*)(g.bias + wn * C::WN + i * 16 + fg * 4);
+            asm volatile("s_waitcnt vmcnt(0)" ::: "memory");
+            __syncthreads();
+#pragma unroll
+            for (int j = 0; j < C::TJ; ++j) {
+                char* lrow = smem + (wm * C::WM + j * 16 + frow) * RB + (wn * C::WN + fg * 4) * 2;
+#pragma unroll
+                for (int i = 0; i < C::TI; ++i) {
+                    f32x4 v = acc[i][j] + bias4[i];
+#pragma unroll
+                    for (int r = 0; r < 4; ++r) v[r] = fmaxf(v[r], 0.f);
+                    u32x2 o;
+                    o[0] = pack2<T>(v[0], v[1]);
+                    o[1] = pack2<T>(v[2], v[3]);
+                    *(u32x2*)(lrow + i * 32) = o;
+                }
+            }
+            const int groups = (g.Kp + 15) >> 4;
+            auto ldw = [&](u32x4(&w)[16], int u) {
+                int frow_w = frow, fg_w = fg;
+                asm volatile("" : "+v"(frow_w), "+v"(fg_w));
+                const uint16_t* wrow = g.W2 + (size_t)(u * 32 + frow_w) * C::BN + fg_w * 8;
+#pragma unroll
+                for (int ks = 0; ks < 8; ++ks) {
+                    w[2 * ks] = *(const u32x4*)(wrow + ks * 32);
+                    w[2 * ks + 1] = *(const u32x4*)(wrow + 16 * C::BN + ks * 32);
+                }
+            };
+            auto ldw_res = [&](u32x4(&w)[16], int u) {
+                int frow_w = frow, fg_w = fg;
+                asm volatile("" : "+v"(frow_w), "+v"(fg_w));
+                const int kr = min(16, g.Kp - 16 * u);
+                const char* wrow = res + (u * 32 + min(frow_w, kr - 1)) * RB + fg_w * 16;
+#pragma unroll
+                for (int ks = 0; ks < 8; ++ks) {
+                    w[2 * ks] = *(const u32x4*)(wrow + ks * 64);
+                    w[2 * ks + 1] = *(const u32x4*)(wrow + kr * RB + ks * 64);
+                }
+            };
+            auto prefetch0 = [&](int nlb) {
+                const int npar = nlb & 3, nm0 = (nlb >> 2) * C::BM;
+                const int di = npar >> 1, dj = npar & 1;
+                const uint16_t* Wn = g.W + (size_t)npar * g.w_parity_stride;
+                char* base = smem + wave * 1024;
+#pragma unroll
+                for (int p = 0; p < C::WP; ++p) {
+                    const int r = (p * C::NWAVES + wave) * C::RPG + rip;
+                    glds16(Wn + (size_t)r * K + swz<C::BK>(r, pslot) * 8, base + p * (C::NWAVES * 1024));
+                }
+#pragma unroll
+                for (int p = 0; p < C::AP; ++p) {
+                    const int r = (p * C::NWAVES + wave) * C::RPG + rip;
+                    int m = ((VP_ABLATE(g) & 2) ? 0 : nm0) + r;
+                    if (m > g.M - 1) m = g.M - 1;
+                    const int t = m / g.Win, i2 = t % g.Hin, j2 = m - t * g.Win;
+                    const bool ok = (unsigned)(i2 + di) < (unsigned)g.Hin && (unsigned)(j2 + dj) < (unsigned)g.Win;
+                    const uint16_t* src = ok ? g.A + (size_t)m * g.Cin + swz<C::BK>(r, pslot) * 8 + (ptrdiff_t)(di * g.Win + dj) * g.Cin : g.zero + pslot * 8;
+                    glds16(src, base + C::W_BYTES + p * (C::NWAVES * 1024));
+                }
+            };
+            u32x4 wA[16], wB[16];
+            if constexpr (!RES) ldw(wA, 0);
+            __syncthreads();
+            if (VP_ABLATE(g) & 32) hs[3] = __builtin_readcyclecounter();
+            u32x4 bf[JW][8];
+#pragma unroll
+            for (int jj = 0; jj < JW; ++jj)
+#pragma unroll
+                for (int ks = 0; ks < 8; ++ks) bf[jj][ks] = *(const u32x4*)(smem + (wave * RPW + jj * 16 + frow) * RB + (ks * 32 + fg * 8) * 2);
+            prefetched = false;
+            if (has_next) {
+                asm volatile("s_waitcnt lgkmcnt(0)" ::: "memory");
+                __builtin_amdgcn_s_barrier();
+                asm volatile("" ::: "memory");
+                if (RES && !(VP_ABLATE(g) & 128)) {
+                    prefetch0(lb + lb_step);
+                    prefetched = true;
+                }
+            }
+            if (VP_ABLATE(g) & 32) {
+                asm volatile("s_waitcnt lgkmcnt(0)" ::: "memory");
+                hs[4] = __builtin_readcyclecounter();
+            }
+            int oimg[JW], opx[JW];
+            const int opix = 4 * g.Hin * g.Win;
+#pragma unroll
+            for (int jj = 0; jj < JW; ++jj) {
+                const int m = m0 + wave * RPW + jj * 16 + frow;
+                const int t = m / g.Win, jx = m - t * g.Win, ii = t % g.Hin, img = t / g.Hin;
+                oimg[jj] = (m < g.M && !(VP_ABLATE(g) & 8)) ? img : -1;
+                opx[jj] = (2 * ii + (parity >> 1)) * (2 * g.Win) + 2 * jx + (parity & 1);
+            }
+            auto group = [&](const u32x4(&w)[16], int u) {
+                f32x4 ah[JW], al[JW];
+                int fg_g = fg;
+                asm volatile("" : "+v"(fg_g));
+                const int nb = u * 16 + fg_g * 4;
+                const f32x4 b2 = RES ? *(const f32x4*)(res + res_b2 + nb * 4)
+                                     : *(const f32x4*)(g.bias2 + nb);
+#pragma unroll
+                for (int jj = 0; jj < JW; ++jj) { ah[jj] = f32x4{0.f, 0.f, 0.f, 0.f}; al[jj] = f32x4{0.f, 0.f, 0.f, 0.f}; }
+#pragma unroll
+                for (int ks = 0; ks < 8; ++ks)
+#pragma unroll
+                    for (int jj = 0; jj < JW; ++jj) {
+                        ah[jj] = mfma16<T>(w[2 * ks], bf[jj][ks], ah[jj]);
+                        al[jj] = mfma16<T>(w[2 * ks + 1], bf[jj][ks], al[jj]);
+                    }
+#pragma unroll
+                for (int jj = 0; jj < JW; ++jj) {
+                    const f32x4 v = ah[jj] + al[jj];
+                    int im = oimg[jj], px = opx[jj];
+                    asm volatile("" : "+v"(im), "+v"(px));
+                    float* orow = g.out2 + ((size_t)im * g.Kp + nb) * opix + px;
+#pragma unroll
+                    for (int r = 0; r < 4; ++r)
+                        if (im >= 0 && nb + r < g.Kp) orow[(size_t)r * opix] = v[r] + b2[r];
+                }
+            };
+            int u = 0;
+            if constexpr (RES) {
+                do {
+                    ldw_res(wA, u);
+                    group(wA, u);
+                } while (++u < groups);
+            } else {
+                do {
+                    ldw(wB, min(u + 1, groups - 1));
+                    group(wA, u);
+                    ldw(wA, min(u + 2, groups - 1));
+                    if (u + 1 < groups) group(wB, u + 1);
+                    u += 2;
+                } while (u < groups);
+            }
+            if (VP_ABLATE(g) & 32) {
+                if (!prefetched) asm volatile("s_waitcnt vmcnt(0)" ::: "memory");
+                hs[5] = __builtin_readcyclecounter();
+                if (tid == 0) {
+                    unsigned long long* st = (unsigned long long*)g.stats_out + (size_t)(g.parity_fast ? lb : blockIdx.x) * 8;
+#pragma unroll
+                    for (int e = 0; e < 6; ++e) st[e] = hs[e];
+                }
             }
         };
-        u32x4 wA[16], wB[16];
-        ldw(wA, 0);
-        __syncthreads();
-        u32x4 bf[JW][8];
-#pragma unroll
-        for (int jj = 0; jj < JW; ++jj)
-#pragma unroll
-            for (int ks = 0; ks < 8; ++ks) bf[jj][ks] = *(const u32x4*)(smem + (wave * RPW + jj * 16 + frow) * RB + (ks * 32 + fg * 8) * 2);
-        int oimg[JW], opx[JW];
-        const int opix = 4 * g.Hin * g.Win;
-#pragma unroll
-        for (int jj = 0; jj < JW; ++jj) {
-            const int m = m0 + wave * RPW + jj * 16 + frow;
-            const int t = m / g.Win, jx = m - t * g.Win, ii = t % g.Hin, img = t / g.Hin;
-            oimg[jj] = (m < g.M && !(VP_ABLATE(g) & 8)) ? img : -1;
-            opx[jj] = (2 * ii + (parity >> 1)) * (2 * g.Win) + 2 * jx + (parity & 1);
-        }
-        auto group = [&](const u32x4(&w)[16], int u) {
-            f32x4 ah[JW], al[JW];
-            int fg_g = fg;
-            asm volatile("" : "+v"(fg_g));
-            const int nb = u * 16 + fg_g * 4;
-            const f32x4 b2 = *(const f32x4*)(g.bias2 + nb);
-#pragma unroll
-            for (int jj = 0; jj < JW; ++jj) { ah[jj] = f32x4{0.f, 0.f, 0.f, 0.f}; al[jj] = f32x4{0.f, 0.f, 0.f, 0.f}; }
-#pragma unroll
-            for (int ks = 0; ks < 8; ++ks)
-#pragma unroll
-                for (int jj = 0; jj < JW; ++jj) {
-                    ah[jj] = mfma16<T>(w[2 * ks], bf[jj][ks], ah[jj]);
-                    al[jj] = mfma16<T>(w[2 * ks + 1], bf[jj][ks], al[jj]);
-                }
-#pragma unroll
-            for (int jj = 0; jj < JW; ++jj) {
-                const f32x4 v = ah[jj] + al[jj];
-                int im = oimg[jj], px = opx[jj];
-                asm volatile("" : "+v"(im), "+v"(px));
-                float* orow = g.out2 + ((size_t)im * g.Kp + nb) * opix + px;
-#pragma unroll
-                for (int r = 0; r < 4; ++r)
-                    if (im >= 0 && nb + r < g.Kp) orow[(size_t)r * opix] = v[r] + b2[r];
-            }
-        };
-        for (int u = 0; u < groups; u += 2) {
-            if (u + 1 < groups) ldw(wB, u + 1);
-            group(wA, u);
-            if (u + 1 < groups) {
-                if (u + 2 < groups) ldw(wA, u + 2);
-                group(wB, u + 1);
-            }
+        if (g.w2_resident) tail(std::true_type{});
+        else tail(std::false_type{});
+        if (has_next) {
+            lb += lb_step;
+            parity = lb & 3;
+            bid = lb >> 2;
+            goto next_tile;
         }
     } else if constexpr (LN_PROD) {
         constexpr int ROWBYTES = C::BN * 4 + 16;
@@ -559,6 +684,7 @@
                     if (nb + r < g.Kp) ((float*)g.out)[orow + (size_t)(nb + r) * 3072] = v[r] + g.bias[nb + r];
             }
         }
+    }
     }
 }
 
@@ -819,9 +945,16 @@
     static_assert(LDS_BYTES + LN_STAT_BYTES <= 160 * 1024, "LDS");
     if (C::PIPE == 6 && a.K % 128 != 0) return hipErrorInvalidValue;
     if (a.ln_part && (a.ln_tiles & 1)) return hipErrorInvalidValue;
+    constexpr int HEAD_LDS_MAX = 160 * 1024;
+    int head_res_bytes = 0;
+    if constexpr (EPI == EPI_DECONV_FINAL) {
+        const long need = 2L * a.Kp * (C::BN * 2 + 16) + 128 + C::BN * 4;
+        if (a.parity_fast && a.Kp <= 32 && LDS_BYTES + need <= HEAD_LDS_MAX) head_res_bytes = (int)need;
+    }
     static bool attr_done[2][64] = {};
-    if (hipError_t e = lds_opt_in((const void*)kern, LDS_BYTES + LN_STAT_BYTES, attr_done[ex]); e != hipSuccess) return e;
+    if (hipError_t e = lds_opt_in((const void*)kern, EPI == EPI_DECONV_FINAL ? HEAD_LDS_MAX : LDS_BYTES + LN_STAT_BYTES, attr_done[ex]); e != hipSuccess) return e;
     GemmArgs g = a;
+    g.w2_resident = head_res_bytes != 0;
     const int tiles_n = (a.N + C::BN - 1) / C::BN;
     g.w_parity_stride = (size_t)a.w_rows * a.K;
     if ((size_t)tiles_n * C::BN > (size_t)a.w_rows) return hipErrorInvalidValue;
@@ -830,10 +963,17 @@
         if (a.splitk < 1 || a.K % (a.splitk * C::BK * (C::PIPE == 6 ? 2 : 1)) != 0 || a.ldo != a.N || a.N % 4 != 0) return hipErrorInvalidValue;
     }
     dim3 grid(AMODE == A_DECONV && a.parity_fast ? tiles * 4 : (EPI == EPI_PARTIAL ? tiles * a.splitk : tiles), AMODE == A_DECONV && !a.parity_fast ? 4 : 1);
+    if constexpr (EPI == EPI_DECONV_FINAL) {
+        if (a.parity_fast) {
+            int wgs = a.head_wgs > 0 ? a.head_wgs : 256;
+            if (wgs > tiles * 4) wgs = tiles * 4;
+            grid.x = (wgs + 7) & ~7;
+        }
+    }
     if (a.desc)
         snprintf(a.desc, a.desc_cap, "gemm_kernel<%s, %d, %d, TileCfg<%d, %d, %d, %d, %d, %d, %d>%s>", std::is_same<T, F16>::value ? "F16" : "BF16", EPI,
                  AMODE, C::BM, C::BN, C::BK, C::WM, C::WN, C::STAGES, C::PIPE, ex ? ", true" : "");
-    hipLaunchKernelGGL(kern, grid, dim3(C::NT), LDS_BYTES + (a.ln_part ? LN_STAT_BYTES : 0), s, g);
+    hipLaunchKernelGGL(kern, grid, dim3(C::NT), LDS_BYTES + head_res_bytes + (a.ln_part ? LN_STAT_BYTES : 0), s, g);
     return hipGetLastError();
 }
 
@@ -873,7 +1013,7 @@
         case EPI_POS_LN: return by_variant<T, EPI_POS_LN, A_DENSE>(a, s);
         case EPI_PARTIAL: return by_variant<T, EPI_PARTIAL, A_DENSE>(a, s);
         case EPI_DECONV_FINAL:
-            if (a.variant != 3 || a.N != Cfg3::BN || !a.W2 || !a.bias2 || !a.out2 || a.Kp <= 0) return hipErrorInvalidValue;
+            if (a.variant != 3 || a.N != Cfg3::BN || !a.W2 || !a.bias2 || !a.out2 || a.Kp <= 0 || a.reverse || a.ln_part) return hipErrorInvalidValue;
             return launch<T, EPI_DECONV_FINAL, A_DECONV, Cfg3>(a, s);
     }
     return hipErrorInvalidValue;
diff --git a/easy_vitpose_amd/csrc/handle.hip b/easy_vitpose_amd/csrc/handle.hip
--- a/easy_vitpose_amd/csrc/handle.hip
+++ b/easy_vitpose_amd/csrc/handle.hip
@@ -83,6 +83,7 @@
     on("VP_GRAPH_NULL", s.graph_null);
     if (const char* f = getenv("VP_CALLER_STREAM")) s.caller_stream_max_n = atoi(f) == 1 ? 16 : atoi(f);
     on("VP_FUSE_HEAD", s.fuse_head);
+    num("VP_HEAD_WGS", s.head_wgs);
     if (const char* f = getenv("VP_FOLD_STATS")) { s.graph_max_n_stats = atoi(f); s.fold_rule = false; }
     on("VP_BLOCKED_QKV", s.blocked_qkv);
     on("VP_FUSE_QKV_ATTN", s.fuse_qkv_attn);
diff --git a/easy_vitpose_amd/csrc/kernels.h b/easy_vitpose_amd/csrc/kernels.h
--- a/easy_vitpose_amd/csrc/kernels.h
+++ b/easy_vitpose_amd/csrc/kernels.h
@@ -53,12 +53,14 @@
     int Hin, Win, Cin;
     const uint16_t* zero;
     int Kp;
+    int w2_resident;
     const uint16_t* W2;
     const float* bias2;
     float* out2;
     int w_rows;
     int variant;
     int group_m;
+    int head_wgs;
     size_t w_parity_stride;
     size_t plane;
     float* stats_out;
diff --git a/easy_vitpose_amd/csrc/tools_taps.hip b/easy_vitpose_amd/csrc/tools_taps.hip
--- a/easy_vitpose_amd/csrc/tools_taps.hip
+++ b/easy_vitpose_amd/csrc/tools_taps.hip
@@ -235,6 +235,50 @@
     return dbg_finish(c, VP_OK);
 }
 
+VP_API int vp_dbg_head_timeline(int32_t device, int32_t dtype, int32_t nh, int32_t Kp, int32_t iters, uint64_t* stamps, int32_t n_slots, float* ms_out) {
+    if (nh <= 0 || Kp <= 0 || iters <= 0 || !stamps || !ms_out || n_slots < nh * 12) return fail(nullptr, VP_ERR_INVALID, "bad head timeline request");
+    vp_ctx* c = dbg_ctx(device, dtype);
+    if (!c) return VP_ERR_HIP;
+    const int M = nh * 768, Cin = 256, K = 4 * Cin;
+    const size_t fin_rows = (size_t)(Kp + 15) / 16 * 32, nst = (size_t)n_slots * 8;
+    uint16_t *dA, *dW, *dW2;
+    float *dB, *dB2, *dO;
+    unsigned long long* dS;
+    int rc;
+    if ((rc = dalloc(c, &dA, (size_t)M * Cin)) || (rc = dalloc(c, &dW, (size_t)4 * 256 * K)) || (rc = dalloc(c, &dW2, pad128(fin_rows) * 256)) || (rc = dalloc(c, &dB, (size_t)256)) ||
+        (rc = dalloc(c, &dB2, pad128(Kp))) || (rc = dalloc(c, &dO, (size_t)nh * Kp * 3072)) || (rc = dalloc(c, &dS, nst)) || (rc = dalloc(c, &c->zero, (size_t)256)))
+        return dbg_finish(c, rc);
+    vp::fill_random16(c->dtype, dA, (size_t)M * Cin, 1u, nullptr);
+    vp::fill_random16(c->dtype, dW, (size_t)4 * 256 * K, 2u, nullptr);
+    vp::fill_random16(c->dtype, dW2, pad128(fin_rows) * 256, 3u, nullptr);
+    hipMemset(dB, 0, 256 * 4); hipMemset(dB2, 0, pad128(Kp) * 4); hipMemset(c->zero, 0, 512); hipMemset(dS, 0, nst * 8);
+    vp::GemmArgs g{};
+    g.A = dA; g.W = dW; g.bias = dB; g.M = M; g.N = 256; g.K = K; g.ldo = 256; g.Hin = 32; g.Win = 24; g.Cin = Cin; g.zero = c->zero; g.Kp = Kp;
+    g.W2 = dW2; g.bias2 = dB2; g.out2 = dO; g.w_rows = 256; g.variant = 3; g.parity_fast = 1;
+    if (const char* e = getenv("VP_HEAD_WGS")) g.head_wgs = atoi(e);
+    const int abl = getenv("VP_TL_ABL") ? atoi(getenv("VP_TL_ABL")) : 0;
+    g.ablate = abl;
+    hipEvent_t e0, e1;
+    hipEventCreate(&e0); hipEventCreate(&e1);
+    hipError_t e = hipSuccess;
+    for (int i = 0; i < 2 && e == hipSuccess; ++i) e = vp::gemm_launch(c->dtype, vp::EPI_DECONV_FINAL, g, nullptr);
+    hipDeviceSynchronize();
+    hipEventRecord(e0, nullptr);
+    for (int i = 0; i < iters && e == hipSuccess; ++i) e = vp::gemm_launch(c->dtype, vp::EPI_DECONV_FINAL, g, nullptr);
+    hipEventRecord(e1, nullptr);
+    if (e == hipSuccess) e = hipDeviceSynchronize();
+    float ms = 0.f;
+    hipEventElapsedTime(&ms, e0, e1);
+    *ms_out = ms / iters;
+    hipEventDestroy(e0); hipEventDestroy(e1);
+    g.ablate = 32 | abl; g.stats_out = (float*)dS;
+    if (e == hipSuccess) e = vp::gemm_launch(c->dtype, vp::EPI_DECONV_FINAL, g, nullptr);
+    if (e == hipSuccess) e = hipDeviceSynchronize();
+    if (e == hipSuccess) e = hipMemcpy(stamps, dS, nst * 8, hipMemcpyDeviceToHost);
+    if (e != hipSuccess) return dbg_finish(c, fail(c, VP_ERR_HIP, std::string("head timeline: ") + hipGetErrorString(e)));
+    return dbg_finish(c, VP_OK);
+}
+
 VP_API int vp_dbg_gemm_compare(int32_t device, int32_t dtype, int32_t epi, int32_t variant_a, int32_t group_a, int32_t flags_a,
                                int32_t variant_b, int32_t group_b, int32_t flags_b, int32_t M, int32_t N, int32_t K, int32_t reps,
                                uint64_t* n_mismatch, double* max_abs_diff) {
diff --git a/include/vitpose_hip.h b/include/vitpose_hip.h
--- a/include/vitpose_hip.h
+++ b/include/vitpose_hip.h
@@ -282,6 +282,8 @@
                             const float* gamma, const float* beta, float* out16, float* out32);
 VP_API int vp_dbg_deconv(int32_t device_id, int32_t dtype, int32_t B, int32_t Hin, int32_t Win, int32_t Cin,
                          const float* x, const vp_tensor_desc* tensors, int32_t n_tensors, float* out);
+VP_API int vp_dbg_head_case(int32_t device_id, int32_t dtype, int32_t nh, int32_t Kp, int32_t head_wgs, const float* x, const float* w, const float* b,
+                            const float* wf, const float* bf, float* out_fused, float* out_pair);
 VP_API int vp_dbg_crop_prep(int32_t device_id, const uint8_t* frame, int32_t fh, int32_t fw, const int32_t* crop_params,
                             int32_t n, uint8_t* out);
 VP_API int vp_dbg_gemm_case(int32_t device_id, int32_t dtype, int32_t epi, int32_t variant, int32_t group_m, int32_t flags,
```

After: 25740 persons/s, median of 6. No clear change (+0.9%).
